# Nextomics/NextPolish2

Hardware: AMD Instinct MI355X
Metric: polished reference Mbp/s (whole node) at 30x HiFi + k21/k31; FASTA identical to oracle (higher is better)
Workload: dtype u8

## Files before the change

### nextpolish2_amd/csrc/np2_batch.cpp

```cpp
#include "../../include/np2.h"
#include "np2_ctx.hpp"

#include <atomic>
#include <climits>
#include <cstring>
#include <condition_variable>
#include <mutex>
#include <thread>
#include <pthread.h>

#include <linux/futex.h>
#include <sys/syscall.h>
#include <unistd.h>

using namespace np2;

namespace {

struct Job {
    np2_contig *contig = nullptr;
    const np2_opts_t *opts = nullptr;
    uint8_t **out_bases = nullptr;
    uint32_t **out_pos = nullptr;
    uint64_t *out_len = nullptr;
    uint32_t *out_span = nullptr;
    int *rc = nullptr;
};

}

struct np2_batch {
    np2_ctx *parent = nullptr;
    int device = 0;
    hipStream_t stream = nullptr;
    std::vector<np2_ctx *> slots;
    std::vector<Recorder> recs;
    std::vector<std::thread> workers;
    std::string err;

    std::mutex mu;
    std::condition_variable cv_start, cv_done;
    uint64_t job_gen = 0;
    std::vector<Job> jobs;
    int n_running = 0;
    bool quit = false;

    std::mutex sync_mu;
    int n_active = 0, n_waiting = 0;
    std::atomic<uint32_t> flush_gen{0};
    std::atomic<bool> failed{false};
    std::string fail_msg;

    uint32_t *done_host = nullptr, *done_dev = nullptr;
    uint32_t done_seq = 0;
    std::atomic<uint32_t> issued_seq{0};
    std::atomic<uint32_t> done_pub{0};
    std::atomic<bool> spinner{false};
    double t_issued_last = 0;
    uint32_t wait_logged_seq = 0;

    bool time_diff = false;
    std::vector<std::pair<hipEvent_t, hipEvent_t>> diff_events;
    size_t diff_used = 0;
    float last_diff_ms = 0;
    int last_diff_launches = 0;
    uint64_t stat_launches = 0, stat_cmds = 0, stat_flushes = 0;
    double t_last_end = 0, ms_host = 0, ms_issue = 0, ms_wait = 0;
    std::vector<double> flush_log;
    double call_ms = 0, tail_ms = 0;
};

namespace {

inline void wait_generation(std::atomic<uint32_t> &gen, uint32_t seen) {
    static const double spin_us = getenv("NP2_BATCH_SPIN_US") ? atof(getenv("NP2_BATCH_SPIN_US")) : (wait_naps() ? 0.0 : 5.0);
    const double t_end = now_ms() + spin_us * 1e-3;
    for (;;) {
        for (int i = 0; i < 64; ++i) {
            if (gen.load(std::memory_order_acquire) != seen) return;
            __builtin_ia32_pause();
        }
        if (now_ms() >= t_end) break;
    }
    while (gen.load(std::memory_order_acquire) == seen)
        (void)syscall(SYS_futex, reinterpret_cast<uint32_t *>(&gen), FUTEX_WAIT_PRIVATE, seen, nullptr, nullptr, 0);
}
inline void publish_generation(std::atomic<uint32_t> &gen, uint32_t next) {
    gen.store(next, std::memory_order_release);
    (void)syscall(SYS_futex, reinterpret_cast<uint32_t *>(&gen), FUTEX_WAKE_PRIVATE, INT_MAX, nullptr, nullptr, 0);
}

__device__ __forceinline__ void k_flush_done(const uint32_t np2_bid, const uint32_t np2_nb, uint32_t *__restrict__ word, uint32_t seq) {
    if (threadIdx.x == 0) {
        __threadfence_system();
        __hip_atomic_store(word, seq, __ATOMIC_RELEASE, __HIP_MEMORY_SCOPE_SYSTEM);
    }
}

void flush(np2_batch *b) {
    const int n = (int)b->recs.size();
    const double t_begin = now_ms();
    double t_issued = t_begin;
    std::vector<size_t> idx(n, 0);
    hipStream_t s = b->stream;
    Recorder *saved = tl_recorder();
    tl_recorder() = nullptr;
    try {
        for (;;) {
            bool any = false;
            for (int i = 0; i < n; ++i) {
                auto &q = b->recs[i].q;
                while (idx[i] < q.size() && !q[idx[i]].kd) {
                    q[idx[i]].fn(s);
                    ++idx[i];
                    ++b->stat_cmds;
                }
                any |= idx[i] < q.size();
            }
            if (!any) break;
            const KernelDesc *best = nullptr;
            int best_n = 0, best_defer = 0;
            static constexpr size_t LOOKAHEAD = 8;
            for (int i = 0; i < n; ++i) {
                auto &q = b->recs[i].q;
                if (idx[i] >= q.size()) continue;
                const KernelDesc *kd = q[idx[i]].kd;
                bool seen = false;
                for (int j = 0; j < i && !seen; ++j)
                    seen = idx[j] < b->recs[j].q.size() && b->recs[j].q[idx[j]].kd == kd;
                if (seen) continue;
                int c = 0, defer = 0;
                for (int j = 0; j < n; ++j) {
                    auto &qj = b->recs[j].q;
                    if (idx[j] >= qj.size()) continue;
                    if (qj[idx[j]].kd == kd) {
                        ++c;
                        continue;
                    }
                    for (size_t k = idx[j] + 1; k < qj.size() && k <= idx[j] + LOOKAHEAD; ++k)
                        if (qj[k].kd == kd) {
                            ++defer;
                            break;
                        }
                }
                if (!best || defer < best_defer || (defer == best_defer && c > best_n)) best = kd, best_n = c, best_defer = defer;
            }
            uint32_t grids[MAXB];
            const void *args[MAXB];
            int m = 0;
            const bool timed = b->time_diff && strcmp(best->name, "k_diff_reads") == 0;
            auto issue = [&]() {
                if (!m) return;
                if (timed) {
                    if (b->diff_used == b->diff_events.size()) {
                        hipEvent_t e0 = nullptr, e1 = nullptr;
                        HIPCHK(hipEventCreate(&e0));
                        HIPCHK(hipEventCreate(&e1));
                        b->diff_events.push_back({e0, e1});
                    }
                    HIPCHK(hipEventRecord(b->diff_events[b->diff_used].first, s));
                }
                best->launch(s, m, grids, args);
                if (timed) {
                    HIPCHK(hipEventRecord(b->diff_events[b->diff_used].second, s));
                    ++b->diff_used;
                }
                ++b->stat_launches;
                m = 0;
            };
            for (int i = 0; i < n; ++i) {
                auto &r = b->recs[i];
                if (idx[i] >= r.q.size() || r.q[idx[i]].kd != best) continue;
                grids[m] = r.q[idx[i]].grid;
                args[m] = r.arena.data() + r.q[idx[i]].arg_off;
                ++m;
                ++idx[i];
                ++b->stat_cmds;
                if (m == best->max_batch) issue();
            }
            issue();
        }
        HIPCHK(hipGetLastError());
        const uint32_t seq = ++b->done_seq;
        NP2_LAUNCH(k_flush_done, 1, 64, s, b->done_dev, seq);
        t_issued = now_ms();
        b->issued_seq.store(seq, std::memory_order_release);
    } catch (const std::exception &ex) {
        b->fail_msg = ex.what();
        b->failed.store(true);
        (void)hipStreamSynchronize(s);
        for (np2_ctx *cx : b->slots) cx->lb_dirty = true, cx->h2d_inflight = false;
    }
    tl_recorder() = saved;
    for (auto &r : b->recs) r.clear();
    ++b->stat_flushes;
    b->ms_host += t_begin - b->t_last_end;
    b->ms_issue += t_issued - t_begin;
    b->flush_log.push_back(t_begin - b->t_last_end);
    b->flush_log.push_back(t_issued - t_begin);
    b->flush_log.push_back(0.0);
    b->t_last_end = t_issued;
    b->t_issued_last = t_issued;
}

void wait_done(np2_batch *b, uint32_t seq) {
    for (;;) {
        const uint32_t pub = b->done_pub.load(std::memory_order_acquire);
        if ((int32_t)(pub - seq) >= 0 || b->failed.load()) break;
        bool expected = false;
        if (b->spinner.compare_exchange_strong(expected, true)) {
            uint64_t spins = 0;
            uint32_t cur;
            HostWait hw;
            while ((int32_t)((cur = __atomic_load_n(b->done_host, __ATOMIC_ACQUIRE)) - seq) < 0) {
                if (b->failed.load()) break;
                if ((++spins & (wait_naps() ? 0xFFu : 0xFFFFu)) == 0) {
                    hipError_t e = hipStreamQuery(b->stream);
                    if (e != hipSuccess && e != hipErrorNotReady) {
                        b->fail_msg = std::string("device error during a batch flush: ") + hipGetErrorString(e);
                        b->failed.store(true);
                        break;
                    }
                    if (e == hipSuccess && (int32_t)(__atomic_load_n(b->done_host, __ATOMIC_ACQUIRE) - seq) < 0) {
                        b->fail_msg = "batch flush completed without posting";
                        b->failed.store(true);
                        break;
                    }
                }
                hw.pause();
            }
            b->spinner.store(false);
            publish_generation(b->done_pub, b->failed.load() ? pub + 1 : cur);
            if (b->failed.load()) return;
            continue;
        }
        wait_generation(b->done_pub, pub);
    }
    if (b->failed.load()) return;
    std::lock_guard<std::mutex> l(b->sync_mu);
    if (b->wait_logged_seq != seq && b->issued_seq.load() == seq && !b->flush_log.empty()) {
        const double t = now_ms();
        b->wait_logged_seq = seq;
        b->ms_wait += t - b->t_issued_last;
        b->flush_log.back() = t - b->t_issued_last;
        b->t_last_end = t;
    }
}

void group_sync(Recorder *r, bool need_done) {
    np2_batch *b = (np2_batch *)r->group;
    uint32_t my_gen;
    bool flushed = false;
    {
        std::lock_guard<std::mutex> l(b->sync_mu);
        my_gen = b->flush_gen.load(std::memory_order_relaxed);
        if (++b->n_waiting == b->n_active) {
            flush(b);
            b->n_waiting = 0;
            publish_generation(b->flush_gen, my_gen + 1);
            flushed = true;
        }
    }
    if (!flushed) wait_generation(b->flush_gen, my_gen);
    if (need_done && !b->failed.load()) wait_done(b, b->issued_seq.load(std::memory_order_acquire));
    if (b->failed.load()) throw Np2Error(NP2_E_DEVICE, "batch flush failed: " + b->fail_msg);
}

void leave_wave(np2_batch *b, Recorder *r) {
    std::lock_guard<std::mutex> l(b->sync_mu);
    if (!r->q.empty()) {
        np2_ctx *cx = b->slots[r->slot];
        cx->lb_dirty = true;
        cx->h2d_inflight = false;
    }
    r->clear();
    --b->n_active;
    if (b->n_active > 0 && b->n_waiting == b->n_active) {
        const uint32_t g = b->flush_gen.load(std::memory_order_relaxed);
        flush(b);
        b->n_waiting = 0;
        publish_generation(b->flush_gen, g + 1);
    }
}

void worker_main(np2_batch *b, int slot) {
    (void)hipSetDevice(b->device);
    (void)pthread_setname_np(pthread_self(), "np2-slot");
    uint64_t seen = 0;
    for (;;) {
        Job job;
        {
            std::unique_lock<std::mutex> l(b->mu);
            b->cv_start.wait(l, [&] { return b->quit || b->job_gen != seen; });
            if (b->quit) return;
            seen = b->job_gen;
            job = b->jobs[slot];
        }
        if (!job.contig) continue;
        Recorder *r = &b->recs[slot];
        tl_recorder() = r;
        int rc = np2_polish_resident(b->slots[slot], job.contig, job.opts, job.out_bases, job.out_pos, job.out_len);
        tl_recorder() = nullptr;
        for (auto &g : r->graveyard)
            dev_release_idle(g.first, (g.second >> 63) ? 0 : g.second, (g.second >> 63) ? (g.second & ~(1ull << 63)) : 0);
        r->graveyard.clear();
        leave_wave(b, r);
        if (rc == NP2_OK && job.out_span) (void)np2_last_span(b->slots[slot], &job.out_span[0], &job.out_span[1]);
        *job.rc = rc;
        {
            std::lock_guard<std::mutex> l(b->mu);
            if (--b->n_running == 0) b->cv_done.notify_all();
        }
    }
}

auto batch_sink(np2_batch *b) {
    return [b](int, const std::string &msg) { b->err = msg; };
}

}

extern "C" {

int np2_batch_create(np2_batch_t **out, np2_ctx_t *parent, int n_slots) {
    if (!out || !parent || n_slots < 1 || n_slots > 256) return NP2_E_ARG;
    *out = nullptr;
    return abi_guard([&] {
        std::unique_ptr<np2_batch, void (*)(np2_batch_t *)> b(new np2_batch(), np2_batch_destroy);
        b->parent = parent;
        b->device = parent->device;
        HIPCHK(hipSetDevice(b->device));
        HIPCHK(hipStreamCreateWithFlags(&b->stream, hipStreamNonBlocking));
        HIPCHK(hipHostMalloc((void **)&b->done_host, 256 * (size_t)(n_slots + 1), hipHostMallocMapped | hipHostMallocCoherent));
        memset(b->done_host, 0, 256 * (size_t)(n_slots + 1));
        HIPCHK(hipHostGetDevicePointer((void **)&b->done_dev, b->done_host, 0));
        b->recs.resize(n_slots);
        b->jobs.resize(n_slots);
        for (int i = 0; i < n_slots; ++i) {
            np2_ctx *cx = ctx_create_slot(parent, b->stream, b->done_host + 64 * (size_t)(i + 1), b->done_dev + 64 * (size_t)(i + 1));
            b->slots.push_back(cx);
            b->recs[i].group = b.get();
            b->recs[i].slot = i;
            b->recs[i].sync_fn = &group_sync;
        }
        for (int i = 0; i < n_slots; ++i) b->workers.emplace_back(worker_main, b.get(), i);
        *out = b.release();
        return NP2_OK;
    }, [parent](int, const std::string &msg) { parent->err = msg; });
}

void np2_batch_destroy(np2_batch_t *b) {
    if (!b) return;
    {
        std::lock_guard<std::mutex> l(b->mu);
        b->quit = true;
    }
    b->cv_start.notify_all();
    for (auto &t : b->workers) t.join();
    (void)hipSetDevice(b->device);
    if (b->stream) (void)hipStreamSynchronize(b->stream);
    {
        DevSyncScope idle;
        for (np2_ctx *cx : b->slots) np2_ctx_destroy(cx);
    }
    for (auto &e : b->diff_events) {
        (void)hipEventDestroy(e.first);
        (void)hipEventDestroy(e.second);
    }
    if (b->done_host) (void)hipHostFree(b->done_host);
    if (b->stream) (void)hipStreamDestroy(b->stream);
    delete b;
}

int np2_batch_set_priority(np2_batch_t *b, int high) {
    if (!b) return NP2_E_ARG;
    return abi_guard([&] {
        HIPCHK(hipSetDevice(b->device));
        int least = 0, greatest = 0;
        HIPCHK(hipDeviceGetStreamPriorityRange(&least, &greatest));
        HIPCHK(hipStreamSynchronize(b->stream));
        hipStream_t s = nullptr;
        HIPCHK(hipStreamCreateWithPriority(&s, hipStreamNonBlocking, high ? greatest : least));
        (void)hipStreamDestroy(b->stream);
        b->stream = s;
        for (np2_ctx *cx : b->slots) ctx_slot_set_stream(cx, s);
        return NP2_OK;
    }, batch_sink(b));
}

int np2_batch_slots(np2_batch_t *b) { return b ? (int)b->slots.size() : 0; }
np2_ctx_t *np2_batch_slot_ctx(np2_batch_t *b, int slot) {
    return (b && slot >= 0 && slot < (int)b->slots.size()) ? b->slots[slot] : nullptr;
}
const char *np2_batch_last_error(np2_batch_t *b) { return b ? b->err.c_str() : "null batch"; }
int np2_batch_set_sink(np2_batch_t *b, int slot, void *device_ptr, uint64_t cap) {
    if (!b || slot < 0 || slot >= (int)b->slots.size()) return NP2_E_ARG;
    b->slots[slot]->sink_dst = (uint8_t *)device_ptr;
    b->slots[slot]->sink_cap = device_ptr ? cap : 0;
    return NP2_OK;
}

int np2_batch_polish(np2_batch_t *b, np2_contig_t *const *contigs, int n, const np2_opts_t *opts, uint8_t **out_bases,
                     uint32_t **out_pos, uint64_t *out_len, uint32_t *out_span, int *rcs) {
    if (!b || !contigs || n < 0 || !opts || !out_len || !rcs) return NP2_E_ARG;
    return abi_guard([&] {
        const int S = (int)b->slots.size();
        int worst = NP2_OK;
        b->diff_used = 0;
        b->flush_log.clear();
        b->t_last_end = now_ms();
        const double t_call0 = b->t_last_end;
        for (int w0 = 0; w0 < n; w0 += S) {
            const int m = std::min(S, n - w0);
            {
                std::lock_guard<std::mutex> l(b->mu);
                for (int i = 0; i < S; ++i) {
                    Job j;
                    if (i < m) {
                        j.contig = contigs[w0 + i];
                        j.opts = opts;
                        j.out_bases = out_bases ? &out_bases[w0 + i] : nullptr;
                        j.out_pos = out_pos ? &out_pos[w0 + i] : nullptr;
                        j.out_len = &out_len[w0 + i];
                        j.out_span = out_span ? &out_span[2 * (w0 + i)] : nullptr;
                        j.rc = &rcs[w0 + i];
                    }
                    b->jobs[i] = j;
                }
                b->n_running = m;
                {
                    std::lock_guard<std::mutex> l2(b->sync_mu);
                    b->n_active = m;
                    b->n_waiting = 0;
                    b->failed.store(false);
                }
                ++b->job_gen;
            }
            b->cv_start.notify_all();
            {
                std::unique_lock<std::mutex> l(b->mu);
                b->cv_done.wait(l, [&] { return b->n_running == 0; });
            }
            for (int i = 0; i < m; ++i)
                if (rcs[w0 + i] != NP2_OK) {
                    worst = rcs[w0 + i];
                    b->err = std::string("contig ") + std::to_string(w0 + i) + ": " + np2_last_error(b->slots[i]);
                }
        }
        b->call_ms = now_ms() - t_call0;
        b->tail_ms = now_ms() - b->t_last_end;
        if (b->time_diff) {
            b->last_diff_ms = 0;
// ... 41 lines not shown
```

### nextpolish2_amd/csrc/np2_cand.hip

```cpp
#include "np2_common.hpp"
#include "np2_kernels.hpp"
#include "np2_blockscan.hpp"
#include "np2_lookback.hpp"

namespace np2 {

template <int MODE>
__device__ __forceinline__ void k_scan_small(const uint32_t np2_bid, const uint32_t np2_nb, const uint32_t *__restrict__ in, uint32_t *__restrict__ out,
                                                     uint32_t n_host, const uint32_t *__restrict__ n_dev,
                                                     uint32_t *__restrict__ total_out, bool write_end) {
    __shared__ uint32_t sh[16];
    const uint32_t n = n_dev ? min(*n_dev, n_host) : n_host;
    uint32_t total;
    if (MODE == 2) {
        total = block_scan_array<OpMinI32>(
            n, sh, [&](uint32_t i) { return in[i]; },
            [&](uint32_t i, uint32_t pre, uint32_t v) { out[i] = OpMinI32::apply(pre, v); });
    } else {
        total = block_scan_array<OpAdd>(
            n, sh, [&](uint32_t i) { return in[i]; },
            [&](uint32_t i, uint32_t pre, uint32_t v) { out[i] = MODE == 0 ? pre : pre + v; });
    }
    if (threadIdx.x == 0) {
        if (MODE == 0 && write_end) out[n] = total;
        if (total_out) *total_out = total;
    }
}

static constexpr uint32_t SCAN_LB_ITEMS = 8;
static constexpr uint32_t SCAN_LB_THREADS = 1024;
static constexpr uint32_t SCAN_LB_BLOCK = SCAN_LB_ITEMS * SCAN_LB_THREADS;
template <bool POPC>
__device__ __forceinline__ void scan_lb_excl_body(const uint32_t np2_bid, const uint32_t np2_nb, Lookback lb, uint32_t n_blocks, const uint32_t *__restrict__ in,
                                                      uint32_t *__restrict__ out, uint32_t n, bool write_end,
                                                      uint32_t *__restrict__ err) {
    __shared__ uint32_t sh[16];
    const uint32_t bid = lb_block_id(lb, sh);
    const uint32_t i0 = bid * SCAN_LB_BLOCK + threadIdx.x * SCAN_LB_ITEMS;
    uint32_t v[SCAN_LB_ITEMS], sum = 0;
    const bool wide = (((uintptr_t)in | (uintptr_t)out) & 15) == 0;
    if (wide && i0 + SCAN_LB_ITEMS <= (POPC ? n - 1 : n)) {
        const uint4 a = *reinterpret_cast<const uint4 *>(in + i0), b = *reinterpret_cast<const uint4 *>(in + i0 + 4);
        v[0] = a.x, v[1] = a.y, v[2] = a.z, v[3] = a.w, v[4] = b.x, v[5] = b.y, v[6] = b.z, v[7] = b.w;
    } else {
#pragma unroll
        for (uint32_t k = 0; k < SCAN_LB_ITEMS; ++k) v[k] = i0 + k < (POPC ? n - 1 : n) ? in[i0 + k] : 0u;
    }
    if (POPC) {
#pragma unroll
        for (uint32_t k = 0; k < SCAN_LB_ITEMS; ++k) v[k] = (uint32_t)__builtin_popcount(v[k]);
    }
#pragma unroll
    for (uint32_t k = 0; k < SCAN_LB_ITEMS; ++k) sum += v[k];
    uint32_t total, pre, dummy;
    uint32_t run = block_excl_scan<OpAdd, 16>(sum, sh, total);
    lb_exclusive2(lb, bid, total, 0u, sh, err, pre, dummy);
    run += pre;
    if (wide && i0 + SCAN_LB_ITEMS <= n) {
        uint4 a, b;
        a.x = run, a.y = a.x + v[0], a.z = a.y + v[1], a.w = a.z + v[2];
        b.x = a.w + v[3], b.y = b.x + v[4], b.z = b.y + v[5], b.w = b.z + v[6];
        *reinterpret_cast<uint4 *>(out + i0) = a;
        *reinterpret_cast<uint4 *>(out + i0 + 4) = b;
        run = b.w + v[7];
    } else {
#pragma unroll
        for (uint32_t k = 0; k < SCAN_LB_ITEMS; ++k) {
            if (i0 + k < n) out[i0 + k] = run;
            run += v[k];
        }
    }
    if (write_end && n && i0 <= n - 1 && n - 1 < i0 + SCAN_LB_ITEMS) out[n] = run;
    if (write_end && n == 0 && bid == 0 && threadIdx.x == 0) out[0] = 0;
}

__device__ __forceinline__ void k_scan_lb_excl(const uint32_t np2_bid, const uint32_t np2_nb, Lookback lb, uint32_t n_blocks, const uint32_t *__restrict__ in,
                                               uint32_t *__restrict__ out, uint32_t n, bool write_end, uint32_t *__restrict__ err) {
    scan_lb_excl_body<false>(np2_bid, np2_nb, lb, n_blocks, in, out, n, write_end, err);
}
__device__ __forceinline__ void k_scan_lb_popc(const uint32_t np2_bid, const uint32_t np2_nb, Lookback lb, uint32_t n_blocks, const uint32_t *__restrict__ in,
                                               uint32_t *__restrict__ out, uint32_t n, bool write_end, uint32_t *__restrict__ err) {
    scan_lb_excl_body<true>(np2_bid, np2_nb, lb, n_blocks, in, out, n, write_end, err);
}

struct CandCtx {
    const np2_read_t *reads;
    const uint8_t *nib;
    const uint64_t *ck_off;
    const uint32_t *ckpt;
    const uint32_t *lq_start;
    const uint32_t *lq_end;
    const uint32_t *pj;
    const uint32_t *pcount;
    const uint8_t *alive;
    const ReadInfo *rinfo;
    const uint32_t *tile_rd_off;
    const uint32_t *tile_rd;
    uint32_t n_tiles;
    uint32_t ksize;
    const uint64_t *rec_key;
    const uint32_t *rec_read;
    const uint32_t *tile_n;
    const uint16_t *rec_pidx;
    uint32_t bucket_cap;
    const uint32_t *refnib;
    uint32_t L;
};

__device__ __forceinline__ void cand_anchor(const CandCtx &cx, uint32_t r, const np2_read_t &rd, uint64_t ck_off, uint32_t start,
                                            uint32_t &col, uint32_t &t) {
    col = 0;
    t = rd.aln_t_s;
    const uint32_t ck_first = (rd.aln_t_s + CKPT - 1) >> CKPT_SHIFT;
    const uint32_t cki = start >> CKPT_SHIFT;
    if (r == 0) {
        col = start;
        t = start;
    } else if (cki >= ck_first) {
        col = cx.ckpt[ck_off + (cki - ck_first)];
        t = cki << CKPT_SHIFT;
    }
}

__device__ __forceinline__ uint32_t nth_col16(uint64_t m64, uint32_t n) {
    uint32_t col = 0;
    uint32_t m = (uint32_t)m64;
    uint32_t c = (uint32_t)__builtin_popcount(m);
    if (n > c) n -= c, col = 8, m = (uint32_t)(m64 >> 32);
    c = (uint32_t)__builtin_popcount(m & 0xFFFFu);
    if (n > c) n -= c, col += 4, m >>= 16;
    c = (uint32_t)__builtin_popcount(m & 0xFFu);
    if (n > c) n -= c, col += 2, m >>= 8;
    c = (uint32_t)__builtin_popcount(m & 0xFu);
    if (n > c) col += 1;
    return col;
}

__device__ uint32_t cand_measure(const CandCtx &cx, uint32_t r, const np2_read_t &rd, uint64_t ck_off, uint32_t start,
                                 uint32_t end, uint32_t &col_start) {
    uint32_t col_ck, t_ck;
    cand_anchor(cx, r, rd, ck_off, start, col_ck, t_ck);
    col_start = col_ck;
    if (end < t_ck) return 0;
    const uint32_t want_s = (start > t_ck ? start - t_ck : 0u) + 1;
    const uint32_t want_e = end + 1 - t_ck + 1;
    const uint8_t *base = cx.nib + rd.nib_off;
    const uint32_t n_cols = rd.n_cols;
    uint32_t seen = 0, len = 0;
    bool started = false;
    uint4 win = make_uint4(0, 0, 0, 0);
    uint32_t win_blk = 0xFFFFFFFFu;
    const uint64_t N1 = 0x1111111111111111ULL;
    for (uint32_t wi = col_ck >> 4;; ++wi) {
        const uint32_t c0 = wi << 4;
        if (c0 >= n_cols) break;
        if ((wi >> 1) != win_blk) {
            win_blk = wi >> 1;
            win = *reinterpret_cast<const uint4 *>(base + ((size_t)win_blk << 4));
        }
        const uint32_t r0 = (wi & 1) ? win.z : win.x, r1 = (wi & 1) ? win.w : win.y;
        const uint64_t w = (uint64_t)(((r0 & 0x0F0F0F0Fu) << 4) | ((r0 >> 4) & 0x0F0F0F0Fu)) |
                           ((uint64_t)(((r1 & 0x0F0F0F0Fu) << 4) | ((r1 >> 4) & 0x0F0F0F0Fu)) << 32);
        uint64_t valid = N1;
        if (c0 < col_ck) valid &= ~((1ULL << (4 * (col_ck - c0))) - 1ULL);
        if (n_cols - c0 < 16) valid &= (1ULL << (4 * (n_cols - c0))) - 1ULL;
// ... 402 lines not shown
        if (lane == 0) {
            reg_ncand[g] = kept;
            reg_bytes[g] = bytes;
            reg_maxlen[g] = mx;
        }
        sum_k[h / 4] += kept, sum_b[h / 4] += bytes, sum_m[h / 4] += mx;
    }
#pragma unroll
    for (uint32_t q = 0; q < RM_RPW / 4; ++q)
        if (lane == 0 && mb0 + q < n_mb) {
            blk_sum[mb0 + q] = sum_k[q];
            blk_sum[n_mb + mb0 + q] = sum_b[q];
            blk_sum[2 * n_mb + mb0 + q] = sum_m[q];
        }
}

__device__ __forceinline__ void k_cand_offsets(const uint32_t np2_bid, const uint32_t np2_nb, const uint32_t *__restrict__ blk_sum, uint32_t n_blk,
                                                       uint32_t n_reg, uint32_t *__restrict__ blk_coff,
                                                       uint32_t *__restrict__ blk_soff, uint32_t *__restrict__ cand_off,
                                                       uint32_t *__restrict__ reg_soff, uint32_t *__restrict__ n_cand,
                                                       uint32_t *__restrict__ n_bytes, uint32_t *__restrict__ grow) {
    __shared__ uint32_t sh[16];
    const uint32_t ta = block_scan_array<OpAdd>(
        n_blk, sh, [&](uint32_t i) { return blk_sum[i]; }, [&](uint32_t i, uint32_t pre, uint32_t) { blk_coff[i] = pre; });
    const uint32_t tb = block_scan_array<OpAdd>(
        n_blk, sh, [&](uint32_t i) { return blk_sum[n_blk + i]; },
        [&](uint32_t i, uint32_t pre, uint32_t) { blk_soff[i] = pre; });
    const uint32_t tc = block_scan_array<OpAdd>(
        n_blk, sh, [&](uint32_t i) { return blk_sum[2 * n_blk + i]; }, [&](uint32_t, uint32_t, uint32_t) {});
    if (threadIdx.x == 0) {
        cand_off[n_reg] = ta;
        reg_soff[n_reg] = tb;
        *n_cand = ta;
        *n_bytes = tb;
        *grow = tc;
    }
}

__device__ __forceinline__ void k_cand_offsets_lb(const uint32_t np2_bid, const uint32_t np2_nb, Lookback lb, uint32_t n_blocks, const uint32_t *__restrict__ blk_sum,
                                                         uint32_t n_blk, uint32_t n_reg, uint32_t *__restrict__ blk_coff,
                                                         uint32_t *__restrict__ blk_soff, uint32_t *__restrict__ cand_off,
                                                         uint32_t *__restrict__ reg_soff, uint32_t *__restrict__ n_cand,
                                                         uint32_t *__restrict__ n_bytes, uint32_t *__restrict__ grow,
                                                         uint32_t *__restrict__ err) {
    __shared__ uint32_t sh[8];
    const uint32_t bid = lb_block_id(lb, sh);
    const uint32_t i0 = (bid * 256 + threadIdx.x) * 4;
    uint32_t a[4], b[4], sa = 0, sb = 0;
#pragma unroll
    for (uint32_t k = 0; k < 4; ++k) {
        a[k] = i0 + k < n_blk ? blk_sum[i0 + k] : 0u;
        b[k] = i0 + k < n_blk ? blk_sum[n_blk + i0 + k] : 0u;
        sa += a[k];
        sb += b[k];
    }
    uint32_t ta, tb, pa, pb;
    uint32_t ra = block_excl_scan<OpAdd, 4>(sa, sh, ta);
    uint32_t rb = block_excl_scan<OpAdd, 4>(sb, sh, tb);
    lb_exclusive2(lb, bid, ta, tb, sh, err, pa, pb);
    ra += pa, rb += pb;
#pragma unroll
    for (uint32_t k = 0; k < 4; ++k)
        if (i0 + k < n_blk) {
            blk_coff[i0 + k] = ra;
            blk_soff[i0 + k] = rb;
            ra += a[k];
            rb += b[k];
        }
    if (bid == n_blocks - 1 && threadIdx.x == 255) {
        cand_off[n_reg] = ra;
        reg_soff[n_reg] = rb;
        *n_cand = ra;
        *n_bytes = rb;
    }
    if (bid == 0) {
        uint32_t c = 0, tc;
        for (uint32_t i = threadIdx.x; i < n_blk; i += 256) c += blk_sum[2 * n_blk + i];
        (void)block_excl_scan<OpAdd, 4>(c, sh, tc);
        if (threadIdx.x == 0) *grow = tc;
    }
}

static constexpr uint32_t MERGE_LB_BLOCKS = 32;
__device__ __forceinline__ void k_lq_merge_scan_lb(const uint32_t np2_bid, const uint32_t np2_nb, Lookback lb, const uint32_t *__restrict__ raw_start,
                                                   const uint32_t *__restrict__ raw_end, const uint32_t *__restrict__ n_raw, uint32_t n_host,
                                                   uint32_t *__restrict__ headflag, uint32_t *__restrict__ hidx, uint32_t *__restrict__ err) {
    __shared__ uint32_t sh[16];
    const uint32_t bid = lb_block_id(lb, sh);
    const uint32_t n = min(*n_raw, n_host);
    const uint32_t seg = ((n + MERGE_LB_BLOCKS - 1) / MERGE_LB_BLOCKS + 1023u) & ~1023u;
    const uint32_t lo = min(bid * seg, n), hi = min(lo + seg, n);
    auto flag = [&](uint32_t j) { return (j >= 1 && raw_end[j] >= raw_start[j - 1]) ? 0u : 1u; };
    uint32_t cnt = 0;
    for (uint32_t j = lo + threadIdx.x; j < hi; j += 1024) cnt += flag(j);
    uint32_t total, pre, dummy;
    (void)block_excl_scan<OpAdd, 16>(cnt, sh, total);
    lb_exclusive2(lb, bid, total, 0u, sh, err, pre, dummy);
    uint32_t carry = pre;
    for (uint32_t j0 = lo; j0 < hi; j0 += 1024) {
        const uint32_t j = j0 + threadIdx.x;
        const uint32_t v = j < hi ? flag(j) : 0u;
        uint32_t tot;
        const uint32_t ex = block_excl_scan<OpAdd, 16>(v, sh, tot);
        if (j < hi) {
            hidx[j] = carry + ex;
            headflag[j] = v;
        }
        carry += tot;
    }
}

__device__ __forceinline__ void k_region_write(const uint32_t np2_bid0, const uint32_t np2_nb, CandCtx cx, uint32_t n_reg, const uint32_t *__restrict__ kept_read,
                                                      const uint32_t *__restrict__ kept_len,
                                                      const uint32_t *__restrict__ kept_col,
                                                      const uint32_t *__restrict__ reg_ncand,
                                                      const uint32_t *__restrict__ reg_bytes,
                                                      const uint32_t *__restrict__ blk_coff,
                                                      const uint32_t *__restrict__ blk_soff,
                                                      uint32_t *__restrict__ cand_off, uint32_t *__restrict__ reg_soff,
                                                      uint32_t cand_cap,
                                                      uint32_t seq_cap, uint32_t *__restrict__ cand_order,
                                                      uint64_t *__restrict__ cand_kmer, uint32_t *__restrict__ cand_seq_off,
                                                      uint8_t *__restrict__ cand_seq) {
    const uint32_t np2_bid = xcd_order(np2_bid0, np2_nb);
    __shared__ __attribute__((aligned(4))) uint8_t s_str[RM_REG][CLEAN_MAX_LEN];
    __shared__ uint64_t s_km[RM_REG];
    __shared__ uint32_t s_so[RM_REG][64];
    __shared__ uint32_t s_oc[RM_REG];
    __shared__ uint32_t s_q[4][RM_RPW * 64];
    const uint32_t lane = threadIdx.x & 63, wv = (uint32_t)__builtin_amdgcn_readfirstlane((int)(threadIdx.x >> 6));
    const uint32_t g0 = (np2_bid * 4 + wv) * RM_RPW, mb0 = g0 / 4;
    uint32_t nq = 0;
    uint32_t oc = 0, ob = 0;
    if (g0 < n_reg) oc = blk_coff[mb0], ob = blk_soff[mb0];
    uint32_t clean_h = 0;
    uint32_t my_len[RM_RPW], my_so[RM_RPW], my_ci[RM_RPW];
    bool my_clean[RM_RPW];
    uint32_t n[RM_RPW], rb[RM_RPW], st[RM_RPW], ln0[RM_RPW];
#pragma unroll
    for (uint32_t h = 0; h < RM_RPW; ++h) {
        const uint32_t g = g0 + h;
        n[h] = 0, rb[h] = 0, st[h] = 0, ln0[h] = 0;
        if (g < n_reg) n[h] = reg_ncand[g], rb[h] = reg_bytes[g], st[h] = cx.lq_start[g], ln0[h] = cx.lq_end[g] - st[h] + 1;
    }
    uint32_t len[RM_RPW], col[RM_RPW], rd_[RM_RPW], refc[RM_RPW];
#pragma unroll
    for (uint32_t h = 0; h < RM_RPW; ++h) {
        const size_t ks = (size_t)(g0 + h) * LQSEQ_MAX_CAN_COUNT + lane;
        const bool act = lane < n[h];
        len[h] = act ? kept_len[ks] : 0u;
        col[h] = act ? kept_col[ks] : 0u;
        rd_[h] = act ? kept_read[ks] : 0u;
        const uint32_t p = st[h] + lane;
        refc[h] = (n[h] && lane < ln0[h] && ln0[h] <= CLEAN_MAX_LEN) ? cx.refnib[p >> 3] >> (4 * (p & 7)) : 0u;
    }
#pragma unroll
    for (uint32_t h = 0; h < RM_RPW; ++h) {
        const uint32_t g = g0 + h, slot = wv * RM_RPW + h;
        my_len[h] = 0, my_so[h] = 0, my_ci[h] = 0, my_clean[h] = false;
        if (g >= n_reg) continue;
        if (g == n_reg - 1 && lane == 0 && cand_off[n_reg] < cand_cap) cand_seq_off[cand_off[n_reg]] = reg_soff[n_reg];
        if (lane == 0) {
            cand_off[g] = oc;
            reg_soff[g] = ob;
            s_oc[slot] = oc;
        }
        const bool act = lane < n[h];
        const uint32_t so = ob + wave_excl(len[h]);
        const uint32_t ci = oc + lane;
        const bool ok = act && ci < cand_cap && (uint64_t)so + len[h] <= seq_cap;
        if (ok) {
            cand_order[ci] = rd_[h];
            cand_seq_off[ci] = so;
        }
        const bool clean = ok && col[h] == CAND_CLEAN;
        const uint64_t cm = __ballot(clean);
        const bool queued = ok && (!clean || (lane == 0 && rd_[h] == 0));
        my_len[h] = len[h], my_so[h] = so, my_ci[h] = ci, my_clean[h] = clean && !queued;
        s_so[slot][lane] = so;
        if (cm) {
            clean_h |= 1u << h;
            if (lane < ln0[h]) s_str[slot][lane] = (uint8_t)((0x54474341u >> (8 * (refc[h] & 3))) & 0xFFu);
        }
        const uint64_t dq = __ballot(queued);
        if (queued) s_q[wv][nq + lanes_below(dq)] = (slot << 6) | lane;
        nq += (uint32_t)__builtin_popcountll(dq);
        oc += n[h];
        ob += rb[h];
    }
    wave_lds_sync();
    for (uint32_t e = lane; e < nq; e += 64) {
        const uint32_t w = s_q[wv][e], slot = w >> 6, li = w & 63;
        const uint32_t g = (np2_bid * 4 + slot / RM_RPW) * RM_RPW + slot % RM_RPW;
        const size_t ks = (size_t)g * LQSEQ_MAX_CAN_COUNT + li;
        const uint32_t r = kept_read[ks], len = kept_len[ks];
        uint32_t col = kept_col[ks];
        const ReadInfo ri = cx.rinfo[r];
        const np2_read_t rd = rinfo_read(ri);
        const uint32_t t0 = max(cx.lq_start[g], rd.aln_t_s);
        if (col == CAND_CLEAN) col = t0;
        const uint32_t ci = s_oc[slot] + li;
        uint64_t km;
        cand_write(cx, r, rd, ri.pj, g, col, t0, len, cand_seq + s_so[slot][li], &km);
        cand_kmer[ci] = km;
        if (li == 0 && r == 0) s_km[slot] = km;
    }
    wave_lds_sync();
#pragma unroll
    for (uint32_t h = 0; h < RM_RPW; ++h) {
        if (!((clean_h >> h) & 1u)) continue;
        const uint32_t slot = wv * RM_RPW + h;
        if (my_clean[h]) {
            cand_kmer[my_ci[h]] = s_km[slot];
            typedef uint32_t u32_any __attribute__((aligned(1)));
            uint8_t *dst = cand_seq + my_so[h];
            const uint32_t L4 = my_len[h] & ~3u;
            for (uint32_t j = 0; j < L4; j += 4) *reinterpret_cast<u32_any *>(dst + j) = *reinterpret_cast<const uint32_t *>(&s_str[slot][j]);
            for (uint32_t j = L4; j < my_len[h]; ++j) dst[j] = s_str[slot][j];
        }
    }
}

void launch_scan_small_excl(hipStream_t s, const uint32_t *in, uint32_t *out, uint32_t n, const uint32_t *n_dev,
                            uint32_t *total_out, bool write_end) {
    NP2_LAUNCH(k_scan_small<0>, dim3(1), 1024, s, in, out, n, n_dev, total_out, write_end);
}
void launch_scan_lb_excl(hipStream_t s, const Lookback &lb, const uint32_t *in, uint32_t *out, uint32_t n, bool write_end,
                          uint32_t *err) {
    const uint32_t nb = scan_lb_blocks(n);
    NP2_LAUNCH(k_scan_lb_excl, dim3(nb), SCAN_LB_THREADS, s, lb, nb, in, out, n, write_end, err);
}
void launch_scan_lb_popc(hipStream_t s, const Lookback &lb, const uint32_t *bits, uint32_t *out, uint32_t n_words, uint32_t *err) {
    const uint32_t nb = scan_lb_blocks((uint64_t)n_words + 1);
    NP2_LAUNCH(k_scan_lb_popc, dim3(nb), SCAN_LB_THREADS, s, lb, nb, bits, out, n_words + 1, false, err);
}
uint32_t scan_lb_blocks(uint64_t n) { return (uint32_t)std::max<uint64_t>(1, (n + SCAN_LB_BLOCK - 1) / SCAN_LB_BLOCK); }
void launch_scan_small_incl(hipStream_t s, const int32_t *in, int32_t *out, uint32_t n, const uint32_t *n_dev) {
    NP2_LAUNCH(k_scan_small<1>, dim3(1), 1024, s, (const uint32_t *)in, (uint32_t *)out, n, n_dev, (uint32_t *)nullptr, false);
}
void launch_scan_small_min(hipStream_t s, const int32_t *in, int32_t *out, uint32_t n, const uint32_t *n_dev) {
    NP2_LAUNCH(k_scan_small<2>, dim3(1), 1024, s, (const uint32_t *)in, (uint32_t *)out, n, n_dev, (uint32_t *)nullptr, false);
}
static CandCtx mk_cand(const CandPtrs &c) {
    return CandCtx{c.reads, c.nib,    c.ck_off, c.ckpt,        c.lq_start, c.lq_end, c.pj,
                   c.pcount, c.alive, c.rinfo, c.tile_rd_off, c.tile_rd, c.n_tiles,  c.ksize,
                   c.rec_key, c.rec_read, c.tile_n, c.rec_pidx, c.bucket_cap, c.refnib, c.L};
}
void launch_region_measure(hipStream_t s, const CandPtrs &c, uint32_t n_reg, uint32_t *kept_read, uint32_t *kept_len,
                           uint32_t *kept_col, uint32_t *reg_ncand, uint32_t *reg_bytes, uint32_t *reg_maxlen,
                           uint32_t *blk_sum) {
    if (n_reg)
        NP2_LAUNCH_WAVES(k_region_measure, RM_WAVES, dim3((n_reg + RM_REG - 1) / RM_REG), 256, s,
                         mk_cand(c), n_reg, kept_read, kept_len, kept_col, reg_ncand, reg_bytes, reg_maxlen, blk_sum);
}
uint32_t cand_offsets_blocks(uint32_t n_reg) { return ((n_reg + 3) / 4 + 1023) / 1024; }
void launch_cand_offsets(hipStream_t s, const uint32_t *blk_sum, uint32_t n_reg, uint32_t *blk_coff, uint32_t *blk_soff,
                         uint32_t *cand_off, uint32_t *reg_soff, uint32_t *n_cand, uint32_t *n_bytes, uint32_t *grow,
                         const Lookback *lb, uint32_t *err) {
    if (lb)
        NP2_LAUNCH(k_cand_offsets_lb, dim3(cand_offsets_blocks(n_reg)), 256, s, *lb, cand_offsets_blocks(n_reg), blk_sum, (n_reg + 3) / 4, n_reg, blk_coff, blk_soff, cand_off, reg_soff, n_cand, n_bytes, grow, err);
    else
        NP2_LAUNCH(k_cand_offsets, dim3(1), 1024, s, blk_sum, (n_reg + 3) / 4, n_reg, blk_coff, blk_soff, cand_off, reg_soff, n_cand, n_bytes, grow);
}
void launch_lq_merge_scan_lb(hipStream_t s, const Lookback &lb, const uint32_t *raw_start, const uint32_t *raw_end, const uint32_t *n_raw,
                             uint32_t n_host, uint32_t *headflag, uint32_t *hidx, uint32_t *err) {
    NP2_LAUNCH(k_lq_merge_scan_lb, dim3(MERGE_LB_BLOCKS), 1024, s, lb, raw_start, raw_end, n_raw, n_host, headflag, hidx, err);
}
uint32_t lq_merge_lb_blocks() { return MERGE_LB_BLOCKS; }
void launch_region_write(hipStream_t s, const CandPtrs &c, uint32_t n_reg, const uint32_t *kept_read,
                         const uint32_t *kept_len, const uint32_t *kept_col, const uint32_t *reg_ncand,
                         const uint32_t *reg_bytes, const uint32_t *blk_coff, const uint32_t *blk_soff, uint32_t *cand_off,
                         uint32_t *reg_soff, uint32_t cand_cap, uint32_t seq_cap, uint32_t *cand_order, uint64_t *cand_kmer,
                         uint32_t *cand_seq_off, uint8_t *cand_seq) {
    if (n_reg)
        NP2_LAUNCH(k_region_write, dim3((n_reg + RM_REG - 1) / RM_REG), 256, s, mk_cand(c), n_reg, kept_read, kept_len, kept_col, reg_ncand, reg_bytes, blk_coff, blk_soff, cand_off, reg_soff, cand_cap, seq_cap, cand_order, cand_kmer, cand_seq_off, cand_seq);
}

}
```

### nextpolish2_amd/csrc/np2_ctx.hpp

```cpp
#pragma once
#include "../../include/np2.h"
#include "np2_abi.hpp"
#include "np2_common.hpp"
#include "np2_kernels.hpp"
#include "np2_hostcpu.hpp"

#include <algorithm>
#include <chrono>
#include <cstdio>
#include <cstdlib>
#include <cstring>
#include <map>
#include <memory>
#include <exception>
#include <mutex>
#include <stdexcept>
#include <string>
#include <vector>

namespace np2h {

using namespace np2;


// ... 341 lines not shown
}

struct YakTable {
    uint32_t k = 0, cap_log2 = 0;
    std::shared_ptr<DevBuf<uint64_t>> table;
    std::shared_ptr<DevBuf<uint32_t>> ord;
    YakDev dev() const { return YakDev{table->p, cap_log2, k, ord ? ord->p : nullptr}; }
};

struct Timing {
    std::vector<std::string> names;
    std::vector<float> ms;
    std::string joined;
    std::vector<std::pair<std::string, float>> host;
};
inline double now_ms() {
    return std::chrono::duration<double, std::milli>(std::chrono::steady_clock::now().time_since_epoch()).count();
}


}

using namespace np2h;

struct np2_contig {
    np2_contig() {
        reads.cached = nib.cached = refnib.cached = ck_off.cached = ckpt.cached = descs.cached = true;
        tile_rd_off.cached = tile_rd.cached = true;
    }
    uint32_t L = 0, R = 0;
    uint64_t nib_bytes = 0, n_cols = 0, n_ckpt = 0;
    DevBuf<np2_read_t> reads;
    DevBuf<uint8_t> nib;
    DevBuf<uint8_t> refnib;
    uint32_t ref_stride = 0;
    DevBuf<uint64_t> ck_off;
    DevBuf<uint32_t> ckpt;
    uint32_t n_chunks = 0;
    DevBuf<ChunkDesc> descs;
    uint32_t n_tiles = 0;
    DevBuf<uint32_t> tile_rd_off, tile_rd;
    uint32_t tile_cap = TILE_CAP;
};

struct np2_ctx {
    int device = 0;
    hipStream_t stream = nullptr;
    hipStream_t stream_out = nullptr;
    hipEvent_t ev_out = nullptr;
    uint8_t *out_host[2] = {nullptr, nullptr};
    size_t out_host_cap[2] = {0, 0};
    int out_slot = 0;
    bool out_pending = false;
    uint64_t out_len = 0;
    std::vector<YakTable> yaks;
    std::string err;
    bool trace = false;
    std::map<std::string, std::vector<uint8_t>> trace_items;
    Timing timing;
    std::vector<std::pair<std::string, std::pair<hipEvent_t, hipEvent_t>>> pending_events;

    PinnedBuf pin_d2h, pin_h2d;
    uint32_t *mbox_host = nullptr, *mbox_dev = nullptr;
    uint32_t mbox_seq = 0;
    bool borrowed_state = false;
    uint8_t *sink_dst = nullptr;
    uint64_t sink_cap = 0;
    uint32_t last_first_pos = 0, last_last_pos = 0;
    const uint8_t *last_dbase = nullptr;
    const uint32_t *last_dpos = nullptr;
    DevBuf<uint32_t> shard_bounds;
    uint64_t last_len = 0;
    bool reuse_identical_pass = true;
    bool h2d_inflight = false;
    bool stage_timing = false;
    DevBuf<uint8_t> tmp;
    DevBuf<uint64_t> keys_raw, keys;
    DevBuf<uint32_t> vals_raw, vals;
    DevBuf<uint32_t> npos, ncount, nminr, nbesti, node_off, run_start, run_end, n0_besti, emit, eoff;
    DevBuf<uint16_t> nbases, ndelta;
    DevBuf<int64_t> nscore;
    DevBuf<int32_t> cov, mval, smin;
    DevBuf<uint8_t> alive, cns_base, cns_cls, lq_kind, lq_nothead;
    DevBuf<uint32_t> cns_pos, lq_next, rflag, rstart, rend, ridx, raw_start, raw_end, headflag, hidx, lq_start,
        lq_end;
    DevBuf<uint32_t> pj, pcount, reg_ncand, reg_bytes, reg_soff, reg_maxlen, blk_sum, blk_coff, blk_soff, kept_read, kept_len, kept_col, cand_off, cand_order, cand_seq_off, kill_ids;
    DevBuf<uint64_t> cand_kmer;
    DevBuf<uint8_t> cand_seq;
    DevBuf<uint16_t> kscore;
    DevBuf<uint32_t> scal;
    DevBuf<uint64_t> lb_status;
    DevBuf<uint32_t> lb_ticket;
    uint32_t lb_ticket_total = 0, lb_epoch = 0;
    bool lb_dirty = false;
    static constexpr size_t LB_MAX_BLOCKS = 1u << 20;
    DevBuf<uint32_t> mlen;
    DevBuf<uint8_t> reg_lable, grp, cns_base2, rech_groups, rech_groups_tmp;
    DevBuf<uint8_t> votepack;
    DevBuf<uint8_t> votepack2;
    DevBuf<uint32_t> rech_headjobs;
    DevBuf<uint32_t> ecount, eval, eval_s, eflag, eidx, seed_cand, keep_n, keep_list, cns_pos2, sp_idx_s,
        sp_idx_e, ap_g, ap_s, ap_e, rech, rech_joboff, job_len,
        job_off32;
    DevBuf<int32_t> ew, ap_delta, ap_shift;
    DevBuf<uint64_t> ekey, ekey_s;
    DevBuf<uint16_t> keep_ks;
    DevBuf<uint32_t> long_list;
    DevBuf<uint64_t> bt_path;
    DevBuf<uint64_t> chunk_st;
    uint32_t chunk_epoch = 0;
    DevBuf<uint32_t> tile_cur, tile_n, tile_scan, tile_scanb, tile_nn, tile_nr, tile_noff, tile_roff;
    uint32_t tile_cap = TILE_CAP;
    uint32_t bucket_cap = 0;
    DevBuf<uint2> nrec;
    DevBuf<uint8_t> votebuf;
    DevBuf<uint32_t> band, band_n, band_off, row_cnt;
    DevBuf<int64_t> run_gain, tile_gain;
    DevBuf<uint8_t> out_snap;
    DevBuf<uint8_t> run_flag;
    uint32_t deep_min = 65536;
    DevBuf<uint32_t> lq_list, hbits;
    DevBuf<uint16_t> tile_pidx;
    bool pidx_valid = false;
    DevBuf<ReadInfo> rinfo;
    DevBuf<uint32_t> lqc, lqoff;
    DevBuf<uint8_t> pflag;
    DevBuf<uint32_t> dp_list;
    DevBuf<uint16_t> pf_slots;
    DevBuf<uint32_t> pf_bad, pf_bad2;
    DevBuf<uint64_t> pf_prof;
    bool front_fused = false;
    struct Hooks {
        bool front_unfused = false, pf_prof = false, edge_sort = false;
        bool test_misspeculate = false, shard_spec_log = false, phase_profile = false, exact_grow = false, no_speculate = false;
        bool has_grow_guess = false;
        uint32_t grow_guess = 0;
        bool has_pf_cap = false, has_pf_cap_big = false, has_pf_halo = false, has_pf_cov_max = false;
        uint32_t pf_cap = 0, pf_cap_big = 0, pf_halo = 0, pf_cov_max = 0;
        void read() {
            auto on = [](const char *n) { return getenv(n) != nullptr; };
            auto u32 = [](const char *n, bool &has, uint32_t &v) {
                if (const char *e = getenv(n)) has = true, v = (uint32_t)atol(e);
            };
            front_unfused = on("NP2_FRONT_UNFUSED"), pf_prof = on("NP2_PF_PROF"), edge_sort = on("NP2_EDGE_SORT");
            test_misspeculate = on("NP2_TEST_MISSPECULATE");
            shard_spec_log = on("NP2_SHARD_SPEC_LOG"), phase_profile = on("NP2_PHASE_PROFILE"), exact_grow = on("NP2_EXACT_GROW");
            no_speculate = on("NP2_NO_SPECULATE");
            u32("NP2_TEST_GROW_GUESS", has_grow_guess, grow_guess);
            u32("NP2_PF_CAP", has_pf_cap, pf_cap), u32("NP2_PF_CAP_BIG", has_pf_cap_big, pf_cap_big);
            u32("NP2_PF_HALO", has_pf_halo, pf_halo), u32("NP2_PF_COV_MAX", has_pf_cov_max, pf_cov_max);
        }
    } hooks;
    bool pf_big = getenv("NP2_PF_BIG") != nullptr;
    uint32_t front_redos = 0;
    DevBuf<uint16_t> kscore_saved;
    DevBuf<uint8_t> sstr;
    DevBuf<uint64_t> soff;
    DevBuf<uint16_t> sscore;
};


namespace np2h {


enum Scal { S_ERR = 0, S_NNODES, S_NRUNS, S_BEST, S_PATHBEGIN, S_NRAW, S_NREG, S_DUP, S_LAST0, S_LAST1, S_GAIN0,
            S_GAIN1, S_DEEP, S_NDPLIST, S_NRECH, S_NGROUPS, S_NLONG, S_NLQ, S_PF, S_M0, S_M1, S_M2, S_M3, S_NC, S_SB, S_GROW,
            S_NBAD, S_PFOUT, S_PFGAIN0, S_PFGAIN1, S_PFEND0, S_PFEND1, S_NBAD2, S_NOKEY, S_COUNT = 34 };
static_assert(S_M1 % 2 == 0 && S_LAST0 % 2 == 0 && S_GAIN0 % 2 == 0 && S_PFGAIN0 % 2 == 0 && S_PFEND0 % 2 == 0,
              "64-bit device counters live in these slot pairs");

static constexpr int NP2_MAX_YAK = 15;
static constexpr uint32_t SCAL_TOTAL = 96;
static_assert(S_COUNT + 2 * (NP2_MAX_YAK + 2) <= SCAL_TOTAL && S_COUNT < 64, "round counters behind the posted block; the mailbox holds 64 words");

inline double thread_cpu_ms() {
    timespec ts;
    clock_gettime(CLOCK_THREAD_CPUTIME_ID, &ts);
    return ts.tv_sec * 1e3 + ts.tv_nsec * 1e-6;
}
struct WallTimer {
    np2_ctx *cx;
    const char *name;
    double t0, c0 = 0;
    WallTimer(np2_ctx *c, const char *n);
    ~WallTimer();
};
// ... 247 lines not shown
```

### nextpolish2_amd/csrc/np2_host.cpp

```cpp
#include "../../include/np2.h"
#include "np2_common.hpp"
#include "np2_kernels.hpp"
#include "np2_ctx.hpp"
#include "np2_phase_host.hpp"

#include <algorithm>
#include <atomic>
#include <thread>
#include <chrono>
#include <cstdio>
#include <cstdlib>
#include <cstring>
#include <map>
#include <mutex>
#include <stdexcept>
#include <string>
#include <unordered_map>
#include <unordered_set>
#include <future>
#include <functional>
#include <vector>

using namespace np2;

// ... 130 lines not shown
            off_own.assign(off, off + R + 1);
            edges_own.assign(edges, edges + off[R]);
            off = off_own.data(), edges = edges_own.data();
        }
        if (!view_key) return;
        pair_key.assign(view_key, view_key + view_n);
        pair_cnt.assign(view_cnt, view_cnt + view_n);
        view_key = nullptr, view_cnt = nullptr, view_n = 0;
    }
    std::vector<uint32_t> first_key;
    std::vector<int32_t> ref_w;
    std::vector<uint8_t> ref_seen, bad;
    const uint8_t *d_bad = nullptr;
    bool key_added = false;
};

bool vote_rows_from_pairs(VoteData &vd, bool use_all) {
    const uint32_t R = vd.R;
    const uint64_t *k = vd.keys();
    const uint32_t *cn = vd.cnts();
    const uint64_t np = vd.n_pairs();
    std::vector<uint32_t> n_lo(R, 0), n_up(R, 0);
    uint32_t nokey = 0;
    auto listed = [&](uint64_t i, uint32_t &a, uint32_t &b) {
        a = (uint32_t)(k[i] >> 32), b = (uint32_t)k[i];
        if (a >= R || b >= R || vd.first_key[a] == 0xFFFFFFFFu || vd.first_key[b] == 0xFFFFFFFFu) return false;
        return use_all || !(vd.bad[a] | vd.bad[b]);
    };
    for (uint64_t i = 0; i < np; ++i) {
        uint32_t a = (uint32_t)(k[i] >> 32), b = (uint32_t)k[i];
        if (b <= a || b - a - 1 >= EDGE_BAND || (i && k[i - 1] >= k[i])) return false;
        if (a >= R || b >= R || vd.first_key[a] == 0xFFFFFFFFu || vd.first_key[b] == 0xFFFFFFFFu) ++nokey;
        if (listed(i, a, b)) ++n_lo[b], ++n_up[a];
    }
    vd.off_own.assign((size_t)R + 1, 0);
    std::vector<uint32_t> cur_lo(R), cur_up(R);
    for (uint32_t v = 0; v < R; ++v) {
        cur_lo[v] = vd.off_own[v], cur_up[v] = vd.off_own[v] + n_lo[v];
        vd.off_own[v + 1] = cur_up[v] + n_up[v];
    }
    vd.edges_own.resize(vd.off_own[R]);
    for (uint64_t i = 0; i < np; ++i) {
        uint32_t a, b;
        if (!listed(i, a, b)) continue;
        const int32_t same = (int32_t)(cn[i] & 0xFFFFu), neg = (int32_t)(cn[i] >> 16);
        const float w = (float)(neg >= 3 ? -neg : same - neg);
        vd.edges_own[cur_lo[b]++] = phase::Graph::Edge(a, w);
        vd.edges_own[cur_up[a]++] = phase::Graph::Edge(b, w);
    }
    vd.off = vd.off_own.data(), vd.edges = vd.edges_own.data(), vd.n_nokey = nokey;
    return true;
}

void vote_collect(np2_ctx *cx, np2_contig *c, PassCounts &pc, bool asref, bool use_all, int pass, uint32_t own_lo,
                  uint32_t own_hi, VoteData &vd, bool wide = false, uint64_t key_add = 0) {
    hipStream_t s = cx->stream;
    const uint32_t R = c->R, n_reg = pc.n_reg;
    RegionTables rt = region_tables(cx, n_reg);
    uint32_t NE = 0, NU = 0;
    vd = VoteData();
    vd.R = R;
    {
        EventTimer t(cx, "vote_phase");
        cx->reg_lable.ensure(n_reg + 2);
        cx->grp.ensure((size_t)pc.NC_cap + 2);
        cx->ecount.ensure(n_reg + 2);
        cx->eoff.ensure(std::max<size_t>(n_reg + 2, (size_t)c->L + 2));
        const size_t RP = ((size_t)R + 63) & ~(size_t)63;
        const size_t band_words = (size_t)R * EDGE_BAND;
        const size_t b_v = RP * 10, b_off = (((size_t)R + 2) * 4 + 15) & ~(size_t)15;
        uint8_t *vbuf;
        uint32_t *row_off;
        if (wide) {
            cx->votebuf.ensure(b_v);
            cx->band_off.ensure((size_t)R + 2);
            vbuf = cx->votebuf.p, row_off = cx->band_off.p;
        } else {
            cx->votepack.ensure(b_v + b_off + band_words * 2 * sizeof(phase::Graph::Edge) + 64);
            vbuf = cx->votepack.p, row_off = (uint32_t *)(cx->votepack.p + b_v);
        }
        uint32_t *v_first = (uint32_t *)vbuf;
        int32_t *v_refw = (int32_t *)(vbuf + RP * 4);
        uint8_t *v_seen = vbuf + RP * 8, *v_bad = vbuf + RP * 9;
        op_fill(cx, v_first, 0xFF, RP * 4);
        op_fill(cx, v_refw, 0, RP * 6);
        launch_vote_phase(s, rt, asref, use_all, cx->lq_start.p, own_lo, own_hi, cx->reg_lable.p, cx->grp.p, cx->ecount.p,
                          v_refw, v_seen, v_bad, v_first, cx->scal.p + S_ERR);
        exclusive_total_n(cx, cx->ecount.p, cx->eoff.p, n_reg);
        launch_vote_counts(s, v_first, v_bad, R, cx->scal.p + S_M1);
        cx->band.ensure(band_words + 4);
        cx->band_n.ensure((size_t)R + 2);
        op_fill(cx, cx->scal.p + S_M3, 0, 4);
        launch_edges_row(s, rt, cx->grp.p, cx->ecount.p, cx->pj.p, cx->pcount.p, cx->alive.p, R, cx->band.p, cx->band_n.p,
                         cx->scal.p + S_M3);
        if (wide) {
            exclusive_total_n(cx, cx->band_n.p, row_off, R);
            cx->ekey.ensure(band_words + 2);
            cx->eval.ensure(band_words + 2);
            launch_band_emit(s, cx->band.p, R, row_off, cx->ekey.p, cx->eval.p, cx->scal.p + S_NRAW, key_add);
        } else {
            cx->row_cnt.ensure((size_t)R + 2);
            launch_vote_rows_count(s, cx->band.p, cx->band_n.p, v_bad, use_all, R, cx->row_cnt.p, cx->scal.p + S_NOKEY);
            exclusive_total_n(cx, cx->row_cnt.p, row_off, R);
            launch_vote_rows_emit(s, cx->band.p, cx->band_n.p, v_bad, use_all, v_first, R, row_off, cx->votepack.p + b_v + b_off,
                                  cx->scal.p + S_NRAW, cx->scal.p + S_NOKEY);
        }
    }
    const size_t RP = ((size_t)R + 63) & ~(size_t)63;
    const size_t b_v = RP * 10, b_off = (((size_t)R + 2) * 4 + 15) & ~(size_t)15;
    auto per_read = [&](const uint8_t *vb) {
        vd.first_key.assign((const uint32_t *)vb, (const uint32_t *)vb + R);
        vd.ref_w.assign((const int32_t *)(vb + RP * 4), (const int32_t *)(vb + RP * 4) + R);
        vd.ref_seen.assign(vb + RP * 8, vb + RP * 8 + R);
        vd.bad.assign(vb + RP * 9, vb + RP * 9 + R);
    };
    bool far = false, have_per_read = false;
    {
        std::vector<uint32_t> sc;
        uint8_t *pin = nullptr;
        const size_t EB = sizeof(phase::Graph::Edge);
        static_assert(sizeof(phase::Graph::Edge) == 8 && alignof(phase::Graph::Edge) <= 8, "an edge is {u32 neighbour, f32 weight}");
        const uint32_t likely = (uint32_t)std::min<size_t>((size_t)R * EDGE_BAND * 2, std::max<size_t>((size_t)R * 128, 1u << 15));
        if (wide) {
            sc = fetch_scal(cx, cx->scal.p + S_M0, cx->eoff.p + n_reg);
        } else {
            pin = (uint8_t *)cx->pin_d2h.ensure(b_v + b_off + (size_t)likely * EB + 64);
            const uint32_t seq = ++cx->mbox_seq;
            launch_post(cx->stream, cx->scal.p, S_COUNT, cx->mbox_dev, seq, cx->scal.p + S_M0, cx->eoff.p + n_reg, nullptr, nullptr,
                        nullptr, nullptr, nullptr, nullptr, nullptr, nullptr);
            op_d2h(cx, pin, cx->votepack.p, b_v + b_off);
            launch_copy_counted(cx->stream, (uint32_t *)(pin + b_v + b_off), (const uint32_t *)(cx->votepack.p + b_v + b_off),
                                (const uint32_t *)(cx->votepack.p + b_v) + R, likely * (uint32_t)(EB / 4), (uint32_t)(EB / 4));
            op_sync(cx);
            if (__atomic_load_n(&cx->mbox_host[0], __ATOMIC_ACQUIRE) != seq)
                throw Np2Error(NP2_E_DEVICE, "mailbox not posted after a synchronisation");
            sc.assign(cx->mbox_host + 1, cx->mbox_host + 1 + S_COUNT);
        }
        check_region_err(cx, sc[S_ERR]);
        pc.resolve(sc);
        NE = sc[S_M0];
        if (!cx->trace && sc[S_M1] == 0 && sc[S_M2] == 0) {
            if (NE) throw Np2Error(NP2_E_DEVICE, "internal: pair edges without voting reads");
            return;
        }
        NU = sc[S_NRAW];
        far = sc[S_M3] != 0 || cx->hooks.edge_sort;
        if (!wide) cx->timing.host.push_back({far ? "vote_sort" : "vote_rows", 1.0f});
        if (!wide) {
            per_read(pin);
            have_per_read = true;
            vd.d_bad = cx->votepack.p + RP * 9;
            if (!far) {
                if (NU > likely) {
                    pin = (uint8_t *)cx->pin_d2h.ensure(b_v + b_off + (size_t)NU * EB + 64);
                    op_d2h(cx, pin, cx->votepack.p, b_v + b_off + (size_t)NU * EB);
                    op_sync(cx);
                }
                vd.off = (const uint32_t *)(pin + b_v), vd.edges = (const phase::Graph::Edge *)(pin + b_v + b_off);
                vd.n_nokey = sc[S_NOKEY];
                if (vd.off[R] != NU) throw Np2Error(NP2_E_DEVICE, "internal: vote rows and edge count disagree");
            }
        }
    }
    vd.any = true;
    if (NE && far) {
        {
            EventTimer t(cx, "vote_phase");
            cx->ekey.ensure(NE + 2);
            cx->ekey_s.ensure(NE + 2);
            cx->eval.ensure(NE + 2);
            cx->eval_s.ensure(NE + 2);
            cx->eflag.ensure(NE + 2);
            cx->eidx.ensure(NE + 2);
            cx->ew.ensure(NE + 2);
            cx->tmp.ensure(prim_temp_bytes((size_t)NE + 2));
// ... 139 lines not shown
        else throw Np2Error(NP2_E_DEVICE, "internal: loser outside the contig's reads");
    losers.clear();
    for (uint32_t r = 0; r < R; ++r)
        if (lost[r]) losers.push_back(r);
    return losers;
}

struct CnsDev {
    uint32_t *pos;
    uint8_t *base;
    const uint32_t *M_p;
    uint32_t M_cap;
};

CnsDev splice_gpu(np2_ctx *cx, const CnsDev &in, uint32_t n_reg, uint8_t lable, uint32_t grow_bound, bool to_b,
                  uint32_t version) {
    hipStream_t s = cx->stream;
    EventTimer t(cx, "splice");
    cx->sp_idx_s.ensure(n_reg + 2);
    cx->sp_idx_e.ensure(n_reg + 2);
    cx->ap_g.ensure(n_reg + 2);
    cx->ap_s.ensure(n_reg + 2);
    cx->ap_e.ensure(n_reg + 2);
    cx->ap_delta.ensure(n_reg + 2);
    cx->ap_shift.ensure(n_reg + 2);
    cx->mlen.ensure(16);
    const uint32_t out_cap = in.M_cap + grow_bound;
    const size_t cap = (size_t)out_cap + 64;
    uint32_t *opos = to_b ? cx->cns_pos2.ensure(cap) : cx->cns_pos.ensure(cap);
    uint8_t *obase = to_b ? cx->cns_base2.ensure(cap) : cx->cns_base.ensure(cap);
    uint32_t *const stuck_p = cx->scal.p + S_COUNT + 2 * version, *const nap_p = stuck_p + 1;
    launch_splice_find(s, in.pos, in.M_p, cx->lq_start.p, cx->lq_end.p, cx->reg_lable.p, lable, n_reg, cx->sp_idx_s.p,
                       cx->sp_idx_e.p, stuck_p);
    launch_splice_plan(s, next_lookback(cx, region_lb_blocks(n_reg)), cx->reg_lable.p, lable, n_reg, stuck_p,
                       cx->sp_idx_s.p, cx->sp_idx_e.p, cx->seed_cand.p, cx->cand_seq_off.p, cx->ap_g.p, cx->ap_s.p,
                       cx->ap_e.p, cx->ap_delta.p, cx->ap_shift.p, nap_p, in.M_p, cx->mlen.p + version, out_cap,
                       cx->scal.p + S_ERR);
    launch_splice_write(s, in.pos, in.base, in.M_p, in.M_cap, cx->ap_g.p, cx->ap_s.p, cx->ap_e.p, cx->ap_delta.p,
                        cx->ap_shift.p, nap_p, n_reg, cx->lq_start.p, cx->seed_cand.p, cx->cand_seq_off.p,
                        cx->cand_seq.p, opos, obase);
    return CnsDev{opos, obase, cx->mlen.p + version, out_cap};
}

Cns fetch_cns_dev(np2_ctx *cx, const CnsDev &c) {
    Cns r;
    const uint32_t M = d2h(cx, c.M_p, 1)[0];
    r.pos = d2h(cx, c.pos, M);
    r.base = d2h(cx, c.base, M);
    return r;
}

CnsDev recheck_gpu(np2_ctx *cx, const CnsDev &in, const PassCounts &pc, int yak_idx, uint16_t min_kmer_count,
                   bool first_yak, bool to_b, uint32_t version) {
    hipStream_t s = cx->stream;
    const uint32_t n_reg = pc.n_reg, ksize = cx->yaks[yak_idx].k;
    uint32_t n_rech = 0, n_groups = 0, n_jobs = 0;
    uint64_t blob_bound = 0;
    {
        EventTimer t(cx, "recheck");
        cx->rech.ensure(n_reg + 2);
        cx->rech_groups.ensure((size_t)(n_reg + 2) * rech_group_bytes());
        cx->rech_joboff.ensure(n_reg + 2);
        cx->rech_groups_tmp.ensure((size_t)(n_reg + 2) * rech_group_bytes());
        cx->rech_headjobs.ensure(n_reg + 2);
        launch_rech_list(s, next_lookback(cx, region_lb_blocks(n_reg)), cx->reg_lable.p, n_reg, cx->rech.p, cx->scal.p + S_NRECH,
                         (unsigned long long *)(cx->scal.p + S_M1), cx->scal.p + S_ERR);
        launch_rech_groups(s, next_lookback(cx, region_lb_blocks(n_reg)), cx->rech.p, cx->scal.p + S_NRECH, n_reg, in.pos, in.M_p,
                           cx->lq_start.p, cx->lq_end.p, cx->keep_n.p, ksize, cx->reg_maxlen.p, cx->rech_groups_tmp.p,
                           cx->rech_headjobs.p, cx->rech_groups.p,
                           cx->rech_joboff.p, cx->scal.p + S_NGROUPS,
                           cx->scal.p + S_M0, (unsigned long long *)(cx->scal.p + S_M1), cx->scal.p + S_ERR);
        std::vector<uint32_t> sc = fetch_scal(cx);
        blob_bound = (uint64_t)sc[S_M1] | ((uint64_t)sc[S_M2] << 32);
        check_region_err(cx, sc[S_ERR]);
        n_rech = sc[S_NRECH];
        n_groups = sc[S_NGROUPS];
        n_jobs = sc[S_M0];
    }
    if (n_rech) {
        RechPtrs rp{cx->rech_groups.p, cx->rech_joboff.p, cx->rech.p, cx->cand_off.p, cx->keep_list.p,
                    cx->cand_seq_off.p, cx->cand_seq.p, in.base, n_groups};
        if (n_jobs) {
            EventTimer t(cx, "recheck");
            cx->job_len.ensure(n_jobs + 2);
            cx->job_off32.ensure(n_jobs + 2);
            cx->soff.ensure(n_jobs + 2);
            cx->sscore.ensure(n_jobs + 2);
            cx->tmp.ensure(prim_temp_bytes((size_t)n_jobs + 2));
            launch_rech_job_len(s, rp, n_jobs, cx->job_len.p);
            exclusive_total_n(cx, cx->job_len.p, cx->job_off32.p, n_jobs);
            if (blob_bound >= 0xFFFFFFF0ull)
                blob_bound = fetch_scal(cx, cx->scal.p + S_M0, cx->job_off32.p + n_jobs)[S_M0];
            cx->sstr.ensure((size_t)blob_bound + 64);
            launch_rech_job_build(s, rp, n_jobs, cx->job_off32.p, cx->soff.p, cx->sstr.p);
            launch_score_strings(s, cx->yaks[yak_idx].dev(), cx->sstr.p, cx->soff.p, n_jobs, min_kmer_count,
                                 cx->sscore.p, true);
            launch_rech_apply(s, rp, cx->sscore.p, cx->keep_ks.p);
        }
        EventTimer t(cx, "recheck");
        launch_rech_select(s, cx->rech.p, cx->scal.p + S_NRECH, n_rech, cx->cand_off.p, cx->keep_n.p, cx->keep_list.p,
                           cx->keep_ks.p, cx->cand_order.p, first_yak, cx->reg_lable.p, cx->seed_cand.p);
    }
    CnsDev out = splice_gpu(cx, in, n_reg, LB_RECH, pc.grow, to_b, version);
    launch_rech_relabel(s, cx->reg_lable.p, n_reg);
    return out;
}

void gpu_score_strings(np2_ctx *cx, int yak_idx, const std::vector<uint8_t> &blob, const std::vector<uint64_t> &off,
                       uint16_t min_kmer_count, std::vector<uint16_t> &scores) {
    const size_t n = off.size() - 1;
    scores.assign(n, 0);
    if (!n) return;
    cx->sstr.ensure(blob.size() + 16);
    cx->soff.ensure(off.size());
    cx->sscore.ensure(n);
    {
        op_sync(cx);
        uint8_t *pin = (uint8_t *)cx->pin_h2d.ensure(blob.size() + off.size() * 8 + 16);
        const size_t o2 = (blob.size() + 7) & ~(size_t)7;
        memcpy(pin, blob.data(), blob.size());
        memcpy(pin + o2, off.data(), off.size() * 8);
        op_h2d(cx, cx->sstr.p, pin, blob.size());
        op_h2d(cx, cx->soff.p, pin + o2, off.size() * 8);
        cx->h2d_inflight = true;
    }
    {
        EventTimer t(cx, "score_strings");
        launch_score_strings(cx->stream, cx->yaks[yak_idx].dev(), cx->sstr.p, cx->soff.p, n, min_kmer_count,
                             cx->sscore.p, false);
    }
    scores = d2h(cx, cx->sscore.p, n);
}

struct PassOut {
    bool has_regions = false;
    Cns cns;
};

void run_diff(np2_ctx *cx, np2_contig *c, uint32_t &T) {
    hipStream_t s = cx->stream;
    const uint32_t L = c->L, R = c->R, NCH = c->n_chunks;
    const uint32_t n_tiles = (L + TILE - 1) >> TILE_SHIFT;
    const uint32_t bcap = std::min(cx->tile_cap, c->tile_cap);
    const uint64_t buckets = (uint64_t)n_tiles * bcap;
    uint64_t ovf_cap = std::max<uint64_t>(c->n_cols / 256 + 65536, 1u << 18);
    cx->tmp.ensure(prim_temp_bytes(std::max<size_t>((size_t)NCH + 2, (size_t)L + 2)));
    cx->tile_n.ensure(n_tiles + 2);
    cx->tile_scan.ensure(n_tiles + 2);
    cx->tile_scanb.ensure(n_tiles + 2);
    cx->tile_nn.ensure(n_tiles + 2);
    cx->tile_nr.ensure(n_tiles + 2);
    cx->tile_noff.ensure(n_tiles + 2);
    cx->tile_roff.ensure(n_tiles + 2);
    cx->tile_gain.ensure(n_tiles + 2);
    if (cx->tile_cur.cap < (size_t)n_tiles + 2) {
        cx->tile_cur.ensure(n_tiles + 2);
        zero32(cx, cx->tile_cur.p, cx->tile_cur.cap);
    }
    if (cx->chunk_st.cap < (size_t)NCH + 2) {
        cx->chunk_st.ensure(NCH + 2);
        zero32(cx, cx->chunk_st.p, cx->chunk_st.cap, 8);
    }
    static const bool precount_env = getenv("NP2_DENSE_PRECOUNT") != nullptr;
    bool precount = precount_env;
    for (int attempt = 0; attempt < 4; ++attempt) {
        if (ovf_cap >= 0xFFFFFFF0ull) throw Np2Error(NP2_E_NOMEM, "too many exception nodes");
        cx->keys_raw.ensure(buckets + ovf_cap + 1);
        cx->vals_raw.ensure(buckets + ovf_cap + 1);
        zero32(cx, cx->scal.p, SCAL_TOTAL);
        if (++cx->chunk_epoch == 0) ++cx->chunk_epoch;
        if (precount) launch_chunk_counts(s, c->descs.p, NCH, c->nib.p, cx->chunk_st.p, cx->chunk_epoch);
        {
            EventTimer t(cx, "diff_reads", true);
            launch_diff_reads(s, c->descs.p, NCH, c->nib.p, (const uint64_t *)c->refnib.p, c->refnib.p, c->refnib.p + c->ref_stride, c->ref_stride, L,
                              cx->keys_raw.p, cx->vals_raw.p, cx->tile_cur.p, n_tiles, bcap, buckets, (uint32_t)ovf_cap,
                              cx->scal.p + S_M3, c->ckpt.p, cx->chunk_st.p, cx->chunk_epoch, cx->scal.p + S_ERR);
        }
        {
            EventTimer t(cx, "sort_exceptions");
            const bool wide = n_tiles >= 2048;
            Lookback lb{};
            if (wide) lb = next_lookback(cx, tile_scan_blocks(n_tiles));
            launch_tile_layout(s, cx->tile_cur.p, n_tiles, bcap, cx->tile_n.p, cx->tile_scan.p, cx->tile_scanb.p,
                               cx->scal.p + S_M3, cx->scal.p + S_M0, wide ? &lb : nullptr, cx->scal.p + S_ERR);
// ... 66 lines not shown
    cx->emit.ensure(L + 2);
    NodeArrays nd{cx->npos.p, cx->nbases.p, cx->ndelta.p, cx->ncount.p, cx->nminr.p};
    launch_tile_count(s, cx->keys_raw.p, cx->vals_raw.p, cx->tile_n.p, cx->tile_scan.p, cx->bucket_cap, n_tiles,
                      cx->alive.p, cx->tile_nn.p, cx->tile_nr.p);
    {
        const bool wide = n_tiles >= 2048;
        Lookback lb{};
        if (wide) lb = next_lookback(cx, tile_scan_blocks(n_tiles));
        launch_tile_offsets(s, cx->tile_nn.p, cx->tile_nr.p, n_tiles, cx->tile_noff.p, cx->tile_roff.p,
                            cx->scal.p + S_NNODES, cx->scal.p + S_NRUNS, cx->scal.p + S_BEST, S_NLQ + 1 - S_BEST,
                            wide ? &lb : nullptr, cx->scal.p + S_ERR);
    }
    launch_tile_write(s, cx->keys_raw.p, cx->vals_raw.p, cx->tile_n.p, cx->tile_scan.p, cx->bucket_cap, cx->tile_noff.p,
                      cx->tile_roff.p, n_tiles, cx->alive.p, L, nd, cx->nrec.p, cx->node_off.p, cx->run_start.p,
                      c->reads.p, c->tile_rd_off.p, c->tile_rd.p, cx->cov.p, c->refnib.p, cx->emit.p,
                      (long long *)cx->tile_gain.p, cx->scal.p + S_DEEP , cx->deep_min,
                      cx->pflag.p);
    n_runs = std::min<uint32_t>(T, L);
    n_nodes = T;
    if (cx->trace) n_nodes = d2h(cx, cx->scal.p + S_NNODES, 1)[0];
}

GraphPtrs graph_ptrs(np2_ctx *cx, np2_contig *c) {
    NodeArrays nd{cx->npos.p, cx->nbases.p, cx->ndelta.p, cx->ncount.p, cx->nminr.p};
    return GraphPtrs{c->refnib.p, cx->node_off.p, nd, cx->cov.p, c->L, cx->nrec.p, cx->scal.p + S_DEEP, cx->pflag.p};
}

void trace_graph(np2_ctx *cx, np2_contig *c, int pass, uint32_t n_nodes) {
    if (!cx->trace) return;
    const uint32_t L = c->L;
    auto off = d2h(cx, cx->node_off.p, (size_t)L + 1);
    auto nb = d2h(cx, cx->nbases.p, n_nodes);
    auto ndl = d2h(cx, cx->ndelta.p, n_nodes);
    auto nc = d2h(cx, cx->ncount.p, n_nodes);
    auto cov = d2h(cx, cx->cov.p, (size_t)L);
    auto rn = d2h(cx, c->refnib.p, (size_t)(L + 1) / 2);
    auto code = [&](uint32_t p) -> unsigned { return (rn[p >> 1] >> (4 * (p & 1))) & 7; };
    std::vector<uint32_t> goff(L + 1, 0), gcount;
    std::vector<uint16_t> gbases, gdelta;
    for (uint32_t p = 0; p < L; ++p) {
        uint16_t b, d;
        if (p >= 2)
            b = (uint16_t)((code(p - 2) << 8) | (code(p - 1) << 4) | code(p)), d = 0;
        else if (p == 1)
            b = (uint16_t)(0x0F00 | (code(0) << 4) | code(1)), d = 1;
        else
            b = (uint16_t)(0x4FF0 | code(0)), d = 0;
        uint32_t e0 = 0;
        for (uint32_t i = off[p]; i < off[p + 1]; ++i)
            if (node_delta3(nb[i], ndl[i]) == 0) e0 += nc[i];
        gbases.push_back(b);
        gdelta.push_back(d);
        gcount.push_back((uint32_t)cov[p] - e0);
        for (uint32_t i = off[p]; i < off[p + 1]; ++i) {
            gbases.push_back(nb[i]);
            gdelta.push_back(ndl[i]);
            gcount.push_back(nc[i]);
        }
        goff[p + 1] = (uint32_t)gcount.size();
    }
    trace_put(cx, pass, "graph.off", goff);
    trace_put(cx, pass, "graph.bases", gbases);
    trace_put(cx, pass, "graph.delta", gdelta);
    trace_put(cx, pass, "graph.count", gcount);
}

struct CnsBounds {
    uint32_t M_cap, lq_cap, n_words;
};
CnsBounds cns_buffers(np2_ctx *cx, np2_contig *c, uint32_t n_nodes, uint32_t n_runs, uint32_t T) {
    const uint32_t L = c->L;
    if ((uint64_t)L + T + 2 >= 0xFFFFFFF0ull) throw Np2Error(NP2_E_NOMEM, "consensus bound exceeds 32 bits");
    const uint32_t M_cap = L + T + 2;
    cx->eoff.ensure(L + 2);
    cx->cns_pos.ensure(M_cap + 2);
    cx->cns_base.ensure(M_cap + 2);
    cx->cns_cls.ensure(M_cap + 2);
    cx->lq_kind.ensure(M_cap + 2);
    cx->lq_next.ensure(M_cap + 2);
    cx->lq_nothead.ensure(M_cap + 2);
    cx->rflag.ensure(M_cap + 2);
    cx->rstart.ensure(M_cap + 2);
    cx->rend.ensure(M_cap + 2);
    cx->ridx.ensure(M_cap + 2);
    cx->raw_start.ensure(M_cap + 2);
    cx->raw_end.ensure(M_cap + 2);
    cx->headflag.ensure(M_cap + 2);
    cx->hidx.ensure(M_cap + 2);
    cx->lq_start.ensure(M_cap + 2);
    cx->lq_end.ensure(M_cap + 2);
    cx->tmp.ensure(prim_temp_bytes((size_t)M_cap + 2));
    const uint32_t lq_cap = (uint32_t)std::min<uint64_t>(2ull * n_nodes + n_runs + 2, M_cap);
    const uint32_t n_words = (M_cap + 31) / 32;
    cx->lq_list.ensure((size_t)lq_cap + 2);
    cx->hbits.ensure((size_t)n_words + 2);
    return CnsBounds{M_cap, lq_cap, n_words};
}
void lq_regions_issue(np2_ctx *cx, const CnsBounds &b, const uint32_t *M_p, const uint32_t *n_lq) {
    hipStream_t s = cx->stream;
    EventTimer t(cx, "lq_regions");
    launch_lq_scan(s, cx->cns_pos.p, cx->cns_base.p, cx->cns_cls.p, M_p, cx->lq_list.p, n_lq, b.lq_cap, cx->lq_kind.p,
                   cx->lq_next.p, cx->lq_nothead.p, cx->hbits.p, b.n_words + 1, cx->rstart.p, cx->rend.p);
    launch_scan_lb_popc(s, next_lookback(cx, scan_lb_blocks((size_t)b.n_words + 1)), cx->hbits.p, cx->ridx.p, b.n_words,
                        cx->scal.p + S_ERR);
    launch_scatter_regions(s, cx->hbits.p, b.n_words, cx->ridx.p, cx->rstart.p, cx->rend.p, cx->raw_start.p,
                           cx->raw_end.p, cx->scal.p + S_NRAW);
    launch_lq_merge_scan_lb(s, next_lookback(cx, lq_merge_lb_blocks()), cx->raw_start.p, cx->raw_end.p, cx->scal.p + S_NRAW, b.M_cap,
                            cx->headflag.p, cx->hidx.p, cx->scal.p + S_ERR);
    launch_lq_merge_write(s, cx->raw_start.p, cx->raw_end.p, cx->scal.p + S_NRAW, cx->headflag.p, cx->hidx.p,
                          cx->lq_start.p, cx->lq_end.p, cx->scal.p + S_NREG);
}

void consensus_and_regions_issue(np2_ctx *cx, np2_contig *c, uint32_t n_nodes, uint32_t n_runs, uint32_t T) {
    hipStream_t s = cx->stream;
    const uint32_t L = c->L;
    const CnsBounds cb = cns_buffers(cx, c, n_nodes, n_runs, T);
    const uint32_t M_cap = cb.M_cap, lq_cap = cb.lq_cap;
    GraphPtrs gp = graph_ptrs(cx, c);
    cx->n0_besti.ensure(L + 2);
    cx->run_gain.ensure((size_t)n_runs + 2);
    cx->run_flag.ensure((size_t)n_runs + 2);
    cx->emit.ensure(L + 2);
    cx->bt_path.ensure((size_t)M_cap + 2);
    cx->lqc.ensure((size_t)n_runs + 4);
    cx->lqoff.ensure((size_t)n_runs + 4);
    const uint32_t *const n_lq = cx->lqoff.p + n_runs;
    const uint32_t *M_p = cx->eoff.p + L;
    {
        EventTimer t(cx, "dp_backtrack");
        cx->dp_list.ensure((size_t)n_runs + 2);
        uint32_t *const dp_list = cx->dp_list.p, *const n_dp_list = cx->scal.p + S_NDPLIST;
        launch_dp_short(s, gp, c->refnib.p, cx->run_start.p, cx->scal.p + S_NRUNS, n_runs, cx->run_end.p, cx->run_gain.p,
                        cx->emit.p, cx->scal.p + S_PATHBEGIN, cx->bt_path.p, dp_list, n_dp_list);
        launch_dp_long(s, gp, cx->run_start.p, n_runs, cx->nrec.p, cx->nscore.p, cx->nbesti.p, cx->n0_besti.p,
                       cx->run_end.p, (int64_t *)(cx->scal.p + S_LAST0), cx->run_gain.p, cx->emit.p,
                       cx->scal.p + S_PATHBEGIN, cx->bt_path.p, cx->run_flag.p, dp_list, n_dp_list);
        launch_dp_finish(s, gp, cx->run_start.p, cx->scal.p + S_NRUNS, cx->nscore.p, cx->nbesti.p, cx->n0_besti.p,
                         (const int64_t *)(cx->scal.p + S_LAST0), (unsigned long long *)(cx->scal.p + S_GAIN0),
                         cx->scal.p + S_DUP , cx->scal.p + S_BEST,
                         cx->run_gain.p, (const long long *)cx->tile_gain.p,
                         (c->L + TILE - 1) >> TILE_SHIFT, cx->emit.p, cx->scal.p + S_PATHBEGIN, cx->bt_path.p);
        exclusive_total(cx, cx->emit.p, cx->eoff.p, (size_t)L + 1);
        launch_bt_write(s, gp, cx->run_start.p, cx->scal.p + S_NRUNS, n_runs, cx->emit.p, cx->eoff.p, cx->bt_path.p,
                        cx->cns_pos.p, cx->cns_base.p, cx->cns_cls.p, cx->lq_nothead.p, cx->lqc.p);
        exclusive_total(cx, cx->lqc.p, cx->lqoff.p, (size_t)n_runs + 1);
        launch_lq_list(s, gp, cx->run_start.p, cx->scal.p + S_NRUNS, n_runs, cx->emit.p, cx->eoff.p, cx->bt_path.p,
                       cx->lqoff.p, lq_cap, cx->lq_list.p, cx->scal.p + S_ERR);
        launch_default_tail(s, gp, cx->scal.p + S_BEST, M_p, cx->cns_base.p, cx->cns_cls.p, cx->lq_list.p,
                            cx->lqoff.p + n_runs, lq_cap, cx->scal.p + S_ERR);
    }
    lq_regions_issue(cx, cb, M_p, n_lq);
}

bool front_can_fuse(np2_ctx *cx) {
    return !cx->hooks.front_unfused && cx->bucket_cap != 0 && cx->pidx_valid;
}
void pass_front_fused_issue(np2_ctx *cx, np2_contig *c, uint32_t T) {
    hipStream_t s = cx->stream;
    const uint32_t L = c->L;
    const uint32_t n_tiles = (L + TILE - 1) >> TILE_SHIFT;
    const CnsBounds cb = cns_buffers(cx, c, T, std::min<uint32_t>(T, L), T);
    cx->pf_slots.ensure(pf_slot_entries(n_tiles, T));
    cx->pf_bad.ensure((size_t)n_tiles + 2);
    cx->pf_bad2.ensure((size_t)n_tiles + 2);
    const np2_ctx::Hooks &hk = cx->hooks;
    const uint32_t cap_lim = hk.has_pf_cap ? hk.pf_cap : PF_CAP, cap_big = hk.has_pf_cap_big ? hk.pf_cap_big : PF_CAP_BIG,
                   halo_lim = (hk.has_pf_halo ? hk.pf_halo : PF_HALO) & ~15u, cov_max = hk.has_pf_cov_max ? hk.pf_cov_max : PF_COV_MAX;
    PfTile a{cx->keys_raw.p, cx->vals_raw.p, cx->tile_n.p, cx->tile_scan.p, cx->tile_pidx.p, cx->alive.p, c->reads.p,
             c->tile_rd_off.p, c->tile_rd.p, c->refnib.p, cx->pf_slots.p, cx->tile_nn.p, cx->tile_nr.p,
             (long long *)cx->tile_gain.p, cx->scal.p + S_PF, cx->scal.p + S_NBAD, cx->pf_bad.p, cx->scal.p + S_NBAD2, cx->pf_bad2.p,
             (long long *)(cx->scal.p + S_PFEND0), (unsigned long long *)(cx->scal.p + S_PFGAIN0), nullptr, L, n_tiles, cx->bucket_cap,
             cap_lim, cap_big, halo_lim, std::min(cov_max, cx->deep_min), cx->pf_big ? 1u : 0u};
    uint32_t *const M_p = cx->eoff.p + L;
    uint32_t *const n_lq = cx->scal.p + S_NRUNS;
    const bool prof = cx->hooks.pf_prof && tl_recorder() == nullptr;
    if (prof) {
        cx->pf_prof.ensure((size_t)n_tiles * 8 + 8);
        zero32(cx, cx->pf_prof.p, (size_t)n_tiles * 8, 8);
        a.prof = (unsigned long long *)cx->pf_prof.p;
    }
    {
        EventTimer t(cx, "pass_front");
        launch_pf_tile(s, a);
        if (prof) {
            auto st = d2h(cx, cx->pf_prof.p, (size_t)n_tiles * 8);
            double sum[8] = {0}, mx[8] = {0};
            size_t cnt = 0;
            for (uint32_t t = 0; t < n_tiles; ++t) {
                const uint64_t *q = st.data() + (size_t)t * 8;
                if (!q[7] || !q[0]) continue;
                ++cnt;
                for (int i = 1; i < 8; ++i) {
                    const double d = (double)(q[i] - q[i - 1]);
// ... 1456 lines not shown
```

### nextpolish2_amd/csrc/np2_kernels.hip

```cpp
#include "np2_common.hpp"
#include "np2_kernels.hpp"
#include "np2_blockscan.hpp"
#include "np2_nib128.hpp"
#include "../../include/np2.h"

namespace np2 {

__device__ __forceinline__ uint8_t ref_code(const uint8_t *__restrict__ refnib, uint32_t p) {
    return (refnib[p >> 1] >> (4 * (p & 1))) & 7;
}

__device__ __forceinline__ void k_encode_ref(const uint32_t np2_bid, const uint32_t np2_nb, const uint8_t *__restrict__ read0, uint32_t L, uint8_t *__restrict__ refnib,
                             uint32_t nbytes_total, uint32_t stride, uint32_t *__restrict__ err) {
    uint32_t i = np2_bid * blockDim.x + threadIdx.x;
    if (i >= nbytes_total) return;
    uint32_t c0 = 2 * i, c1 = 2 * i + 1;
    uint8_t b = c0 < L ? read0[i] : 0;
    uint8_t hi = c0 < L ? (b >> 4) : 0, lo = c1 < L ? (b & 15) : 0;
    if ((c0 < L && c0 != 0 && (hi & 8)) || (c1 < L && (lo & 8))) atomicOr(err, 1u);
    if (c0 < L && (hi & 7) == 7) atomicOr(err, 1u);
    if (c1 < L && (lo & 7) == 7) atomicOr(err, 1u);
    refnib[i] = (uint8_t)((hi & 7) | ((lo & 7) << 4));
    const uint8_t nx = c1 + 1 < L ? (uint8_t)((read0[i + 1] >> 4) & 7) : (uint8_t)0;
    refnib[stride + i] = (uint8_t)(((hi & 7) << 4) | (lo & 7));
    refnib[2 * (size_t)stride + i] = (uint8_t)(((lo & 7) << 4) | nx);
}

__device__ __forceinline__ void k_post(const uint32_t np2_bid, const uint32_t np2_nb, uint32_t *__restrict__ scal, uint32_t n_scal, uint32_t *__restrict__ mbox, uint32_t seq,
                       uint32_t *__restrict__ dst0, const uint32_t *__restrict__ src0, uint32_t *__restrict__ dst1,
                       const uint32_t *__restrict__ src1, uint32_t *__restrict__ dst2, const uint32_t *__restrict__ src2,
                       uint32_t *__restrict__ dst3, const uint32_t *__restrict__ src3,
                       const uint32_t *__restrict__ ends_of, uint32_t *__restrict__ ends_dst) {
    if (threadIdx.x == 0) {
        if (dst0) *dst0 = *src0;
        if (dst1) *dst1 = *src1;
        if (dst2) *dst2 = *src2;
        if (dst3) *dst3 = *src3;
        if (ends_of) {
            const uint32_t n = *dst0;
            ends_dst[0] = n ? ends_of[0] : 0u;
            ends_dst[1] = n ? ends_of[n - 1] : 0u;
        }
    }
    __threadfence();
    if (threadIdx.x < n_scal)
        mbox[1 + threadIdx.x] = __hip_atomic_load(&scal[threadIdx.x], __ATOMIC_RELAXED, __HIP_MEMORY_SCOPE_AGENT);
    __threadfence_system();
    if (threadIdx.x == 0) __hip_atomic_store(&mbox[0], seq, __ATOMIC_RELEASE, __HIP_MEMORY_SCOPE_SYSTEM);
}
__device__ __forceinline__ void k_fill(const uint32_t np2_bid, const uint32_t np2_nb, uint8_t *__restrict__ p, uint64_t n, uint32_t v4) {
    const uint64_t o = ((uint64_t)np2_bid * 256 + threadIdx.x) * 16;
    if (o >= n) return;
    if ((((uintptr_t)p) & 15) == 0 && o + 16 <= n) {
        *reinterpret_cast<uint4 *>(p + o) = make_uint4(v4, v4, v4, v4);
    } else {
        for (uint64_t i = o; i < min(o + 16, n); ++i) p[i] = (uint8_t)v4;
    }
}
__device__ __forceinline__ void k_copy(const uint32_t np2_bid, const uint32_t np2_nb, uint8_t *__restrict__ dst, const uint8_t *__restrict__ src, uint64_t n) {
    const uint64_t o = ((uint64_t)np2_bid * 256 + threadIdx.x) * 16;
    if (o >= n) return;
    const uintptr_t al = ((uintptr_t)dst) | ((uintptr_t)src);
    if ((al & 15) == 0 && o + 16 <= n) {
        *reinterpret_cast<uint4 *>(dst + o) = *reinterpret_cast<const uint4 *>(src + o);
    } else if ((al & 3) == 0 && o + 16 <= n) {
#pragma unroll
        for (uint32_t q = 0; q < 4; ++q)
            *reinterpret_cast<uint32_t *>(dst + o + 4 * q) = *reinterpret_cast<const uint32_t *>(src + o + 4 * q);
    } else {
        for (uint64_t i = o; i < min(o + 16, n); ++i) dst[i] = src[i];
    }
}
__device__ __forceinline__ void k_copy_len(const uint32_t np2_bid, const uint32_t np2_nb, uint8_t *__restrict__ dst, const uint8_t *__restrict__ src,
                                           const uint32_t *__restrict__ n_dev, uint32_t elem, uint64_t cap) {
    k_copy(np2_bid, np2_nb, dst, src, min((uint64_t)*n_dev * elem, cap));
}
__device__ __forceinline__ void k_copy_counted(const uint32_t np2_bid, const uint32_t np2_nb, uint32_t *__restrict__ dst, const uint32_t *__restrict__ src,
                                               const uint32_t *__restrict__ n_dev, uint32_t cap, uint32_t words_per) {
    const uint32_t n = (uint32_t)min((uint64_t)*n_dev * words_per, (uint64_t)cap);
    const bool wide = ((((uintptr_t)dst) | ((uintptr_t)src)) & 15) == 0;
    for (uint64_t o = ((uint64_t)np2_bid * 256 + threadIdx.x) * 4; o < n; o += (uint64_t)np2_nb * 256 * 4) {
        if (wide && o + 4 <= n) {
            *reinterpret_cast<uint4 *>(dst + o) = *reinterpret_cast<const uint4 *>(src + o);
        } else {
            for (uint64_t i = o; i < min(o + 4, (uint64_t)n); ++i) dst[i] = src[i];
        }
    }
}
__device__ __forceinline__ void k_init_alive(const uint32_t np2_bid, const uint32_t np2_nb, const np2_read_t *__restrict__ reads, uint32_t R, uint8_t *__restrict__ alive) {
    uint32_t r = np2_bid * blockDim.x + threadIdx.x;
    if (r < R) alive[r] = (reads[r].flags & NP2_READ_DROPPED) ? 0 : 1;
}
__device__ __forceinline__ void k_kill_flagged(const uint32_t np2_bid, const uint32_t np2_nb, const uint8_t *__restrict__ flag, uint32_t n, uint8_t *__restrict__ alive) {
    uint32_t i = np2_bid * blockDim.x + threadIdx.x;
    if (i < n && flag[i]) alive[i] = 0;
}
__device__ __forceinline__ void k_kill_reads(const uint32_t np2_bid, const uint32_t np2_nb, const uint32_t *__restrict__ ids, uint32_t n, uint8_t *__restrict__ alive) {
    uint32_t i = np2_bid * blockDim.x + threadIdx.x;
    if (i < n) alive[ids[i]] = 0;
}
__device__ __forceinline__ void k_revive_reads(const uint32_t np2_bid, const uint32_t np2_nb, const uint32_t *__restrict__ ids, uint32_t n, uint8_t *__restrict__ alive) {
    uint32_t i = np2_bid * blockDim.x + threadIdx.x;
    if (i < n) alive[ids[i]] = 1;
}

struct Graph {
    const uint8_t *refnib;
    const uint32_t *node_off;
    NodeArrays nd;
    const int32_t *cov;
    uint32_t L;
    const uint2 *nrec;
    const uint32_t *deep;
};
__device__ __forceinline__ void n0_key(const Graph &g, uint32_t p, uint16_t &bases, uint16_t &delta) {
    const uint8_t c = ref_code(g.refnib, p);
    if (p >= 2) {
        bases = (uint16_t)((ref_code(g.refnib, p - 2) << 8) | (ref_code(g.refnib, p - 1) << 4) | c);
        delta = 0;
    } else if (p == 1) {
        bases = (uint16_t)(0x0F00 | (ref_code(g.refnib, 0) << 4) | c);
        delta = 1;
    } else {
        bases = (uint16_t)(0x4FF0 | c);
        delta = 0;
    }
}
__device__ __forceinline__ uint32_t n0_count(const Graph &g, uint32_t p) {
    uint32_t e0 = 0;
    for (uint32_t i = g.node_off[p]; i < g.node_off[p + 1]; ++i)
    {
        const uint2 rc = g.nrec[i];
        if (node_delta3((uint16_t)rc.x, (uint16_t)(rc.x >> 16)) == 0) e0 += rc.y;
    }
// ... 841 lines not shown
#pragma unroll
            for (uint32_t st = 1; st <= 8; ++st) {
                if (resolved) continue;
                const uint32_t w = 8 - st;
                const uint8_t cl = (uint8_t)(c8 >> (8 * w));
                if (cl == CLS_RESET) {
                    kind = LQK_RESET, pp = p + st, resolved = true;
                } else if (cl == CLS_LQ) {
                    kind = LQK_LINK, pp = p + st, resolved = true;
                } else if (st > 4) {
                    const uint32_t w1 = w + 1 <= 7 ? w + 1 : 7, w2 = w + 2 <= 7 ? w + 2 : 7;
                    if (ps[w1] != ps[w2] && (uint8_t)(b8 >> (8 * w1)) != (uint8_t)(b8 >> (8 * w2)))
                        kind = LQK_CLOSE, pp = p + st, resolved = true;
                }
            }
            if (!resolved) pp = p + 9;
        }
        for (; !resolved && pp < M; ++pp) {
            const uint32_t ii = M - 1 - pp;
            const uint8_t cl = cns_cls[ii];
            if (cl == CLS_RESET) {
                kind = LQK_RESET;
                break;
            }
            if (cl == CLS_LQ) {
                kind = LQK_LINK;
                break;
            }
            if (pp - p > 4) {
                const uint32_t i1 = ii + 1, i2 = ii + 2;
                if (cns_pos[i1] != cns_pos[i2] && cns_base[i1] != cns_base[i2]) {
                    kind = LQK_CLOSE;
                    break;
                }
            }
        }
        lq_kind[p] = kind;
        lq_next[p] = pp;
        if (kind == LQK_LINK) lq_nothead[pp] = 1;
    }
}

__device__ __forceinline__ void k_lq_region(const uint32_t np2_bid, const uint32_t np2_nb, const uint32_t *__restrict__ cns_pos, const uint8_t *__restrict__ cns_base,
                            const uint32_t *__restrict__ M_p, const uint32_t *__restrict__ lq_list,
                            const uint32_t *__restrict__ n_lq_p, uint32_t lq_cap,
                            const uint8_t *__restrict__ lq_kind, const uint32_t *__restrict__ lq_next,
                            const uint8_t *__restrict__ lq_nothead, uint32_t *__restrict__ hbits,
                            uint32_t *__restrict__ rstart, uint32_t *__restrict__ rend) {
    const uint32_t M = *M_p, n_lq = min(*n_lq_p, lq_cap);
    for (uint32_t j = np2_bid * blockDim.x + threadIdx.x; j < n_lq; j += np2_nb * blockDim.x) {
        const uint32_t p = M - 1 - lq_list[j];
        if (lq_nothead[p]) continue;
        uint32_t q = p;
        while (lq_kind[q] == LQK_LINK) q = lq_next[q];
        if (lq_kind[q] != LQK_CLOSE) continue;
        const uint32_t pe = lq_next[q];
        const uint32_t lq_e = pe - 2;
        uint32_t lq_s = p > 2 ? p - 2 : 1;
#define CP(x) cns_pos[M - 1 - (x)]
#define CB(x) cns_base[M - 1 - (x)]
        for (;;) {
            const uint32_t i = M - 1 - lq_s;
            if (lq_s <= 1) break;
            if (lq_s >= 9 && i + 8 < M) {
                uint32_t ps[9];
                uint8_t bs[9];
                __builtin_memcpy(ps, cns_pos + i, 36);
                __builtin_memcpy(bs, cns_base + i, 9);
                uint32_t k = 0;
                while (k < 8 && (ps[k + 1] == ps[k] || bs[k + 1] == bs[k])) ++k;
                lq_s -= k;
                if (k < 8) break;
            } else {
                if (CP(lq_s - 1) == CP(lq_s) || CB(lq_s - 1) == CB(lq_s)) --lq_s; else break;
            }
        }
        rend[p] = CP(lq_s);
        rstart[p] = CP(lq_e);
#undef CP
#undef CB
        atomicOr(&hbits[p >> 5], 1u << (p & 31));
    }
}
__device__ __forceinline__ void k_lq_bits_count(const uint32_t np2_bid, const uint32_t np2_nb, const uint32_t *__restrict__ hbits, uint32_t n_words,
                                uint32_t *__restrict__ wcnt) {
    const uint32_t w = np2_bid * blockDim.x + threadIdx.x;
    if (w <= n_words) wcnt[w] = w < n_words ? (uint32_t)__builtin_popcount(hbits[w]) : 0u;
}
__device__ __forceinline__ void k_scatter_regions(const uint32_t np2_bid, const uint32_t np2_nb, const uint32_t *__restrict__ hbits, uint32_t n_words,
                                  const uint32_t *__restrict__ woff, const uint32_t *__restrict__ rstart,
                                  const uint32_t *__restrict__ rend, uint32_t *__restrict__ raw_start,
                                  uint32_t *__restrict__ raw_end, uint32_t *__restrict__ n_raw) {
    const uint32_t w = np2_bid * blockDim.x + threadIdx.x;
    if (w == 0) *n_raw = woff[n_words];
    if (w >= n_words) return;
    uint32_t bits = hbits[w], k = woff[w];
    for (; bits; bits &= bits - 1, ++k) {
        const uint32_t p = (w << 5) + (uint32_t)__builtin_ctz(bits);
        raw_start[k] = rstart[p];
        raw_end[k] = rend[p];
    }
}

__device__ __forceinline__ void k_lq_merge_flag(const uint32_t np2_bid, const uint32_t np2_nb, const uint32_t *__restrict__ raw_start, const uint32_t *__restrict__ raw_end,
                                const uint32_t *__restrict__ n_raw, uint32_t *__restrict__ headflag) {
    const uint32_t n = *n_raw;
    for (uint32_t j = np2_bid * blockDim.x + threadIdx.x; j < n; j += np2_nb * blockDim.x)
        headflag[j] = !(j >= 1 && raw_end[j] >= raw_start[j - 1]);
}
__device__ __forceinline__ void k_lq_merge_scan(const uint32_t np2_bid, const uint32_t np2_nb, const uint32_t *__restrict__ raw_start, const uint32_t *__restrict__ raw_end,
                                                const uint32_t *__restrict__ n_raw, uint32_t n_host, uint32_t *__restrict__ headflag,
                                                uint32_t *__restrict__ hidx) {
    __shared__ uint32_t sh[16];
    const uint32_t n = min(*n_raw, n_host);
    block_scan_array<OpAdd>(
        n, sh, [&](uint32_t j) { return (j >= 1 && raw_end[j] >= raw_start[j - 1]) ? 0u : 1u; },
        [&](uint32_t j, uint32_t pre, uint32_t v) {
            hidx[j] = pre;
            headflag[j] = v;
        });
}
__device__ __forceinline__ void k_lq_merge_write(const uint32_t np2_bid, const uint32_t np2_nb, const uint32_t *__restrict__ raw_start, const uint32_t *__restrict__ raw_end,
                                 const uint32_t *__restrict__ n_raw, const uint32_t *__restrict__ headflag,
                                 const uint32_t *__restrict__ hidx, uint32_t *__restrict__ lq_start,
                                 uint32_t *__restrict__ lq_end, uint32_t *__restrict__ n_reg) {
    const uint32_t n = *n_raw;
    for (uint32_t j = np2_bid * blockDim.x + threadIdx.x; j < n; j += np2_nb * blockDim.x) {
        if (headflag[j]) {
            uint32_t l = j;
            while (l + 1 < n && !headflag[l + 1]) ++l;
            lq_end[hidx[j]] = raw_end[j];
            lq_start[hidx[j]] = raw_start[l];
        }
        if (j == n - 1) *n_reg = hidx[j] + headflag[j];
    }
}

__device__ __forceinline__ uint32_t count_ge_desc(const uint32_t *a, uint32_t n, uint32_t v) {
    uint32_t lo = 0, hi = n;
    while (lo < hi) {
        uint32_t mid = (lo + hi) >> 1;
        if (a[mid] >= v) lo = mid + 1; else hi = mid;
    }
    return lo;
}
__device__ __forceinline__ uint32_t count_gt_desc(const uint32_t *a, uint32_t n, uint32_t v) {
    uint32_t lo = 0, hi = n;
    while (lo < hi) {
        uint32_t mid = (lo + hi) >> 1;
        if (a[mid] > v) lo = mid + 1; else hi = mid;
    }
    return lo;
}

__device__ __forceinline__ void k_read_m(const uint32_t np2_bid, const uint32_t np2_nb, const np2_read_t *__restrict__ reads, uint32_t R, const uint8_t *__restrict__ alive,
                         const uint32_t *__restrict__ lq_start, uint32_t n_reg, int32_t *__restrict__ mval) {
    uint32_t r = np2_bid * blockDim.x + threadIdx.x;
    if (r >= R) return;
    if (!alive[r]) {
        mval[r] = 0x7FFFFFFF;
        return;
    }
    const uint32_t c = count_ge_desc(lq_start, n_reg, reads[r].aln_t_s);
    mval[r] = c ? (int32_t)(c - 1) : 0;
}

__device__ __forceinline__ void k_pair_count(const uint32_t np2_bid, const uint32_t np2_nb, const np2_read_t *__restrict__ reads, uint32_t R, const uint8_t *__restrict__ alive,
                             const uint32_t *__restrict__ lq_start, const uint32_t *__restrict__ lq_end,
                             uint32_t n_reg, const int32_t *__restrict__ smin, uint32_t *__restrict__ pj,
                             uint32_t *__restrict__ pcount, const uint64_t *__restrict__ ck_off,
                             ReadInfo *__restrict__ rinfo) {
    uint32_t r = np2_bid * blockDim.x + threadIdx.x;
    if (r >= R) return;
    uint32_t cnt = 0, j = 0;
    const np2_read_t rd = reads[r];
    if (alive[r]) {
        const uint32_t s = min((uint32_t)smin[r], n_reg - 1);
        const uint32_t ts = rd.aln_t_s, te = rd.aln_t_e;
        if (!(lq_start[s] < ts || lq_end[s] > te)) {
            j = count_gt_desc(lq_end, n_reg, te);
            cnt = s - j + 1;
        }
    }
    pj[r] = j;
    pcount[r] = cnt;
    rinfo[r] = ReadInfo{rd.aln_t_s, rd.n_cols, (uint32_t)(rd.nib_off >> 4), (uint32_t)ck_off[r], rd.aln_t_e, j, cnt, 0u};
}


__global__ void k_yak_insert(const uint64_t *__restrict__ words, const uint64_t *__restrict__ bucket_off,
                             uint32_t n_buckets, uint64_t *__restrict__ table, uint32_t cap_log2,
                             uint32_t *__restrict__ dup_flag, uint32_t gap) {
    const uint32_t b = blockIdx.y;
    if (b >= n_buckets) return;
    const uint64_t n = bucket_off[b + 1] - bucket_off[b] - gap;
    const uint64_t capm = (1ULL << cap_log2) - 1;
    uint64_t *tb = table + ((uint64_t)b << cap_log2);
    for (uint64_t i = (uint64_t)blockIdx.x * blockDim.x + threadIdx.x; i < n; i += (uint64_t)gridDim.x * blockDim.x) {
        const uint64_t w = words[bucket_off[b] + i];
        const uint64_t key = w >> 10;
        uint64_t s = key & capm;
        for (;;) {
            const unsigned long long old = atomicCAS((unsigned long long *)&tb[s], (unsigned long long)YAK_EMPTY,
                                                     (unsigned long long)w);
            if (old == YAK_EMPTY) break;
            if ((old >> 10) == key) {
                atomicOr(dup_flag, 1u);
                break;
            }
            s = (s + 1) & capm;
        }
    }
}

__global__ void k_yak_insert_dup(const uint64_t *__restrict__ words, const uint64_t *__restrict__ bucket_off,
                                 uint32_t n_buckets, uint64_t *__restrict__ table, uint32_t cap_log2,
                                 uint32_t *__restrict__ ord, uint32_t gap) {
    const uint32_t b = blockIdx.y;
    if (b >= n_buckets) return;
// ... 56 lines not shown
                __builtin_memcpy(&x, s + st + 8 * wd, 8);
                uint64_t c = ((x >> 1) ^ (x >> 2)) & 0x0303030303030303ULL;
                c = (c | (c >> 6)) & 0x000F000F000F000FULL;
                c = (c | (c >> 12)) & 0x000000FF000000FFULL;
                c = (c | (c >> 24)) & 0xFFFFULL;
                codes |= c << (16 * wd);
                uint64_t b = (x >> 3) & 0x0101010101010101ULL;
                b = (b | (b >> 7)) & 0x0003000300030003ULL;
                b = (b | (b >> 14)) & 0x0000000F0000000FULL;
                b = (b | (b >> 28)) & 0xFFULL;
                bad |= b << (8 * wd);
            }
            if ((bad & ((1ULL << k) - 1ULL)) == 0) {
                codes &= mask;
                uint64_t rb = __builtin_bitreverse64(codes);
                rb = ((rb >> 1) & 0x5555555555555555ULL) | ((rb & 0x5555555555555555ULL) << 1);
                const uint64_t fw = rb >> (64 - 2 * k), rv = ~codes & mask;
                mn = min(mn, (uint32_t)yak_get(y, yak_hash64(fw < rv ? fw : rv, mask), min_count));
            }
        }
    }
    for (int o = 32; o > 0; o >>= 1) mn = min(mn, (uint32_t)__shfl_xor(mn, o));
    return mn == 0xFFFFFFFFu ? (uint16_t)0 : (uint16_t)mn;
}

__device__ __forceinline__ void k_score_strings(const uint32_t np2_bid, const uint32_t np2_nb, YakDev y, const uint8_t *__restrict__ strs, const uint64_t *__restrict__ off,
                                uint64_t n, uint16_t min_count, uint16_t *__restrict__ out, uint32_t own_strings) {
    const uint64_t w = ((uint64_t)np2_bid * (blockDim.x >> 6)) + (uint32_t)__builtin_amdgcn_readfirstlane((int)(threadIdx.x >> 6));
    if (w >= n) return;
    const uint16_t sc = own_strings ? wave_score_string(y, strs + off[w], (uint32_t)(off[w + 1] - off[w]), min_count)
                                    : wave_score_string_any(y, strs + off[w], (uint32_t)(off[w + 1] - off[w]), min_count);
    if ((threadIdx.x & 63) == 0) out[w] = sc;
}

__device__ __forceinline__ void k_cand_score(const uint32_t np2_bid, const uint32_t np2_nb, YakDev y, const uint32_t *__restrict__ cand_seq_off, const uint64_t *__restrict__ cand_kmer,
                             const uint32_t *__restrict__ n_cand_p, uint16_t min_count,
                             uint16_t *__restrict__ kscore, uint32_t *__restrict__ long_list,
                             uint32_t *__restrict__ n_long) {
    const uint32_t c = np2_bid * blockDim.x + threadIdx.x;
    const bool live = c < *n_cand_p;
    const uint32_t len = live ? cand_seq_off[c + 1] - cand_seq_off[c] : 0u;
    const bool is_long = live && len > y.k;
    const uint64_t m = __ballot(is_long);
    if (m) {
        const uint32_t lane = threadIdx.x & 63, lead = (uint32_t)__builtin_ctzll(m);
        uint32_t base = 0;
        if (lane == lead) base = atomicAdd(n_long, (uint32_t)__builtin_popcountll(m));
        base = __shfl(base, lead);
        if (is_long) long_list[base + (uint32_t)__builtin_popcountll(m & ((1ULL << lane) - 1ULL))] = c;
    }
    if (!live) return;
    uint16_t sc = 0;
    if (!is_long) {
        const uint64_t km = cand_kmer[c];
        if (km != INVALID_KMER) sc = yak_get(y, km, min_count);
    }
    kscore[c] = sc;
}
__device__ __forceinline__ void k_cand_score_long(const uint32_t np2_bid, const uint32_t np2_nb, YakDev y, const uint32_t *__restrict__ cand_seq_off,
                                  const uint8_t *__restrict__ cand_seq, const uint32_t *__restrict__ long_list,
                                  const uint32_t *__restrict__ n_long, uint16_t min_count,
                                  uint16_t *__restrict__ kscore) {
    const uint32_t nl = *n_long;
    for (uint32_t w = (uint32_t)__builtin_amdgcn_readfirstlane((int)((np2_bid * blockDim.x + threadIdx.x) >> 6)); w < nl; w += (np2_nb * blockDim.x) >> 6) {
        const uint32_t c = long_list[w];
        const uint16_t sc = wave_score_string(y, cand_seq + cand_seq_off[c], cand_seq_off[c + 1] - cand_seq_off[c],
                                              min_count);
        if ((threadIdx.x & 63) == 0) kscore[c] = sc;
    }
}

}

namespace np2 {
static inline dim3 grid1(uint64_t n, uint32_t bs = 256) { return dim3((unsigned)((n + bs - 1) / bs)); }

void launch_encode_ref(hipStream_t s, const uint8_t *read0, uint32_t L, uint8_t *refnib, uint32_t nbytes,
                       uint32_t stride, uint32_t *err) {
    NP2_LAUNCH(k_encode_ref, grid1(nbytes), 256, s, read0, L, refnib, nbytes, stride, err);
}
void launch_post(hipStream_t s, uint32_t *scal, uint32_t n_scal, uint32_t *mbox, uint32_t seq, uint32_t *d0,
                 const uint32_t *s0, uint32_t *d1, const uint32_t *s1, uint32_t *d2, const uint32_t *s2, uint32_t *d3,
                 const uint32_t *s3, const uint32_t *ends_of, uint32_t *ends_dst) {
    NP2_LAUNCH(k_post, dim3(1), 64, s, scal, n_scal, mbox, seq, d0, s0, d1, s1, d2, s2, d3, s3, ends_of, ends_dst);
}
void launch_fill(hipStream_t s, uint8_t *p, uint64_t bytes, uint8_t byte) {
    if (bytes) NP2_LAUNCH(k_fill, grid1((bytes + 15) / 16), 256, s, p, bytes, 0x01010101u * byte);
}
void launch_copy(hipStream_t s, uint8_t *dst, const uint8_t *src, uint64_t bytes) {
    if (bytes) NP2_LAUNCH(k_copy, grid1((bytes + 15) / 16), 256, s, dst, src, bytes);
}
void launch_copy_len(hipStream_t s, uint8_t *dst, const uint8_t *src, const uint32_t *n_dev, uint32_t elem, uint64_t cap_bytes) {
    if (cap_bytes) NP2_LAUNCH(k_copy_len, grid1((cap_bytes + 15) / 16), 256, s, dst, src, n_dev, elem, cap_bytes);
}
void launch_copy_counted(hipStream_t s, uint32_t *dst, const uint32_t *src, const uint32_t *n_dev, uint32_t cap, uint32_t words_per) {
    if (cap) NP2_LAUNCH(k_copy_counted, dim3(std::max<uint32_t>(1, std::min<uint32_t>((cap + 1023) / 1024, 2048))), 256, s, dst, src, n_dev, cap, words_per);
}
void launch_init_alive(hipStream_t s, const np2_read_t *reads, uint32_t R, uint8_t *alive) {
    NP2_LAUNCH(k_init_alive, grid1(R), 256, s, reads, R, alive);
}
void launch_kill_flagged(hipStream_t s, const uint8_t *flag, uint32_t n, uint8_t *alive) {
    if (n) NP2_LAUNCH(k_kill_flagged, grid1(n), 256, s, flag, n, alive);
}
void launch_kill_reads(hipStream_t s, const uint32_t *ids, uint32_t n, uint8_t *alive) {
    if (n) NP2_LAUNCH(k_kill_reads, grid1(n), 256, s, ids, n, alive);
}
void launch_revive_reads(hipStream_t s, const uint32_t *ids, uint32_t n, uint8_t *alive) {
    if (n) NP2_LAUNCH(k_revive_reads, grid1(n), 256, s, ids, n, alive);
}
static Graph mk_graph(const GraphPtrs &gp) { return Graph{gp.refnib, gp.node_off, gp.nd, gp.cov, gp.L, gp.nrec, gp.deep}; }

void launch_dp_short(hipStream_t s, const GraphPtrs &gp, const void *refw, const uint32_t *run_start,
                     const uint32_t *n_runs, uint32_t max_runs, uint32_t *run_end, int64_t *run_gain, uint32_t *emit,
                     uint32_t *path_begin, uint64_t *path, uint32_t *dp_list, uint32_t *n_dp_list) {
    if (max_runs)
        NP2_LAUNCH(k_dp_bt_short, dim3(std::min<uint32_t>((max_runs + 63) / 64, DP_GRID_CAP)), 64, s, run_start, n_runs, mk_graph(gp), (const uint32_t *)refw, run_end, run_gain, emit, path_begin, path, dp_list, n_dp_list);
}
void launch_dp_long(hipStream_t s, const GraphPtrs &gp, const uint32_t *run_start, uint32_t max_runs, const uint2 *nrec,
                    int64_t *nscore, uint32_t *nbesti, uint32_t *n0_besti, uint32_t *run_end, int64_t *last_n0_score,
                    int64_t *run_gain, uint32_t *emit, uint32_t *path_begin, uint64_t *path, uint8_t *run_flag,
                    const uint32_t *dp_list, const uint32_t *n_dp_list) {
    if (!max_runs) return;
    NP2_LAUNCH(k_dp_bt_oct, dim3(std::min<uint32_t>((max_runs + 7) / 8, 2048u)), 64, s, run_start, mk_graph(gp), nrec, nscore, nbesti, n0_besti, run_end, last_n0_score, run_gain, emit, path_begin, path, run_flag, dp_list, n_dp_list);
    NP2_LAUNCH(k_dp_bt_long, dim3(std::min<uint32_t>((max_runs + DP_BLOCK - 1) / DP_BLOCK, 512u)), DP_BLOCK, s, run_start, mk_graph(gp), nrec, nscore, nbesti, n0_besti, run_end, last_n0_score, run_gain, emit, path_begin, path, run_flag, dp_list, n_dp_list);
}
void launch_dp_finish(hipStream_t s, const GraphPtrs &gp, const uint32_t *run_start, const uint32_t *n_runs,
                      const int64_t *nscore, const uint32_t *nbesti, const uint32_t *n0_besti, const int64_t *last_n0_score,
                      unsigned long long *total_gain, uint32_t *blocks_done, uint32_t *best_idx, const int64_t *run_gain,
                      const long long *tile_gain, uint32_t n_tiles, uint32_t *emit, uint32_t *path_begin, uint64_t *path) {
    NP2_LAUNCH(k_dp_finish, dim3(64), 256, s, run_gain, n_runs, tile_gain, n_tiles, total_gain, blocks_done, mk_graph(gp), nscore, last_n0_score, run_start, nbesti, n0_besti, best_idx, emit, path_begin, path);
}
static inline dim3 run_grid(uint32_t bound) { return dim3(std::max<uint32_t>(1, std::min<uint32_t>((bound + 256) / 256, 4096))); }
void launch_bt_write(hipStream_t s, const GraphPtrs &gp, const uint32_t *run_start, const uint32_t *n_runs,
                     uint32_t run_bound, const uint32_t *emit, const uint32_t *eoff, const uint64_t *path,
                     uint32_t *cns_pos, uint8_t *cns_base, uint8_t *cns_cls, uint8_t *lq_nothead, uint32_t *lqc) {
    NP2_LAUNCH(k_cns_write, grid1(gp.L), 256, s, gp.refnib, gp.pflag, emit, eoff, gp.L, cns_pos, cns_base, cns_cls, lq_nothead);
    NP2_LAUNCH(k_cns_runs, run_grid(4 * (uint64_t)run_bound > 0xFFFFFFF0ull ? 0xFFFFFFF0u : 4 * run_bound), 256, s, run_start, n_runs, run_bound, gp.node_off, emit, eoff, path, cns_pos, cns_base, cns_cls, lq_nothead, lqc);
}
void launch_lq_list(hipStream_t s, const GraphPtrs &gp, const uint32_t *run_start, const uint32_t *n_runs,
                    uint32_t run_bound, const uint32_t *emit, const uint32_t *eoff, const uint64_t *path,
                    const uint32_t *lqoff, uint32_t cap, uint32_t *lq_list, uint32_t *err) {
    NP2_LAUNCH(k_lq_list, run_grid(run_bound), 256, s, run_start, n_runs, run_bound, gp.node_off, emit, eoff, path, lqoff, cap, lq_list, err);
}
void launch_default_tail(hipStream_t s, const GraphPtrs &gp, const uint32_t *best_idx, const uint32_t *M_p, uint8_t *cns_base,
                         uint8_t *cns_cls, uint32_t *lq_list, uint32_t *n_lq, uint32_t cap, uint32_t *err) {
    NP2_LAUNCH(k_default_tail, 1, 64, s, best_idx, gp.node_off, gp.pflag, gp.L, M_p, cns_base, cns_cls, lq_list, n_lq, cap, err);
}
static inline dim3 lq_grid(uint32_t cap) { return dim3(std::max<uint32_t>(1, std::min<uint32_t>((cap + 2047) / 2048, 2048))); }
void launch_lq_scan(hipStream_t s, const uint32_t *cns_pos, const uint8_t *cns_base, const uint8_t *cns_cls,
                    const uint32_t *M_p, const uint32_t *lq_list, const uint32_t *n_lq, uint32_t lq_cap, uint8_t *lq_kind,
                    uint32_t *lq_next, uint8_t *lq_nothead, uint32_t *hbits, uint32_t n_hwords, uint32_t *rstart, uint32_t *rend) {
    NP2_LAUNCH(k_lq_scan, lq_grid(std::max(lq_cap, n_hwords / 4)), 256, s, cns_pos, cns_base, cns_cls, M_p, lq_list, n_lq, lq_cap, lq_kind, lq_next, lq_nothead, hbits, n_hwords);
    NP2_LAUNCH(k_lq_region, lq_grid(lq_cap), 256, s, cns_pos, cns_base, M_p, lq_list, n_lq, lq_cap, lq_kind, lq_next, lq_nothead, hbits, rstart, rend);
}
void launch_lq_bits_count(hipStream_t s, const uint32_t *hbits, uint32_t n_words, uint32_t *wcnt) {
    NP2_LAUNCH(k_lq_bits_count, grid1((uint64_t)n_words + 1), 256, s, hbits, n_words, wcnt);
}
void launch_scatter_regions(hipStream_t s, const uint32_t *hbits, uint32_t n_words, const uint32_t *woff,
                            const uint32_t *rstart, const uint32_t *rend, uint32_t *raw_start, uint32_t *raw_end,
                            uint32_t *n_raw) {
    NP2_LAUNCH(k_scatter_regions, grid1(std::max<uint32_t>(n_words, 1)), 256, s, hbits, n_words, woff, rstart, rend, raw_start, raw_end, n_raw);
}
void launch_lq_merge_flag(hipStream_t s, const uint32_t *raw_start, const uint32_t *raw_end, const uint32_t *n_raw,
                          uint32_t *headflag) {
    NP2_LAUNCH(k_lq_merge_flag, dim3(256), 256, s, raw_start, raw_end, n_raw, headflag);
}
void launch_lq_merge_scan(hipStream_t s, const uint32_t *raw_start, const uint32_t *raw_end, const uint32_t *n_raw, uint32_t n_host,
                          uint32_t *headflag, uint32_t *hidx) {
    NP2_LAUNCH(k_lq_merge_scan, dim3(1), 1024, s, raw_start, raw_end, n_raw, n_host, headflag, hidx);
}
void launch_lq_merge_write(hipStream_t s, const uint32_t *raw_start, const uint32_t *raw_end, const uint32_t *n_raw,
                           const uint32_t *headflag, const uint32_t *hidx, uint32_t *lq_start, uint32_t *lq_end,
                           uint32_t *n_reg) {
    NP2_LAUNCH(k_lq_merge_write, dim3(256), 256, s, raw_start, raw_end, n_raw, headflag, hidx, lq_start, lq_end, n_reg);
}
void launch_read_m(hipStream_t s, const np2_read_t *reads, uint32_t R, const uint8_t *alive, const uint32_t *lq_start,
                   uint32_t n_reg, int32_t *mval) {
    NP2_LAUNCH(k_read_m, grid1(R), 256, s, reads, R, alive, lq_start, n_reg, mval);
}
void launch_pair_count(hipStream_t s, const np2_read_t *reads, uint32_t R, const uint8_t *alive,
                       const uint32_t *lq_start, const uint32_t *lq_end, uint32_t n_reg, const int32_t *smin,
                       uint32_t *pj, uint32_t *pcount, const uint64_t *ck_off, ReadInfo *rinfo) {
    NP2_LAUNCH(k_pair_count, grid1(R), 256, s, reads, R, alive, lq_start, lq_end, n_reg, smin, pj, pcount, ck_off, rinfo);
}
void launch_yak_insert(hipStream_t s, const uint64_t *words, const uint64_t *bucket_off, uint32_t n_buckets,
                       uint64_t max_bucket, uint64_t *table, uint32_t cap_log2, uint32_t *dup_flag, uint32_t gap) {
    uint32_t gx = (uint32_t)((max_bucket + 255) / 256);
    if (gx == 0) gx = 1;
    if (gx > 64) gx = 64;
    hipLaunchKernelGGL(k_yak_insert, dim3(gx, n_buckets), dim3(256), 0, s, words, bucket_off, n_buckets, table,
                       cap_log2, dup_flag, gap);
}
void launch_yak_insert_dup(hipStream_t s, const uint64_t *words, const uint64_t *bucket_off, uint32_t n_buckets,
                           uint64_t max_bucket, uint64_t *table, uint32_t cap_log2, uint32_t *ord, uint32_t gap) {
    uint32_t gx = (uint32_t)((max_bucket + 255) / 256);
    gx = std::min<uint32_t>(64, std::max<uint32_t>(1, gx));
    hipLaunchKernelGGL(k_yak_insert_dup, dim3(gx, n_buckets), dim3(256), 0, s, words, bucket_off, n_buckets, table,
                       cap_log2, ord, gap);
}
void launch_lookup(hipStream_t s, const YakDev &y, const uint64_t *hashes, uint64_t n, uint16_t min_count,
                   uint16_t *out) {
    if (n) NP2_LAUNCH(k_lookup, grid1(n), 256, s, y, hashes, n, min_count, out);
}
void launch_score_strings(hipStream_t s, const YakDev &y, const uint8_t *strs, const uint64_t *off, uint64_t n,
                          uint16_t min_count, uint16_t *out, bool own_strings) {
    if (n) NP2_LAUNCH(k_score_strings, grid1(n * 64), 256, s, y, strs, off, n, min_count, out, own_strings ? 1u : 0u);
}
void launch_cand_score(hipStream_t s, const YakDev &y, const uint32_t *cand_seq_off, const uint8_t *cand_seq,
                       const uint64_t *cand_kmer, const uint32_t *n_cand_p, uint32_t cand_cap, uint16_t min_count,
                       uint16_t *kscore, uint32_t *long_list, uint32_t *n_long) {
    if (!cand_cap) return;
    NP2_LAUNCH(k_cand_score, grid1(cand_cap), 256, s, y, cand_seq_off, cand_kmer, n_cand_p, min_count, kscore, long_list, n_long);
    NP2_LAUNCH(k_cand_score_long, dim3(std::max<uint32_t>(16, std::min<uint32_t>(1024, cand_cap / 4096))), 256, s, y, cand_seq_off, cand_seq, long_list, n_long, min_count, kscore);
}
}
```

### nextpolish2_amd/csrc/np2_kernels.hpp

```cpp
#pragma once
#include <cstddef>
#include <cstdint>
#include <hip/hip_runtime.h>
#include "../../include/np2.h"
#include "np2_lookback.hpp"
#include "np2_launch.hpp"

namespace np2 {

static constexpr uint32_t TILE_SHIFT = 10;
static constexpr uint32_t TILE = 1u << TILE_SHIFT;
static constexpr uint32_t TILE_CAP = 4096;

static constexpr uint32_t DENSE_COLS = 4096;
struct ChunkDesc {
    uint64_t nib_off;
    uint64_t ckbase;
    uint32_t read, ts;
    uint32_t c0, ncols;
    uint32_t first_chunk;
    uint32_t aln_t_e, nck;
    uint32_t pad0;
    uint32_t pad[4];
};
// ... 13 lines not shown
    uint32_t L;
    const uint2 *nrec;
    const uint32_t *deep;
    const uint8_t *pflag;
};
struct __attribute__((aligned(16))) ReadInfo {
    uint32_t aln_t_s, n_cols;
    uint32_t nib16;
    uint32_t ck_off;
    uint32_t aln_t_e;
    uint32_t pj, pcount;
    uint32_t pad;
};
struct CandPtrs {
    const np2_read_t *reads;
    const uint8_t *nib;
    const uint64_t *ck_off;
    const uint32_t *ckpt;
    const uint32_t *lq_start;
    const uint32_t *lq_end;
    const uint32_t *pj;
    const uint32_t *pcount;
    const uint8_t *alive;
    const ReadInfo *rinfo;
    const uint32_t *tile_rd_off;
    const uint32_t *tile_rd;
    uint32_t n_tiles;
    uint32_t ksize;
    const uint64_t *rec_key;
    const uint32_t *rec_read;
    const uint32_t *tile_n;
    const uint16_t *rec_pidx;
    uint32_t bucket_cap;
    const uint32_t *refnib;
    uint32_t L;
};
struct YakDev {
    const uint64_t *table;
    uint32_t cap_log2;
    uint32_t k;
    const uint32_t *ord;
};
static constexpr uint64_t YAK_EMPTY = ~0ULL;
#if defined(__HIPCC__)
__device__ __forceinline__ uint16_t yak_get(const YakDev &y, uint64_t x, uint16_t min_count) {
    const uint64_t capm = (1ULL << y.cap_log2) - 1;
    const uint64_t *tb = y.table + ((x & 1023) << y.cap_log2);
    const uint64_t key = x >> 10;
    uint64_t s = key & capm;
    if (y.ord) {
        const uint32_t *ob = y.ord + ((x & 1023) << y.cap_log2);
        uint16_t c = 0;
        int64_t at = -1;
        for (;;) {
            const uint64_t w = tb[s];
            if (w == YAK_EMPTY) return c;
            if ((w >> 10) == key && (uint16_t)(w & 1023) >= min_count && (int64_t)ob[s] > at) at = ob[s], c = (uint16_t)(w & 1023);
            s = (s + 1) & capm;
        }
    }
    for (;;) {
        const uint64_t w = tb[s];
        if (w == YAK_EMPTY) return 0;
        if ((w >> 10) == key) {
            const uint16_t c = (uint16_t)(w & 1023);
            return c >= min_count ? c : 0;
        }
        s = (s + 1) & capm;
    }
}
#endif

void launch_encode_ref(hipStream_t s, const uint8_t *read0, uint32_t L, uint8_t *refnib, uint32_t nbytes, uint32_t stride, uint32_t *err);
void launch_chunk_counts(hipStream_t s, const ChunkDesc *descs, uint32_t n_chunks, const uint8_t *nib, uint64_t *chunk_st, uint32_t epoch);
void launch_diff_reads(hipStream_t s, const ChunkDesc *descs, uint32_t n_chunks, const uint8_t *nib, const uint64_t *refw,
                       const uint8_t *refnib, const uint8_t *refeo, uint32_t eo_stride, uint32_t L, uint64_t *keys, uint32_t *vals, uint32_t *tile_cur,
                       uint32_t n_tiles, uint32_t bucket_cap, uint64_t ovf_base, uint32_t ovf_cap, uint32_t *ovf_cnt,
                       uint32_t *ckpt, uint64_t *chunk_st, uint32_t epoch, uint32_t *err);
void launch_post(hipStream_t s, uint32_t *scal, uint32_t n_scal, uint32_t *mbox, uint32_t seq, uint32_t *d0 = nullptr,
                 const uint32_t *s0 = nullptr, uint32_t *d1 = nullptr, const uint32_t *s1 = nullptr, uint32_t *d2 = nullptr,
                 const uint32_t *s2 = nullptr, uint32_t *d3 = nullptr, const uint32_t *s3 = nullptr,
                 const uint32_t *ends_of = nullptr, uint32_t *ends_dst = nullptr);
void launch_fill(hipStream_t s, uint8_t *p, uint64_t bytes, uint8_t byte);
void launch_copy(hipStream_t s, uint8_t *dst, const uint8_t *src, uint64_t bytes);
void launch_copy_len(hipStream_t s, uint8_t *dst, const uint8_t *src, const uint32_t *n_dev, uint32_t elem, uint64_t cap_bytes);
void launch_copy_counted(hipStream_t s, uint32_t *dst, const uint32_t *src, const uint32_t *n_dev, uint32_t cap, uint32_t words_per = 1);
void launch_init_alive(hipStream_t s, const np2_read_t *reads, uint32_t R, uint8_t *alive);
void launch_kill_reads(hipStream_t s, const uint32_t *ids, uint32_t n, uint8_t *alive);
void launch_revive_reads(hipStream_t s, const uint32_t *ids, uint32_t n, uint8_t *alive);
void launch_kill_flagged(hipStream_t s, const uint8_t *flag, uint32_t n, uint8_t *alive);
void launch_dp_short(hipStream_t s, const GraphPtrs &gp, const void *refw, const uint32_t *run_start,
                     const uint32_t *n_runs, uint32_t max_runs, uint32_t *run_end, int64_t *run_gain, uint32_t *emit,
                     uint32_t *path_begin, uint64_t *path, uint32_t *dp_list, uint32_t *n_dp_list);
void launch_dp_long(hipStream_t s, const GraphPtrs &gp, const uint32_t *run_start, uint32_t max_runs, const uint2 *nrec,
                    int64_t *nscore, uint32_t *nbesti, uint32_t *n0_besti, uint32_t *run_end, int64_t *last_n0_score,
                    int64_t *run_gain, uint32_t *emit, uint32_t *path_begin, uint64_t *path, uint8_t *run_flag,
                    const uint32_t *dp_list, const uint32_t *n_dp_list);
void launch_dp_finish(hipStream_t s, const GraphPtrs &gp, const uint32_t *run_start, const uint32_t *n_runs,
                      const int64_t *nscore, const uint32_t *nbesti, const uint32_t *n0_besti, const int64_t *last_n0_score,
                      unsigned long long *total_gain, uint32_t *blocks_done, uint32_t *best_idx, const int64_t *run_gain,
                      const long long *tile_gain, uint32_t n_tiles, uint32_t *emit, uint32_t *path_begin, uint64_t *path);
void launch_bt_write(hipStream_t s, const GraphPtrs &gp, const uint32_t *run_start, const uint32_t *n_runs,
                     uint32_t run_bound, const uint32_t *emit, const uint32_t *eoff, const uint64_t *path,
                     uint32_t *cns_pos, uint8_t *cns_base, uint8_t *cns_cls, uint8_t *lq_nothead, uint32_t *lqc);
void launch_lq_list(hipStream_t s, const GraphPtrs &gp, const uint32_t *run_start, const uint32_t *n_runs,
                    uint32_t run_bound, const uint32_t *emit, const uint32_t *eoff, const uint64_t *path,
                    const uint32_t *lqoff, uint32_t cap, uint32_t *lq_list, uint32_t *err);
void launch_default_tail(hipStream_t s, const GraphPtrs &gp, const uint32_t *best_idx, const uint32_t *M_p, uint8_t *cns_base,
                         uint8_t *cns_cls, uint32_t *lq_list, uint32_t *n_lq, uint32_t cap, uint32_t *err);
void launch_lq_scan(hipStream_t s, const uint32_t *cns_pos, const uint8_t *cns_base, const uint8_t *cns_cls,
                    const uint32_t *M_p, const uint32_t *lq_list, const uint32_t *n_lq, uint32_t lq_cap, uint8_t *lq_kind,
                    uint32_t *lq_next, uint8_t *lq_nothead, uint32_t *hbits, uint32_t n_hwords, uint32_t *rstart, uint32_t *rend);
void launch_lq_merge_scan_lb(hipStream_t s, const Lookback &lb, const uint32_t *raw_start, const uint32_t *raw_end, const uint32_t *n_raw,
                             uint32_t n_host, uint32_t *headflag, uint32_t *hidx, uint32_t *err);
uint32_t lq_merge_lb_blocks();
void launch_lq_merge_scan(hipStream_t s, const uint32_t *raw_start, const uint32_t *raw_end, const uint32_t *n_raw, uint32_t n_host,
                          uint32_t *headflag, uint32_t *hidx);
void launch_scan_lb_popc(hipStream_t s, const Lookback &lb, const uint32_t *bits, uint32_t *out, uint32_t n_words, uint32_t *err);
void launch_lq_bits_count(hipStream_t s, const uint32_t *hbits, uint32_t n_words, uint32_t *wcnt);
void launch_scatter_regions(hipStream_t s, const uint32_t *hbits, uint32_t n_words, const uint32_t *woff,
                            const uint32_t *rstart, const uint32_t *rend, uint32_t *raw_start, uint32_t *raw_end,
                            uint32_t *n_raw);
void launch_lq_merge_flag(hipStream_t s, const uint32_t *raw_start, const uint32_t *raw_end, const uint32_t *n_raw,
                          uint32_t *headflag);
void launch_lq_merge_write(hipStream_t s, const uint32_t *raw_start, const uint32_t *raw_end, const uint32_t *n_raw,
                           const uint32_t *headflag, const uint32_t *hidx, uint32_t *lq_start, uint32_t *lq_end,
                           uint32_t *n_reg);
void launch_read_m(hipStream_t s, const np2_read_t *reads, uint32_t R, const uint8_t *alive, const uint32_t *lq_start,
                   uint32_t n_reg, int32_t *mval);
void launch_yak_insert(hipStream_t s, const uint64_t *words, const uint64_t *bucket_off, uint32_t n_buckets,
                       uint64_t max_bucket, uint64_t *table, uint32_t cap_log2, uint32_t *dup_flag, uint32_t gap = 0);
void launch_yak_insert_dup(hipStream_t s, const uint64_t *words, const uint64_t *bucket_off, uint32_t n_buckets,
                           uint64_t max_bucket, uint64_t *table, uint32_t cap_log2, uint32_t *ord, uint32_t gap = 0);
void launch_lookup(hipStream_t s, const YakDev &y, const uint64_t *hashes, uint64_t n, uint16_t min_count, uint16_t *out);
void launch_score_strings(hipStream_t s, const YakDev &y, const uint8_t *strs, const uint64_t *off, uint64_t n,
                          uint16_t min_count, uint16_t *out, bool own_strings);
void launch_cand_score(hipStream_t s, const YakDev &y, const uint32_t *cand_seq_off, const uint8_t *cand_seq,
                       const uint64_t *cand_kmer, const uint32_t *n_cand_p, uint32_t cand_cap, uint16_t min_count,
                       uint16_t *kscore, uint32_t *long_list, uint32_t *n_long);


void launch_pair_count(hipStream_t s, const np2_read_t *reads, uint32_t R, const uint8_t *alive,
                       const uint32_t *lq_start, const uint32_t *lq_end, uint32_t n_reg, const int32_t *smin,
                       uint32_t *pj, uint32_t *pcount, const uint64_t *ck_off, ReadInfo *rinfo);
void launch_scan_lb_excl(hipStream_t s, const Lookback &lb, const uint32_t *in, uint32_t *out, uint32_t n, bool write_end,
                          uint32_t *err);
uint32_t scan_lb_blocks(uint64_t n);
void launch_scan_small_excl(hipStream_t s, const uint32_t *in, uint32_t *out, uint32_t n, const uint32_t *n_dev,
                            uint32_t *total_out, bool write_end);
void launch_scan_small_incl(hipStream_t s, const int32_t *in, int32_t *out, uint32_t n, const uint32_t *n_dev);
void launch_scan_small_min(hipStream_t s, const int32_t *in, int32_t *out, uint32_t n, const uint32_t *n_dev);
void launch_region_measure(hipStream_t s, const CandPtrs &c, uint32_t n_reg, uint32_t *kept_read, uint32_t *kept_len,
                           uint32_t *kept_col, uint32_t *reg_ncand, uint32_t *reg_bytes, uint32_t *reg_maxlen,
                           uint32_t *blk_sum);
uint32_t cand_offsets_blocks(uint32_t n_reg);
void launch_cand_offsets(hipStream_t s, const uint32_t *blk_sum, uint32_t n_reg, uint32_t *blk_coff, uint32_t *blk_soff,
                         uint32_t *cand_off, uint32_t *reg_soff, uint32_t *n_cand, uint32_t *n_bytes, uint32_t *grow,
                         const Lookback *lb = nullptr, uint32_t *err = nullptr);
void launch_region_write(hipStream_t s, const CandPtrs &c, uint32_t n_reg, const uint32_t *kept_read,
                         const uint32_t *kept_len, const uint32_t *kept_col, const uint32_t *reg_ncand,
                         const uint32_t *reg_bytes, const uint32_t *blk_coff, const uint32_t *blk_soff, uint32_t *cand_off,
                         uint32_t *reg_soff, uint32_t cand_cap, uint32_t seq_cap, uint32_t *cand_order, uint64_t *cand_kmer,
                         uint32_t *cand_seq_off, uint8_t *cand_seq);

uint32_t tile_scan_blocks(uint32_t n_tiles);
void launch_tile_layout(hipStream_t s, uint32_t *tile_cur, uint32_t n_tiles, uint32_t bucket_cap, uint32_t *tile_n,
                        uint32_t *tile_scan, uint32_t *tile_scanb, const uint32_t *ovf_cnt, uint32_t *out,
                        const Lookback *lb = nullptr, uint32_t *err = nullptr);
void launch_tile_sort(hipStream_t s, uint16_t *pidx, const np2_read_t *reads, const uint8_t *nib, const uint32_t *tile_n,
                      uint32_t n_tiles, uint32_t bucket_cap, uint32_t max_tile, uint64_t *keys, uint32_t *vals,
                      uint32_t *err);
void launch_gather_buckets(hipStream_t s, const np2_read_t *reads, const uint8_t *nib, const uint32_t *tile_n,
                           const uint32_t *tile_scanb, uint32_t n_tiles, uint32_t bucket_cap, const uint64_t *bkeys,
                           const uint32_t *bvals, uint64_t *keys, uint32_t *vals);
void launch_gather_spill(hipStream_t s, const np2_read_t *reads, const uint8_t *nib, const uint64_t *okeys,
                         const uint32_t *ovals, uint32_t n, uint64_t *keys, uint32_t *vals);
void launch_tile_count(hipStream_t s, const uint64_t *keys, const uint32_t *vals, const uint32_t *tile_n,
                       const uint32_t *tile_scan, uint32_t bucket_cap, uint32_t n_tiles, const uint8_t *alive,
                       uint32_t *tile_nn, uint32_t *tile_nr);
void launch_tile_offsets(hipStream_t s, const uint32_t *tile_nn, const uint32_t *tile_nr, uint32_t n_tiles,
                         uint32_t *tile_noff, uint32_t *tile_roff, uint32_t *n_nodes, uint32_t *n_runs, uint32_t *reset,
                         uint32_t n_reset, const Lookback *lb = nullptr, uint32_t *err = nullptr,
                         const long long *tile_gain = nullptr, unsigned long long *gain_total = nullptr);
void launch_tile_write(hipStream_t s, const uint64_t *keys, const uint32_t *vals, const uint32_t *tile_n,
                       const uint32_t *tile_scan, uint32_t bucket_cap, const uint32_t *tile_noff, const uint32_t *tile_roff,
                       uint32_t n_tiles, const uint8_t *alive, uint32_t L, NodeArrays nd, uint2 *nrec, uint32_t *node_off,
                       uint32_t *run_start, const np2_read_t *reads, const uint32_t *tile_rd_off, const uint32_t *tile_rd,
                       int32_t *cov, const uint8_t *refnib, uint32_t *emit, long long *tile_gain, uint32_t *deep_flag, uint32_t deep_min,
                       uint8_t *pflag);

static constexpr uint32_t PF_CAP = 960;
static constexpr uint32_t PF_HALO = 64;
static constexpr uint32_t PF_CAP_MID = 2048;
static constexpr uint32_t PF_CAP_BIG = 3584;
static constexpr uint32_t PF_COV_MAX = 8192;
static constexpr uint32_t PF_REDO = 1u;
static constexpr uint32_t PF_NEED_BIG = 2u;
struct PfTile {
    const uint64_t *keys;
    const uint32_t *vals;
    const uint32_t *tile_n, *tile_scan;
    const uint16_t *pidx;
    const uint8_t *alive;
    const np2_read_t *reads;
    const uint32_t *tile_rd_off, *tile_rd;
    const uint8_t *refnib;
    uint16_t *slots;
    uint32_t *tile_cnt, *tile_lq;
    long long *tile_gain;
    uint32_t *flags, *n_bad, *bad_list, *n_bad2, *bad_list2;
    long long *end_rel;
    unsigned long long *gain_total;
    unsigned long long *prof;
    uint32_t L, n_tiles, bucket_cap;
    uint32_t cap_lim, cap_lim_big, halo_lim, cov_max;
    uint32_t big_enabled;
};
uint64_t pf_slot_entries(uint32_t n_tiles, uint64_t T);
void launch_pf_tile(hipStream_t s, const PfTile &a);
void launch_pf_compact(hipStream_t s, uint32_t n_tiles, const uint16_t *slots, const uint32_t *tile_scan, const uint32_t *tile_cnt,
                       const uint32_t *tile_coff, const uint32_t *tile_lqoff, uint32_t *cns_pos, uint8_t *cns_base,
                       uint8_t *cns_cls, uint8_t *lq_nothead, uint32_t *lq_list, uint32_t lq_cap, uint32_t *err, uint32_t *flags,
                       uint32_t *flags_out, uint32_t *n_bad, uint32_t *n_bad2);

struct RegionTables {
    const uint32_t *cand_off;
    const uint32_t *order;
    uint16_t *kscore;
    const uint32_t *seq_off;
    const uint8_t *seq;
    uint32_t n_reg;
};
struct RechPtrs {
    const void *groups;
    const uint32_t *job_off;
    const uint32_t *rech;
    const uint32_t *cand_off;
    const uint32_t *keep_list;
    const uint32_t *seq_off;
    const uint8_t *seq;
    const uint8_t *cns_base;
    uint32_t n_groups;
};
void launch_vote_phase(hipStream_t s, const RegionTables &rt, bool asref, bool use_all, const uint32_t *lq_start,
                       uint32_t own_lo, uint32_t own_hi, uint8_t *reg_lable, uint8_t *grp, uint32_t *ecount, int32_t *ref_w,
                       uint8_t *ref_seen, uint8_t *bad, uint32_t *first_reg, uint32_t *err);
void launch_vote_counts(hipStream_t s, const uint32_t *first_reg, const uint8_t *bad, uint32_t R, uint32_t *out);
void launch_edges_write(hipStream_t s, const RegionTables &rt, const uint8_t *reg_lable, const uint8_t *grp,
                        const uint32_t *ecount, const uint32_t *eoff, uint64_t *ekey, uint32_t *eval);
static constexpr uint32_t EDGE_BAND = 256;
void launch_edges_row(hipStream_t s, const RegionTables &rt, const uint8_t *grp, const uint32_t *ecount, const uint32_t *pj,
                      const uint32_t *pcount, const uint8_t *alive, uint32_t R, uint32_t *band, uint32_t *row_n, uint32_t *ovf);
void launch_band_emit(hipStream_t s, const uint32_t *band, uint32_t R, const uint32_t *row_off, uint64_t *ukey, uint32_t *uw,
                      uint32_t *n_out, uint64_t key_add = 0);
void launch_vote_rows_count(hipStream_t s, const uint32_t *band, const uint32_t *row_n, const uint8_t *bad, bool use_all, uint32_t R,
                            uint32_t *cnt, uint32_t *nokey);
void launch_vote_rows_emit(hipStream_t s, const uint32_t *band, const uint32_t *row_n, const uint8_t *bad, bool use_all,
                           const uint32_t *first_reg, uint32_t R, const uint32_t *off, void *edges, uint32_t *n_out, uint32_t *nokey);
void launch_edge_reduce(hipStream_t s, const uint64_t *ekey, const uint32_t *eval, uint32_t n, uint32_t *flag, uint32_t *wout);
void launch_edge_compact(hipStream_t s, const uint64_t *ekey, const uint32_t *flag, const uint32_t *idx, const uint32_t *wout,
                         uint32_t n, uint64_t *ukey, uint32_t *uw, uint32_t *n_out);
void launch_seed(hipStream_t s, const RegionTables &rt, int32_t max_indel_len, uint8_t *reg_lable, uint32_t *seed_cand,
                 uint32_t *keep_n, uint32_t *keep_list, uint16_t *keep_ks, uint32_t *err);
uint32_t region_lb_blocks(uint32_t n_reg);
void launch_splice_find(hipStream_t s, const uint32_t *cns_pos, const uint32_t *M_p, const uint32_t *lq_start,
                        const uint32_t *lq_end, const uint8_t *reg_lable, uint8_t lable, uint32_t n_reg, uint32_t *idx_s,
                        uint32_t *idx_e, uint32_t *stuck);
void launch_splice_plan(hipStream_t s, const Lookback &lb, const uint8_t *reg_lable, uint8_t lable, uint32_t n_reg,
                        const uint32_t *stuck, const uint32_t *idx_s, const uint32_t *idx_e, const uint32_t *seed_cand,
                        const uint32_t *seq_off, uint32_t *ap_g, uint32_t *ap_s, uint32_t *ap_e, int32_t *ap_delta,
                        int32_t *ap_shift_incl, uint32_t *n_ap, const uint32_t *M_in, uint32_t *M_out, uint32_t out_cap , uint32_t *err);
void launch_splice_write(hipStream_t s, const uint32_t *in_pos, const uint8_t *in_base, const uint32_t *M_p, uint32_t M_cap,
                         const uint32_t *ap_g, const uint32_t *ap_s, const uint32_t *ap_e, const int32_t *ap_delta,
                         const int32_t *ap_shift_incl, const uint32_t *n_ap, uint32_t max_ap, const uint32_t *lq_start,
                         const uint32_t *seed_cand, const uint32_t *seq_off, const uint8_t *seq, uint32_t *out_pos,
                         uint8_t *out_base);
void launch_shard_bounds(hipStream_t s, const uint32_t *cns_pos, const uint32_t *M_p, const uint32_t *t, uint32_t *out);
void launch_rech_list(hipStream_t s, const Lookback &lb, const uint8_t *reg_lable, uint32_t n_reg, uint32_t *rech,
                      uint32_t *n_rech, unsigned long long *blob_bound, uint32_t *err);
void launch_rech_groups(hipStream_t s, const Lookback &lb, const uint32_t *rech, const uint32_t *n_rech_p, uint32_t max_rech,
                        const uint32_t *cns_pos, const uint32_t *M_p, const uint32_t *lq_start, const uint32_t *lq_end,
                        const uint32_t *keep_n, uint32_t ksize, const uint32_t *reg_maxlen, void *tmp_groups,
                        uint32_t *head_jobs, void *groups, uint32_t *job_off, uint32_t *n_groups, uint32_t *n_jobs,
                        unsigned long long *blob_bound, uint32_t *err);
size_t rech_group_bytes();
void launch_rech_job_len(hipStream_t s, const RechPtrs &p, uint32_t n_jobs, uint32_t *len);
void launch_rech_job_build(hipStream_t s, const RechPtrs &p, uint32_t n_jobs, const uint32_t *soff32, uint64_t *soff64,
                           uint8_t *blob);
void launch_rech_apply(hipStream_t s, const RechPtrs &p, const uint16_t *score, uint16_t *keep_ks);
void launch_rech_select(hipStream_t s, const uint32_t *rech, const uint32_t *n_rech_p, uint32_t max_rech,
                        const uint32_t *cand_off, const uint32_t *keep_n, const uint32_t *keep_list, const uint16_t *keep_ks,
                        const uint32_t *order, bool first_yak, uint8_t *reg_lable, uint32_t *seed_cand);
void launch_rech_relabel(hipStream_t s, uint8_t *reg_lable, uint32_t n_reg);

struct FrontOp {
    uint32_t col0, q0, t0;
    uint32_t len_type;
};
struct FrontRec {
    uint32_t pos, n_ops;
    uint64_t op_off;
    uint64_t seq_off;
    uint64_t out_off;
    uint32_t n_cols;
    uint32_t pad;
};
struct FrontOut {
    uint32_t aln_t_s, aln_t_e, n_cols, pad;
};
void launch_columnarise(hipStream_t s, const FrontRec *recs, uint32_t n_recs, const FrontOp *ops, const uint8_t *ref,
                        const uint8_t *seq4, uint8_t *nib, FrontOut *out);
void launch_pack_ref(hipStream_t s, const uint8_t *ref, uint32_t L, uint8_t *dst);

size_t prim_temp_bytes(size_t n);
int prim_sort_pairs_u64_u32(hipStream_t s, void *tmp, size_t tmp_bytes, const uint64_t *kin, uint64_t *kout,
                            const uint32_t *vin, uint32_t *vout, size_t n, unsigned end_bit);
int prim_exclusive_sum_u32(hipStream_t s, void *tmp, size_t tmp_bytes, const uint32_t *in, uint32_t *out, size_t n);
int prim_inclusive_sum_i32(hipStream_t s, void *tmp, size_t tmp_bytes, const int32_t *in, int32_t *out, size_t n);
int prim_inclusive_min_i32(hipStream_t s, void *tmp, size_t tmp_bytes, const int32_t *in, int32_t *out, size_t n);

}
```

### nextpolish2_amd/csrc/np2_regions.hip

```cpp
#include "np2_common.hpp"
#include "np2_kernels.hpp"
#include "np2_blockscan.hpp"
#include "np2_lookback.hpp"

namespace np2 {

static constexpr uint8_t LB_TEMP = 0x01, LB_SUCC = 0x80, LB_HETE = 0x40, LB_RECH = 0x20;

__device__ __forceinline__ uint32_t min_support(uint32_t n) { return n >= 9 ? 3u : (n >= 6 ? 2u : 1u); }

struct SubWave {
    uint32_t base;
    bool half;
    __device__ __forceinline__ uint64_t ballot(bool p) const {
        const uint64_t b = __ballot(p);
        return half ? (b >> base) & 0xFFFFFFFFull : b;
    }
    template <class T> __device__ __forceinline__ T shfl(T v, uint32_t j) const { return __shfl(v, (int)(base + j)); }
};

struct WaveStats {
    uint64_t eqmask;
    uint32_t stat;
    uint32_t c;
// ... 869 lines not shown
                                                      const uint32_t *__restrict__ n_rech_p,
                                                      const uint32_t *__restrict__ head_jobs,
                                                      const RechGroup *__restrict__ tmp_groups,
                                                      RechGroup *__restrict__ groups, uint32_t *__restrict__ job_off,
                                                      uint32_t *__restrict__ n_groups, uint32_t *__restrict__ n_jobs,
                                                      uint32_t *__restrict__ err) {
    __shared__ uint32_t sh[8];
    const uint32_t bid = lb_block_id(lb, sh);
    const uint32_t n_rech = *n_rech_p;
    uint32_t hj[LB_REG_ITEMS], hs = 0, js = 0;
#pragma unroll
    for (uint32_t k = 0; k < LB_REG_ITEMS; ++k) {
        const uint32_t e = (bid * 256 + threadIdx.x) * LB_REG_ITEMS + k;
        hj[k] = e < n_rech ? head_jobs[e] : 0u;
        hs += hj[k] ? 1u : 0u;
        js += hj[k] ? hj[k] - 1u : 0u;
    }
    uint32_t nh, nj, pre_h, pre_j;
    uint32_t lh = block_excl_scan<OpAdd, 4>(hs, sh, nh);
    uint32_t lj = block_excl_scan<OpAdd, 4>(js, sh, nj);
    lb_exclusive2(lb, bid, nh, nj, sh, err, pre_h, pre_j);
    if (pre_j + nj < pre_j) atomicOr(err, 128u);
#pragma unroll
    for (uint32_t k = 0; k < LB_REG_ITEMS; ++k) {
        if (!hj[k]) continue;
        const uint32_t e = (bid * 256 + threadIdx.x) * LB_REG_ITEMS + k;
        groups[pre_h + lh] = tmp_groups[e];
        job_off[pre_h + lh] = pre_j + lj;
        ++lh;
        lj += hj[k] - 1u;
    }
    if (bid == n_blocks - 1 && threadIdx.x == 0) {
        *n_groups = pre_h + nh;
        *n_jobs = pre_j + nj;
        job_off[pre_h + nh] = pre_j + nj;
    }
}

struct RechCtx {
    const RechGroup *groups;
    const uint32_t *job_off;
    const uint32_t *rech;
    const uint32_t *cand_off;
    const uint32_t *keep_list;
    const uint32_t *seq_off;
    const uint8_t *seq;
    const uint8_t *cns_base;
    uint32_t n_groups;
};
__device__ __forceinline__ uint32_t job_group(const RechCtx &cx, uint32_t job) {
    uint32_t lo = 0, hi = cx.n_groups;
    while (lo < hi) {
        const uint32_t mid = (lo + hi) >> 1;
        if (cx.job_off[mid] <= job) lo = mid + 1; else hi = mid;
    }
    return lo - 1;
}
template <bool WRITE> __device__ uint32_t rech_string(const RechCtx &cx, uint32_t job, uint8_t *__restrict__ out) {
    const uint32_t gi = job_group(cx, job);
    const RechGroup &G = cx.groups[gi];
    uint32_t rem = job - cx.job_off[gi];
    uint32_t pick[6];
    for (uint32_t x = G.n; x-- > 0;) {
        pick[x] = rem % G.lens[x];
        rem /= G.lens[x];
    }
    uint32_t o = 0;
    for (uint32_t i = G.sl; i < G.el; ++i, ++o)
        if (WRITE) out[o] = cx.cns_base[i];
    for (uint32_t x = 0; x < G.n; ++x) {
        const uint32_t g = cx.rech[G.first + x];
        const uint32_t c = cx.keep_list[cx.cand_off[g] + pick[x]];
        const uint32_t so = cx.seq_off[c], len = cx.seq_off[c + 1] - so;
        for (uint32_t t = 0; t < len; ++t, ++o)
            if (WRITE) out[o] = cx.seq[so + t];
        if (x + 1 < G.n)
            for (uint32_t i = G.bs[x]; i < G.be[x]; ++i, ++o)
                if (WRITE) out[o] = cx.cns_base[i];
    }
    for (uint32_t i = G.sr; i < G.er; ++i, ++o)
        if (WRITE) out[o] = cx.cns_base[i];
    return o;
}
__device__ __forceinline__ void k_rech_job_len(const uint32_t np2_bid, const uint32_t np2_nb, RechCtx cx, uint32_t n_jobs, uint32_t *__restrict__ len) {
    uint32_t j = np2_bid * blockDim.x + threadIdx.x;
    if (j < n_jobs) len[j] = rech_string<false>(cx, j, nullptr);
}
__device__ __forceinline__ void k_rech_job_build(const uint32_t np2_bid, const uint32_t np2_nb, RechCtx cx, uint32_t n_jobs, const uint64_t *__restrict__ soff,
                                 uint8_t *__restrict__ blob) {
    uint32_t j = np2_bid * blockDim.x + threadIdx.x;
    if (j < n_jobs) rech_string<true>(cx, j, blob + soff[j]);
}
__device__ __forceinline__ void k_u32_to_u64_off(const uint32_t np2_bid, const uint32_t np2_nb, const uint32_t *__restrict__ in, uint32_t n, uint64_t *__restrict__ out) {
    uint32_t i = np2_bid * blockDim.x + threadIdx.x;
    if (i < n) out[i] = in[i];
}

__device__ __forceinline__ void k_rech_apply(const uint32_t np2_bid, const uint32_t np2_nb, RechCtx cx, const uint16_t *__restrict__ score, uint16_t *__restrict__ keep_ks) {
    uint32_t gi = np2_bid * blockDim.x + threadIdx.x;
    if (gi >= cx.n_groups) return;
    const RechGroup &G = cx.groups[gi];
    const uint32_t j0 = cx.job_off[gi];
    if (G.n == 1) {
        const uint32_t g = cx.rech[G.first];
        for (uint32_t t = 0; t < G.lens[0]; ++t) keep_ks[cx.cand_off[g] + t] = score[j0 + t];
        return;
    }
    for (uint32_t x = 0; x < G.n; ++x) {
        const uint32_t g = cx.rech[G.first + x];
        for (uint32_t t = 0; t < G.lens[x]; ++t) keep_ks[cx.cand_off[g] + t] = 0;
    }
    for (uint32_t j = 0; j < G.njobs; ++j) {
        const uint16_t ks = score[j0 + j];
        if (!ks) continue;
        uint32_t rem = j;
        for (uint32_t x = G.n; x-- > 0;) {
            const uint32_t p = rem % G.lens[x];
            rem /= G.lens[x];
            keep_ks[cx.cand_off[cx.rech[G.first + x]] + p] = ks;
        }
    }
}

__device__ __forceinline__ void k_rech_select(const uint32_t np2_bid, const uint32_t np2_nb, const uint32_t *__restrict__ rech, const uint32_t *__restrict__ n_rech_p,
                              const uint32_t *__restrict__ cand_off, const uint32_t *__restrict__ keep_n,
                              const uint32_t *__restrict__ keep_list, const uint16_t *__restrict__ keep_ks,
                              const uint32_t *__restrict__ order, uint32_t first_yak, uint8_t *__restrict__ reg_lable,
                              uint32_t *__restrict__ seed_cand) {
    uint32_t e = np2_bid * blockDim.x + threadIdx.x;
    if (e >= *n_rech_p) return;
    const uint32_t g = rech[e], c0 = cand_off[g], n = keep_n[g];
    uint32_t c = 0, valid = 0;
    for (uint32_t p = 0; p < n; ++p)
        if (keep_ks[c0 + p] != 0) {
            if (c == 0 || order[keep_list[c0 + p]] == 0) c = p + 1;
            ++valid;
        }
    if (valid > 1) reg_lable[g] |= LB_TEMP;
    if (c != 0) {
        seed_cand[g] = keep_list[c0 + c - 1];
    } else if (first_yak) {
        uint32_t i = 0;
        for (uint32_t p = 0; p < n; ++p)
            if (order[keep_list[c0 + p]] == 0) {
                i = p;
                break;
            }
        seed_cand[g] = keep_list[c0 + i];
    }
}
__device__ __forceinline__ void k_rech_relabel(const uint32_t np2_bid, const uint32_t np2_nb, uint8_t *__restrict__ reg_lable, uint32_t n_reg) {
    uint32_t g = np2_bid * blockDim.x + threadIdx.x;
    if (g >= n_reg) return;
    const uint8_t l = reg_lable[g];
    if (!(l & LB_RECH)) return;
    reg_lable[g] = (l & LB_TEMP) ? (uint8_t)(l ^ LB_TEMP) : (uint8_t)(l ^ LB_RECH);
}

__device__ __forceinline__ void k_vote_counts(const uint32_t np2_bid, const uint32_t np2_nb, const uint32_t *__restrict__ first_reg, const uint8_t *__restrict__ bad,
                                                      uint32_t R, uint32_t *__restrict__ out) {
    __shared__ uint32_t sk[16], sb[16];
    uint32_t nk = 0, nb = 0;
    for (uint32_t r = threadIdx.x; r < R; r += 1024) {
        nk += first_reg[r] != 0xFFFFFFFFu ? 1u : 0u;
        nb += bad[r] ? 1u : 0u;
    }
    for (int o = 32; o > 0; o >>= 1) {
        nk += __shfl_xor(nk, o);
        nb += __shfl_xor(nb, o);
    }
    if ((threadIdx.x & 63) == 0) {
        sk[threadIdx.x >> 6] = nk;
        sb[threadIdx.x >> 6] = nb;
    }
    __syncthreads();
    if (threadIdx.x == 0) {
        uint32_t a = 0, b = 0;
        for (int i = 0; i < 16; ++i) {
            a += sk[i];
            b += sb[i];
        }
        out[0] = a;
        out[1] = b;
    }
}

static inline dim3 g1(uint64_t n, uint32_t bs = 256) { return dim3((unsigned)((n + bs - 1) / bs)); }

void launch_vote_phase(hipStream_t s, const RegionTables &rt, bool asref, bool use_all, const uint32_t *lq_start,
                       uint32_t own_lo, uint32_t own_hi, uint8_t *reg_lable, uint8_t *grp, uint32_t *ecount, int32_t *ref_w,
                       uint8_t *ref_seen, uint8_t *bad, uint32_t *first_reg, uint32_t *err) {
    if (rt.n_reg)
        NP2_LAUNCH(k_vote_phase, g1((uint64_t)((rt.n_reg + 1) / 2) * 64), 256, s, rt, asref ? 1u : 0u, use_all ? 1u : 0u, lq_start, own_lo, own_hi, reg_lable, grp, ecount, ref_w, ref_seen, bad, first_reg, err);
}
void launch_vote_counts(hipStream_t s, const uint32_t *first_reg, const uint8_t *bad, uint32_t R, uint32_t *out) {
    NP2_LAUNCH(k_vote_counts, dim3(1), 1024, s, first_reg, bad, R, out);
}
void launch_edges_write(hipStream_t s, const RegionTables &rt, const uint8_t *reg_lable, const uint8_t *grp,
                        const uint32_t *ecount, const uint32_t *eoff, uint64_t *ekey, uint32_t *eval) {
    if (rt.n_reg)
        NP2_LAUNCH(k_edges_write, g1((uint64_t)rt.n_reg * 64), 256, s, rt, reg_lable, grp, ecount, eoff, ekey, eval);
}
void launch_edges_row(hipStream_t s, const RegionTables &rt, const uint8_t *grp, const uint32_t *ecount, const uint32_t *pj,
                      const uint32_t *pcount, const uint8_t *alive, uint32_t R, uint32_t *band, uint32_t *row_n, uint32_t *ovf) {
    if (R) NP2_LAUNCH(k_edges_row, g1((uint64_t)R * 64), 256, s, rt, grp, ecount, pj, pcount, alive, R, band, row_n, ovf);
}
void launch_vote_rows_count(hipStream_t s, const uint32_t *band, const uint32_t *row_n, const uint8_t *bad, bool use_all, uint32_t R,
                            uint32_t *cnt, uint32_t *nokey) {
    if (R) NP2_LAUNCH(k_vote_rows_count, g1((uint64_t)R * 64), 256, s, band, row_n, bad, use_all ? 1u : 0u, R, cnt, nokey);
}
void launch_vote_rows_emit(hipStream_t s, const uint32_t *band, const uint32_t *row_n, const uint8_t *bad, bool use_all,
                           const uint32_t *first_reg, uint32_t R, const uint32_t *off, void *edges, uint32_t *n_out, uint32_t *nokey) {
    if (R) NP2_LAUNCH(k_vote_rows_emit, g1((uint64_t)R * 64), 256, s, band, row_n, bad, use_all ? 1u : 0u, first_reg, R, off, (uint2 *)edges, n_out, nokey);
}
void launch_band_emit(hipStream_t s, const uint32_t *band, uint32_t R, const uint32_t *row_off, uint64_t *ukey, uint32_t *uw,
                      uint32_t *n_out, uint64_t key_add) {
    if (R) NP2_LAUNCH(k_band_emit, g1((uint64_t)R * 64), 256, s, band, R, row_off, ukey, uw, n_out, key_add);
}
void launch_edge_reduce(hipStream_t s, const uint64_t *ekey, const uint32_t *eval, uint32_t n, uint32_t *flag,
                        uint32_t *wout) {
    if (n) NP2_LAUNCH(k_edge_reduce, g1(n), 256, s, ekey, eval, n, flag, wout);
}
void launch_edge_compact(hipStream_t s, const uint64_t *ekey, const uint32_t *flag, const uint32_t *idx,
                         const uint32_t *wout, uint32_t n, uint64_t *ukey, uint32_t *uw, uint32_t *n_out) {
    if (n) NP2_LAUNCH(k_edge_compact, g1(n), 256, s, ekey, flag, idx, wout, n, ukey, uw, n_out);
}
void launch_seed(hipStream_t s, const RegionTables &rt, int32_t max_indel_len, uint8_t *reg_lable, uint32_t *seed_cand,
                 uint32_t *keep_n, uint32_t *keep_list, uint16_t *keep_ks, uint32_t *err) {
    if (rt.n_reg)
        NP2_LAUNCH(k_seed, g1((uint64_t)((rt.n_reg + 1) / 2) * 64), 256, s, rt, max_indel_len, reg_lable, seed_cand, keep_n, keep_list, keep_ks, err);
}
uint32_t region_lb_blocks(uint32_t n_reg) { return (n_reg + 256 * LB_REG_ITEMS - 1) / (256 * LB_REG_ITEMS); }
void launch_splice_find(hipStream_t s, const uint32_t *cns_pos, const uint32_t *M_p, const uint32_t *lq_start,
                        const uint32_t *lq_end, const uint8_t *reg_lable, uint8_t lable, uint32_t n_reg,
                        uint32_t *idx_s, uint32_t *idx_e, uint32_t *stuck) {
    NP2_LAUNCH(k_splice_find, g1(n_reg), 256, s, cns_pos, M_p, lq_start, lq_end, reg_lable, lable, n_reg, idx_s, idx_e, stuck);
}
void launch_splice_plan(hipStream_t s, const Lookback &lb, const uint8_t *reg_lable, uint8_t lable, uint32_t n_reg,
                        const uint32_t *stuck, const uint32_t *idx_s, const uint32_t *idx_e, const uint32_t *seed_cand,
                        const uint32_t *seq_off, uint32_t *ap_g, uint32_t *ap_s, uint32_t *ap_e, int32_t *ap_delta,
                        int32_t *ap_shift_incl, uint32_t *n_ap, const uint32_t *M_in, uint32_t *M_out, uint32_t out_cap, uint32_t *err) {
    const uint32_t nb = region_lb_blocks(n_reg);
    NP2_LAUNCH(k_splice_plan, dim3(nb), 256, s, lb, nb, reg_lable, lable, n_reg, stuck, idx_s, idx_e, seed_cand, seq_off, ap_g, ap_s, ap_e, ap_delta, ap_shift_incl, n_ap, M_in, M_out, out_cap, err);
}
void launch_splice_write(hipStream_t s, const uint32_t *in_pos, const uint8_t *in_base, const uint32_t *M_p, uint32_t M_cap,
                         const uint32_t *ap_g, const uint32_t *ap_s, const uint32_t *ap_e, const int32_t *ap_delta,
                         const int32_t *ap_shift_incl, const uint32_t *n_ap, uint32_t max_ap, const uint32_t *lq_start,
                         const uint32_t *seed_cand, const uint32_t *seq_off, const uint8_t *seq, uint32_t *out_pos,
                         uint8_t *out_base) {
    NP2_LAUNCH(k_splice_bases, dim3((M_cap + SPLICE_SPAN - 1) / SPLICE_SPAN), 256, s, in_pos, in_base, M_p, ap_s, ap_e, ap_shift_incl, n_ap, out_pos, out_base);
    if (max_ap)
        NP2_LAUNCH(k_splice_seeds, g1((uint64_t)max_ap * 8, 256), 256, s, ap_g, ap_s, ap_delta, ap_shift_incl, n_ap, lq_start, seed_cand, seq_off, seq, out_pos, out_base);
}
void launch_shard_bounds(hipStream_t s, const uint32_t *cns_pos, const uint32_t *M_p, const uint32_t *t, uint32_t *out) {
    NP2_LAUNCH(k_shard_bounds, dim3(1), 64, s, cns_pos, M_p, t[0], t[1], t[2], t[3], t[4], t[5], out);
}
void launch_rech_list(hipStream_t s, const Lookback &lb, const uint8_t *reg_lable, uint32_t n_reg, uint32_t *rech,
                      uint32_t *n_rech, unsigned long long *blob_bound, uint32_t *err) {
    const uint32_t nb = region_lb_blocks(n_reg);
    NP2_LAUNCH(k_rech_list, dim3(nb), 256, s, lb, nb, reg_lable, n_reg, rech, n_rech, blob_bound, err);
}
void launch_rech_groups(hipStream_t s, const Lookback &lb, const uint32_t *rech, const uint32_t *n_rech_p, uint32_t max_rech,
                        const uint32_t *cns_pos, const uint32_t *M_p, const uint32_t *lq_start, const uint32_t *lq_end,
                        const uint32_t *keep_n, uint32_t ksize, const uint32_t *reg_maxlen, void *tmp_groups,
                        uint32_t *head_jobs, void *groups, uint32_t *job_off, uint32_t *n_groups, uint32_t *n_jobs,
                        unsigned long long *blob_bound, uint32_t *err) {
    NP2_LAUNCH(k_rech_groups, dim3((max_rech + 255) / 256), 256, s, rech, n_rech_p, cns_pos, M_p, lq_start, lq_end, keep_n, ksize, reg_maxlen, (RechGroup *)tmp_groups, head_jobs, blob_bound, err);
    const uint32_t nb = region_lb_blocks(max_rech);
    NP2_LAUNCH(k_rech_compact, dim3(nb), 256, s, lb, nb, n_rech_p, head_jobs, (const RechGroup *)tmp_groups, (RechGroup *)groups, job_off, n_groups, n_jobs, err);
}
size_t rech_group_bytes() { return sizeof(RechGroup); }
static RechCtx mk_rech(const RechPtrs &p) {
    return RechCtx{(const RechGroup *)p.groups, p.job_off, p.rech, p.cand_off, p.keep_list, p.seq_off, p.seq,
                   p.cns_base, p.n_groups};
}
void launch_rech_job_len(hipStream_t s, const RechPtrs &p, uint32_t n_jobs, uint32_t *len) {
    if (n_jobs) NP2_LAUNCH(k_rech_job_len, g1(n_jobs, 64), 64, s, mk_rech(p), n_jobs, len);
}
void launch_rech_job_build(hipStream_t s, const RechPtrs &p, uint32_t n_jobs, const uint32_t *soff32, uint64_t *soff64,
                           uint8_t *blob) {
    if (!n_jobs) return;
    NP2_LAUNCH(k_u32_to_u64_off, g1(n_jobs + 1), 256, s, soff32, n_jobs + 1, soff64);
    NP2_LAUNCH(k_rech_job_build, g1(n_jobs, 64), 64, s, mk_rech(p), n_jobs, soff64, blob);
}
void launch_rech_apply(hipStream_t s, const RechPtrs &p, const uint16_t *score, uint16_t *keep_ks) {
    if (p.n_groups) NP2_LAUNCH(k_rech_apply, g1(p.n_groups, 64), 64, s, mk_rech(p), score, keep_ks);
}
void launch_rech_select(hipStream_t s, const uint32_t *rech, const uint32_t *n_rech_p, uint32_t max_rech,
                        const uint32_t *cand_off, const uint32_t *keep_n, const uint32_t *keep_list,
                        const uint16_t *keep_ks, const uint32_t *order, bool first_yak, uint8_t *reg_lable,
                        uint32_t *seed_cand) {
    if (max_rech)
        NP2_LAUNCH(k_rech_select, g1(max_rech, 64), 64, s, rech, n_rech_p, cand_off, keep_n, keep_list, keep_ks, order, first_yak ? 1u : 0u, reg_lable, seed_cand);
}
void launch_rech_relabel(hipStream_t s, uint8_t *reg_lable, uint32_t n_reg) {
    NP2_LAUNCH(k_rech_relabel, g1(n_reg), 256, s, reg_lable, n_reg);
}

}
```

Measured before the change: 4288.

## Fuse small pipeline kernels and fold flush completion into final post kernel

Several chains of small kernels are merged: the popcount scan and region scatter become one decoupled-lookback kernel, the merge scan and merge write are combined, and recheck length, offset scan, u64 conversion and build collapse into one lookback-scan kernel. Apply and select are also fused, and two fills are merged into one launch. The batch flush can attach its completion signal to the final k_post launches through a device counter instead of issuing a separate done kernel. Together these cut launch count and per-launch latency in a launch-bound pipeline, at the cost of more complex kernels and a counter-based completion protocol.

```diff
diff --git a/nextpolish2_amd/csrc/np2_batch.cpp b/nextpolish2_amd/csrc/np2_batch.cpp
--- a/nextpolish2_amd/csrc/np2_batch.cpp
+++ b/nextpolish2_amd/csrc/np2_batch.cpp
@@ -53,6 +53,7 @@
 
     uint32_t *done_host = nullptr, *done_dev = nullptr;
     uint32_t done_seq = 0;
+    uint32_t *done_cnt = nullptr;
     std::atomic<uint32_t> issued_seq{0};
     std::atomic<uint32_t> done_pub{0};
     std::atomic<bool> spinner{false};
@@ -103,6 +104,8 @@
     double t_issued = t_begin;
     std::vector<size_t> idx(n, 0);
     hipStream_t s = b->stream;
+    bool carried = false;
+    uint32_t carried_seq = 0;
     Recorder *saved = tl_recorder();
     tl_recorder() = nullptr;
     try {
@@ -145,6 +148,25 @@
                 }
                 if (!best || defer < best_defer || (defer == best_defer && c > best_n)) best = kd, best_n = c, best_defer = defer;
             }
+            if (strcmp(best->name, "k_post") == 0) {
+                int heads = 0;
+                bool last = true;
+                for (int i = 0; i < n && last; ++i) {
+                    auto &q = b->recs[i].q;
+                    if (idx[i] >= q.size()) continue;
+                    last = q[idx[i]].kd == best && idx[i] + 1 == q.size();
+                    ++heads;
+                }
+                if (last && heads <= best->max_batch) {
+                    carried_seq = ++b->done_seq;
+                    for (int i = 0; i < n; ++i) {
+                        auto &r = b->recs[i];
+                        if (idx[i] < r.q.size())
+                            (void)post_carry_done(best->name, r.arena.data() + r.q[idx[i]].arg_off, b->done_dev, carried_seq, b->done_cnt, (uint32_t)heads);
+                    }
+                    carried = true;
+                }
+            }
             uint32_t grids[MAXB];
             const void *args[MAXB];
             int m = 0;
@@ -181,8 +203,8 @@
             issue();
         }
         HIPCHK(hipGetLastError());
-        const uint32_t seq = ++b->done_seq;
-        NP2_LAUNCH(k_flush_done, 1, 64, s, b->done_dev, seq);
+        const uint32_t seq = carried ? carried_seq : ++b->done_seq;
+        if (!carried) NP2_LAUNCH(k_flush_done, 1, 64, s, b->done_dev, seq);
         t_issued = now_ms();
         b->issued_seq.store(seq, std::memory_order_release);
     } catch (const std::exception &ex) {
@@ -334,6 +356,9 @@
         HIPCHK(hipHostMalloc((void **)&b->done_host, 256 * (size_t)(n_slots + 1), hipHostMallocMapped | hipHostMallocCoherent));
         memset(b->done_host, 0, 256 * (size_t)(n_slots + 1));
         HIPCHK(hipHostGetDevicePointer((void **)&b->done_dev, b->done_host, 0));
+        HIPCHK(hipMalloc((void **)&b->done_cnt, 64));
+        HIPCHK(hipMemset(b->done_cnt, 0, 64));
+        HIPCHK(hipStreamSynchronize(nullptr));
         b->recs.resize(n_slots);
         b->jobs.resize(n_slots);
         for (int i = 0; i < n_slots; ++i) {
@@ -368,6 +393,7 @@
         (void)hipEventDestroy(e.second);
     }
     if (b->done_host) (void)hipHostFree(b->done_host);
+    if (b->done_cnt) (void)hipFree(b->done_cnt);
     if (b->stream) (void)hipStreamDestroy(b->stream);
     delete b;
 }
diff --git a/nextpolish2_amd/csrc/np2_cand.hip b/nextpolish2_amd/csrc/np2_cand.hip
--- a/nextpolish2_amd/csrc/np2_cand.hip
+++ b/nextpolish2_amd/csrc/np2_cand.hip
@@ -81,6 +81,37 @@
 __device__ __forceinline__ void k_scan_lb_popc(const uint32_t np2_bid, const uint32_t np2_nb, Lookback lb, uint32_t n_blocks, const uint32_t *__restrict__ in,
                                                uint32_t *__restrict__ out, uint32_t n, bool write_end, uint32_t *__restrict__ err) {
     scan_lb_excl_body<true>(np2_bid, np2_nb, lb, n_blocks, in, out, n, write_end, err);
+}
+
+__device__ __forceinline__ void k_lq_scatter_lb(const uint32_t np2_bid, const uint32_t np2_nb, Lookback lb, uint32_t n_blocks, const uint32_t *__restrict__ hbits,
+                                                uint32_t n_words, const uint32_t *__restrict__ rstart, const uint32_t *__restrict__ rend,
+                                                uint32_t *__restrict__ raw_start, uint32_t *__restrict__ raw_end, uint32_t *__restrict__ n_raw,
+                                                uint32_t *__restrict__ err) {
+    __shared__ uint32_t sh[16];
+    const uint32_t bid = lb_block_id(lb, sh);
+    const uint32_t i0 = bid * SCAN_LB_BLOCK + threadIdx.x * SCAN_LB_ITEMS;
+    uint32_t w[SCAN_LB_ITEMS], sum = 0;
+    if ((((uintptr_t)hbits) & 15) == 0 && i0 + SCAN_LB_ITEMS <= n_words) {
+        const uint4 a = *reinterpret_cast<const uint4 *>(hbits + i0), b = *reinterpret_cast<const uint4 *>(hbits + i0 + 4);
+        w[0] = a.x, w[1] = a.y, w[2] = a.z, w[3] = a.w, w[4] = b.x, w[5] = b.y, w[6] = b.z, w[7] = b.w;
+    } else {
+#pragma unroll
+        for (uint32_t k = 0; k < SCAN_LB_ITEMS; ++k) w[k] = i0 + k < n_words ? hbits[i0 + k] : 0u;
+    }
+#pragma unroll
+    for (uint32_t k = 0; k < SCAN_LB_ITEMS; ++k) sum += (uint32_t)__builtin_popcount(w[k]);
+    uint32_t total, pre, dummy;
+    uint32_t run = block_excl_scan<OpAdd, 16>(sum, sh, total);
+    lb_exclusive2(lb, bid, total, 0u, sh, err, pre, dummy);
+    run += pre;
+#pragma unroll
+    for (uint32_t k = 0; k < SCAN_LB_ITEMS; ++k)
+        for (uint32_t bits = w[k]; bits; bits &= bits - 1, ++run) {
+            const uint32_t p = ((i0 + k) << 5) + (uint32_t)__builtin_ctz(bits);
+            raw_start[run] = rstart[p];
+            raw_end[run] = rend[p];
+        }
+    if (i0 <= n_words && n_words < i0 + SCAN_LB_ITEMS) *n_raw = run;
 }
 
 struct CandCtx {
@@ -649,9 +680,10 @@
 }
 
 static constexpr uint32_t MERGE_LB_BLOCKS = 32;
-__device__ __forceinline__ void k_lq_merge_scan_lb(const uint32_t np2_bid, const uint32_t np2_nb, Lookback lb, const uint32_t *__restrict__ raw_start,
-                                                   const uint32_t *__restrict__ raw_end, const uint32_t *__restrict__ n_raw, uint32_t n_host,
-                                                   uint32_t *__restrict__ headflag, uint32_t *__restrict__ hidx, uint32_t *__restrict__ err) {
+__device__ __forceinline__ void k_lq_merge_lb(const uint32_t np2_bid, const uint32_t np2_nb, Lookback lb, const uint32_t *__restrict__ raw_start,
+                                              const uint32_t *__restrict__ raw_end, const uint32_t *__restrict__ n_raw, uint32_t n_host,
+                                              uint32_t *__restrict__ lq_start, uint32_t *__restrict__ lq_end, uint32_t *__restrict__ n_reg,
+                                              uint32_t *__restrict__ err) {
     __shared__ uint32_t sh[16];
     const uint32_t bid = lb_block_id(lb, sh);
     const uint32_t n = min(*n_raw, n_host);
@@ -669,12 +701,15 @@
         const uint32_t v = j < hi ? flag(j) : 0u;
         uint32_t tot;
         const uint32_t ex = block_excl_scan<OpAdd, 16>(v, sh, tot);
-        if (j < hi) {
-            hidx[j] = carry + ex;
-            headflag[j] = v;
+        if (v) {
+            uint32_t l = j;
+            while (l + 1 < n && !flag(l + 1)) ++l;
+            lq_end[carry + ex] = raw_end[j];
+            lq_start[carry + ex] = raw_start[l];
         }
         carry += tot;
     }
+    if (threadIdx.x == 0 && (n ? (lo < n && hi == n) : bid == 0)) *n_reg = carry;
 }
 
 __device__ __forceinline__ void k_region_write(const uint32_t np2_bid0, const uint32_t np2_nb, CandCtx cx, uint32_t n_reg, const uint32_t *__restrict__ kept_read,
@@ -829,9 +864,14 @@
     else
         NP2_LAUNCH(k_cand_offsets, dim3(1), 1024, s, blk_sum, (n_reg + 3) / 4, n_reg, blk_coff, blk_soff, cand_off, reg_soff, n_cand, n_bytes, grow);
 }
-void launch_lq_merge_scan_lb(hipStream_t s, const Lookback &lb, const uint32_t *raw_start, const uint32_t *raw_end, const uint32_t *n_raw,
-                             uint32_t n_host, uint32_t *headflag, uint32_t *hidx, uint32_t *err) {
-    NP2_LAUNCH(k_lq_merge_scan_lb, dim3(MERGE_LB_BLOCKS), 1024, s, lb, raw_start, raw_end, n_raw, n_host, headflag, hidx, err);
+void launch_lq_scatter_lb(hipStream_t s, const Lookback &lb, const uint32_t *hbits, uint32_t n_words, const uint32_t *rstart,
+                          const uint32_t *rend, uint32_t *raw_start, uint32_t *raw_end, uint32_t *n_raw, uint32_t *err) {
+    const uint32_t nb = scan_lb_blocks((uint64_t)n_words + 1);
+    NP2_LAUNCH(k_lq_scatter_lb, dim3(nb), SCAN_LB_THREADS, s, lb, nb, hbits, n_words, rstart, rend, raw_start, raw_end, n_raw, err);
+}
+void launch_lq_merge_lb(hipStream_t s, const Lookback &lb, const uint32_t *raw_start, const uint32_t *raw_end, const uint32_t *n_raw,
+                        uint32_t n_host, uint32_t *lq_start, uint32_t *lq_end, uint32_t *n_reg, uint32_t *err) {
+    NP2_LAUNCH(k_lq_merge_lb, dim3(MERGE_LB_BLOCKS), 1024, s, lb, raw_start, raw_end, n_raw, n_host, lq_start, lq_end, n_reg, err);
 }
 uint32_t lq_merge_lb_blocks() { return MERGE_LB_BLOCKS; }
 void launch_region_write(hipStream_t s, const CandPtrs &c, uint32_t n_reg, const uint32_t *kept_read,
diff --git a/nextpolish2_amd/csrc/np2_ctx.hpp b/nextpolish2_amd/csrc/np2_ctx.hpp
--- a/nextpolish2_amd/csrc/np2_ctx.hpp
+++ b/nextpolish2_amd/csrc/np2_ctx.hpp
@@ -447,8 +447,7 @@
     DevBuf<int64_t> nscore;
     DevBuf<int32_t> cov, mval, smin;
     DevBuf<uint8_t> alive, cns_base, cns_cls, lq_kind, lq_nothead;
-    DevBuf<uint32_t> cns_pos, lq_next, rflag, rstart, rend, ridx, raw_start, raw_end, headflag, hidx, lq_start,
-        lq_end;
+    DevBuf<uint32_t> cns_pos, lq_next, rflag, rstart, rend, raw_start, raw_end, lq_start, lq_end;
     DevBuf<uint32_t> pj, pcount, reg_ncand, reg_bytes, reg_soff, reg_maxlen, blk_sum, blk_coff, blk_soff, kept_read, kept_len, kept_col, cand_off, cand_order, cand_seq_off, kill_ids;
     DevBuf<uint64_t> cand_kmer;
     DevBuf<uint8_t> cand_seq;
@@ -465,8 +464,7 @@
     DevBuf<uint8_t> votepack2;
     DevBuf<uint32_t> rech_headjobs;
     DevBuf<uint32_t> ecount, eval, eval_s, eflag, eidx, seed_cand, keep_n, keep_list, cns_pos2, sp_idx_s,
-        sp_idx_e, ap_g, ap_s, ap_e, rech, rech_joboff, job_len,
-        job_off32;
+        sp_idx_e, ap_g, ap_s, ap_e, rech, rech_joboff;
     DevBuf<int32_t> ew, ap_delta, ap_shift;
     DevBuf<uint64_t> ekey, ekey_s;
     DevBuf<uint16_t> keep_ks;
diff --git a/nextpolish2_amd/csrc/np2_host.cpp b/nextpolish2_amd/csrc/np2_host.cpp
--- a/nextpolish2_amd/csrc/np2_host.cpp
+++ b/nextpolish2_amd/csrc/np2_host.cpp
@@ -236,15 +236,13 @@
         uint32_t *v_first = (uint32_t *)vbuf;
         int32_t *v_refw = (int32_t *)(vbuf + RP * 4);
         uint8_t *v_seen = vbuf + RP * 8, *v_bad = vbuf + RP * 9;
-        op_fill(cx, v_first, 0xFF, RP * 4);
-        op_fill(cx, v_refw, 0, RP * 6);
+        launch_fill3(s, (uint8_t *)v_first, RP * 4, 0xFF, (uint8_t *)v_refw, RP * 6, 0, (uint8_t *)(cx->scal.p + S_M3), 4, 0);
         launch_vote_phase(s, rt, asref, use_all, cx->lq_start.p, own_lo, own_hi, cx->reg_lable.p, cx->grp.p, cx->ecount.p,
                           v_refw, v_seen, v_bad, v_first, cx->scal.p + S_ERR);
         exclusive_total_n(cx, cx->ecount.p, cx->eoff.p, n_reg);
         launch_vote_counts(s, v_first, v_bad, R, cx->scal.p + S_M1);
         cx->band.ensure(band_words + 4);
         cx->band_n.ensure((size_t)R + 2);
-        op_fill(cx, cx->scal.p + S_M3, 0, 4);
         launch_edges_row(s, rt, cx->grp.p, cx->ecount.p, cx->pj.p, cx->pcount.p, cx->alive.p, R, cx->band.p, cx->band_n.p,
                          cx->scal.p + S_M3);
         if (wide) {
@@ -550,24 +548,22 @@
                     cx->cand_seq_off.p, cx->cand_seq.p, in.base, n_groups};
         if (n_jobs) {
             EventTimer t(cx, "recheck");
-            cx->job_len.ensure(n_jobs + 2);
-            cx->job_off32.ensure(n_jobs + 2);
             cx->soff.ensure(n_jobs + 2);
             cx->sscore.ensure(n_jobs + 2);
-            cx->tmp.ensure(prim_temp_bytes((size_t)n_jobs + 2));
-            launch_rech_job_len(s, rp, n_jobs, cx->job_len.p);
-            exclusive_total_n(cx, cx->job_len.p, cx->job_off32.p, n_jobs);
-            if (blob_bound >= 0xFFFFFFF0ull)
-                blob_bound = fetch_scal(cx, cx->scal.p + S_M0, cx->job_off32.p + n_jobs)[S_M0];
+            if (blob_bound >= 0xFFFFFFF0ull) {
+                launch_rech_strings(s, next_lookback(cx, rech_string_blocks(n_jobs)), rp, n_jobs, cx->soff.p, nullptr, false,
+                                    cx->scal.p + S_ERR);
+                blob_bound = fetch_scal(cx, cx->scal.p + S_M0, (const uint32_t *)(cx->soff.p + n_jobs))[S_M0];
+            }
             cx->sstr.ensure((size_t)blob_bound + 64);
-            launch_rech_job_build(s, rp, n_jobs, cx->job_off32.p, cx->soff.p, cx->sstr.p);
+            launch_rech_strings(s, next_lookback(cx, rech_string_blocks(n_jobs)), rp, n_jobs, cx->soff.p, cx->sstr.p, true,
+                                cx->scal.p + S_ERR);
             launch_score_strings(s, cx->yaks[yak_idx].dev(), cx->sstr.p, cx->soff.p, n_jobs, min_kmer_count,
                                  cx->sscore.p, true);
-            launch_rech_apply(s, rp, cx->sscore.p, cx->keep_ks.p);
         }
         EventTimer t(cx, "recheck");
-        launch_rech_select(s, cx->rech.p, cx->scal.p + S_NRECH, n_rech, cx->cand_off.p, cx->keep_n.p, cx->keep_list.p,
-                           cx->keep_ks.p, cx->cand_order.p, first_yak, cx->reg_lable.p, cx->seed_cand.p);
+        launch_rech_apply_select(s, rp, n_jobs ? cx->sscore.p : nullptr, cx->keep_ks.p, cx->keep_n.p, cx->cand_order.p, first_yak,
+                                 cx->reg_lable.p, cx->seed_cand.p);
     }
     CnsDev out = splice_gpu(cx, in, n_reg, LB_RECH, pc.grow, to_b, version);
     launch_rech_relabel(s, cx->reg_lable.p, n_reg);
@@ -800,11 +796,8 @@
     cx->rflag.ensure(M_cap + 2);
     cx->rstart.ensure(M_cap + 2);
     cx->rend.ensure(M_cap + 2);
-    cx->ridx.ensure(M_cap + 2);
     cx->raw_start.ensure(M_cap + 2);
     cx->raw_end.ensure(M_cap + 2);
-    cx->headflag.ensure(M_cap + 2);
-    cx->hidx.ensure(M_cap + 2);
     cx->lq_start.ensure(M_cap + 2);
     cx->lq_end.ensure(M_cap + 2);
     cx->tmp.ensure(prim_temp_bytes((size_t)M_cap + 2));
@@ -819,14 +812,10 @@
     EventTimer t(cx, "lq_regions");
     launch_lq_scan(s, cx->cns_pos.p, cx->cns_base.p, cx->cns_cls.p, M_p, cx->lq_list.p, n_lq, b.lq_cap, cx->lq_kind.p,
                    cx->lq_next.p, cx->lq_nothead.p, cx->hbits.p, b.n_words + 1, cx->rstart.p, cx->rend.p);
-    launch_scan_lb_popc(s, next_lookback(cx, scan_lb_blocks((size_t)b.n_words + 1)), cx->hbits.p, cx->ridx.p, b.n_words,
-                        cx->scal.p + S_ERR);
-    launch_scatter_regions(s, cx->hbits.p, b.n_words, cx->ridx.p, cx->rstart.p, cx->rend.p, cx->raw_start.p,
-                           cx->raw_end.p, cx->scal.p + S_NRAW);
-    launch_lq_merge_scan_lb(s, next_lookback(cx, lq_merge_lb_blocks()), cx->raw_start.p, cx->raw_end.p, cx->scal.p + S_NRAW, b.M_cap,
-                            cx->headflag.p, cx->hidx.p, cx->scal.p + S_ERR);
-    launch_lq_merge_write(s, cx->raw_start.p, cx->raw_end.p, cx->scal.p + S_NRAW, cx->headflag.p, cx->hidx.p,
-                          cx->lq_start.p, cx->lq_end.p, cx->scal.p + S_NREG);
+    launch_lq_scatter_lb(s, next_lookback(cx, scan_lb_blocks((size_t)b.n_words + 1)), cx->hbits.p, b.n_words, cx->rstart.p,
+                         cx->rend.p, cx->raw_start.p, cx->raw_end.p, cx->scal.p + S_NRAW, cx->scal.p + S_ERR);
+    launch_lq_merge_lb(s, next_lookback(cx, lq_merge_lb_blocks()), cx->raw_start.p, cx->raw_end.p, cx->scal.p + S_NRAW, b.M_cap,
+                       cx->lq_start.p, cx->lq_end.p, cx->scal.p + S_NREG, cx->scal.p + S_ERR);
 }
 
 void consensus_and_regions_issue(np2_ctx *cx, np2_contig *c, uint32_t n_nodes, uint32_t n_runs, uint32_t T) {
diff --git a/nextpolish2_amd/csrc/np2_kernels.hip b/nextpolish2_amd/csrc/np2_kernels.hip
--- a/nextpolish2_amd/csrc/np2_kernels.hip
+++ b/nextpolish2_amd/csrc/np2_kernels.hip
@@ -30,7 +30,8 @@
                        uint32_t *__restrict__ dst0, const uint32_t *__restrict__ src0, uint32_t *__restrict__ dst1,
                        const uint32_t *__restrict__ src1, uint32_t *__restrict__ dst2, const uint32_t *__restrict__ src2,
                        uint32_t *__restrict__ dst3, const uint32_t *__restrict__ src3,
-                       const uint32_t *__restrict__ ends_of, uint32_t *__restrict__ ends_dst) {
+                       const uint32_t *__restrict__ ends_of, uint32_t *__restrict__ ends_dst,
+                       uint32_t *__restrict__ done_word, uint32_t done_seq, uint32_t *__restrict__ done_cnt, uint32_t done_n) {
     if (threadIdx.x == 0) {
         if (dst0) *dst0 = *src0;
         if (dst1) *dst1 = *src1;
@@ -47,9 +48,33 @@
         mbox[1 + threadIdx.x] = __hip_atomic_load(&scal[threadIdx.x], __ATOMIC_RELAXED, __HIP_MEMORY_SCOPE_AGENT);
     __threadfence_system();
     if (threadIdx.x == 0) __hip_atomic_store(&mbox[0], seq, __ATOMIC_RELEASE, __HIP_MEMORY_SCOPE_SYSTEM);
+    if (done_word && threadIdx.x == 0) {
+        __threadfence_system();
+        if (__hip_atomic_fetch_add(done_cnt, 1u, __ATOMIC_RELAXED, __HIP_MEMORY_SCOPE_AGENT) == done_n - 1) {
+            __hip_atomic_store(done_cnt, 0u, __ATOMIC_RELAXED, __HIP_MEMORY_SCOPE_AGENT);
+            __threadfence_system();
+            __hip_atomic_store(done_word, done_seq, __ATOMIC_RELEASE, __HIP_MEMORY_SCOPE_SYSTEM);
+        }
+    }
 }
 __device__ __forceinline__ void k_fill(const uint32_t np2_bid, const uint32_t np2_nb, uint8_t *__restrict__ p, uint64_t n, uint32_t v4) {
     const uint64_t o = ((uint64_t)np2_bid * 256 + threadIdx.x) * 16;
+    if (o >= n) return;
+    if ((((uintptr_t)p) & 15) == 0 && o + 16 <= n) {
+        *reinterpret_cast<uint4 *>(p + o) = make_uint4(v4, v4, v4, v4);
+    } else {
+        for (uint64_t i = o; i < min(o + 16, n); ++i) p[i] = (uint8_t)v4;
+    }
+}
+__device__ __forceinline__ void k_fill3(const uint32_t np2_bid, const uint32_t np2_nb, uint8_t *__restrict__ p0, uint64_t n0, uint32_t v0, uint8_t *__restrict__ p1,
+                                        uint64_t n1, uint32_t v1, uint8_t *__restrict__ p2, uint64_t n2, uint32_t v2) {
+    const uint32_t b0 = (uint32_t)((n0 + 4095) / 4096), b1 = (uint32_t)((n1 + 4095) / 4096);
+    uint8_t *p = p0;
+    uint64_t n = n0;
+    uint32_t v4 = v0, b = np2_bid;
+    if (b >= b0 + b1) p = p2, n = n2, v4 = v2, b -= b0 + b1;
+    else if (b >= b0) p = p1, n = n1, v4 = v1, b -= b0;
+    const uint64_t o = ((uint64_t)b * 256 + threadIdx.x) * 16;
     if (o >= n) return;
     if ((((uintptr_t)p) & 15) == 0 && o + 16 <= n) {
         *reinterpret_cast<uint4 *>(p + o) = make_uint4(v4, v4, v4, v4);
@@ -1057,59 +1082,6 @@
         atomicOr(&hbits[p >> 5], 1u << (p & 31));
     }
 }
-__device__ __forceinline__ void k_lq_bits_count(const uint32_t np2_bid, const uint32_t np2_nb, const uint32_t *__restrict__ hbits, uint32_t n_words,
-                                uint32_t *__restrict__ wcnt) {
-    const uint32_t w = np2_bid * blockDim.x + threadIdx.x;
-    if (w <= n_words) wcnt[w] = w < n_words ? (uint32_t)__builtin_popcount(hbits[w]) : 0u;
-}
-__device__ __forceinline__ void k_scatter_regions(const uint32_t np2_bid, const uint32_t np2_nb, const uint32_t *__restrict__ hbits, uint32_t n_words,
-                                  const uint32_t *__restrict__ woff, const uint32_t *__restrict__ rstart,
-                                  const uint32_t *__restrict__ rend, uint32_t *__restrict__ raw_start,
-                                  uint32_t *__restrict__ raw_end, uint32_t *__restrict__ n_raw) {
-    const uint32_t w = np2_bid * blockDim.x + threadIdx.x;
-    if (w == 0) *n_raw = woff[n_words];
-    if (w >= n_words) return;
-    uint32_t bits = hbits[w], k = woff[w];
-    for (; bits; bits &= bits - 1, ++k) {
-        const uint32_t p = (w << 5) + (uint32_t)__builtin_ctz(bits);
-        raw_start[k] = rstart[p];
-        raw_end[k] = rend[p];
-    }
-}
-
-__device__ __forceinline__ void k_lq_merge_flag(const uint32_t np2_bid, const uint32_t np2_nb, const uint32_t *__restrict__ raw_start, const uint32_t *__restrict__ raw_end,
-                                const uint32_t *__restrict__ n_raw, uint32_t *__restrict__ headflag) {
-    const uint32_t n = *n_raw;
-    for (uint32_t j = np2_bid * blockDim.x + threadIdx.x; j < n; j += np2_nb * blockDim.x)
-        headflag[j] = !(j >= 1 && raw_end[j] >= raw_start[j - 1]);
-}
-__device__ __forceinline__ void k_lq_merge_scan(const uint32_t np2_bid, const uint32_t np2_nb, const uint32_t *__restrict__ raw_start, const uint32_t *__restrict__ raw_end,
-                                                const uint32_t *__restrict__ n_raw, uint32_t n_host, uint32_t *__restrict__ headflag,
-                                                uint32_t *__restrict__ hidx) {
-    __shared__ uint32_t sh[16];
-    const uint32_t n = min(*n_raw, n_host);
-    block_scan_array<OpAdd>(
-        n, sh, [&](uint32_t j) { return (j >= 1 && raw_end[j] >= raw_start[j - 1]) ? 0u : 1u; },
-        [&](uint32_t j, uint32_t pre, uint32_t v) {
-            hidx[j] = pre;
-            headflag[j] = v;
-        });
-}
-__device__ __forceinline__ void k_lq_merge_write(const uint32_t np2_bid, const uint32_t np2_nb, const uint32_t *__restrict__ raw_start, const uint32_t *__restrict__ raw_end,
-                                 const uint32_t *__restrict__ n_raw, const uint32_t *__restrict__ headflag,
-                                 const uint32_t *__restrict__ hidx, uint32_t *__restrict__ lq_start,
-                                 uint32_t *__restrict__ lq_end, uint32_t *__restrict__ n_reg) {
-    const uint32_t n = *n_raw;
-    for (uint32_t j = np2_bid * blockDim.x + threadIdx.x; j < n; j += np2_nb * blockDim.x) {
-        if (headflag[j]) {
-            uint32_t l = j;
-            while (l + 1 < n && !headflag[l + 1]) ++l;
-            lq_end[hidx[j]] = raw_end[j];
-            lq_start[hidx[j]] = raw_start[l];
-        }
-        if (j == n - 1) *n_reg = hidx[j] + headflag[j];
-    }
-}
 
 __device__ __forceinline__ uint32_t count_ge_desc(const uint32_t *a, uint32_t n, uint32_t v) {
     uint32_t lo = 0, hi = n;
@@ -1332,10 +1304,31 @@
 void launch_post(hipStream_t s, uint32_t *scal, uint32_t n_scal, uint32_t *mbox, uint32_t seq, uint32_t *d0,
                  const uint32_t *s0, uint32_t *d1, const uint32_t *s1, uint32_t *d2, const uint32_t *s2, uint32_t *d3,
                  const uint32_t *s3, const uint32_t *ends_of, uint32_t *ends_dst) {
-    NP2_LAUNCH(k_post, dim3(1), 64, s, scal, n_scal, mbox, seq, d0, s0, d1, s1, d2, s2, d3, s3, ends_of, ends_dst);
+    NP2_LAUNCH(k_post, dim3(1), 64, s, scal, n_scal, mbox, seq, d0, s0, d1, s1, d2, s2, d3, s3, ends_of, ends_dst,
+               (uint32_t *)nullptr, 0u, (uint32_t *)nullptr, 0u);
+}
+bool post_carry_done(const char *kernel_name, void *pack, uint32_t *done_word, uint32_t done_seq, uint32_t *done_cnt, uint32_t done_n) {
+    if (strcmp(kernel_name, "k_post") != 0) return false;
+    using P = Sig<decltype(&k_post)>::pack_t;
+    constexpr size_t I = 14;
+    P &pk = *static_cast<P *>(pack);
+    auto set = [](const auto &field, auto v) {
+        static_assert(sizeof(field) == sizeof(v), "k_post's trailing parameters");
+        memcpy(const_cast<void *>(static_cast<const void *>(&field)), &v, sizeof v);
+    };
+    set(PackGet<I, P>::get(pk), done_word);
+    set(PackGet<I + 1, P>::get(pk), done_seq);
+    set(PackGet<I + 2, P>::get(pk), done_cnt);
+    set(PackGet<I + 3, P>::get(pk), done_n);
+    return true;
 }
 void launch_fill(hipStream_t s, uint8_t *p, uint64_t bytes, uint8_t byte) {
     if (bytes) NP2_LAUNCH(k_fill, grid1((bytes + 15) / 16), 256, s, p, bytes, 0x01010101u * byte);
+}
+void launch_fill3(hipStream_t s, uint8_t *p0, uint64_t n0, uint8_t v0, uint8_t *p1, uint64_t n1, uint8_t v1, uint8_t *p2, uint64_t n2,
+                  uint8_t v2) {
+    const uint64_t nb = (n0 + 4095) / 4096 + (n1 + 4095) / 4096 + (n2 + 4095) / 4096;
+    if (nb) NP2_LAUNCH(k_fill3, dim3((unsigned)nb), 256, s, p0, n0, 0x01010101u * v0, p1, n1, 0x01010101u * v1, p2, n2, 0x01010101u * v2);
 }
 void launch_copy(hipStream_t s, uint8_t *dst, const uint8_t *src, uint64_t bytes) {
     if (bytes) NP2_LAUNCH(k_copy, grid1((bytes + 15) / 16), 256, s, dst, src, bytes);
@@ -1403,27 +1396,6 @@
     NP2_LAUNCH(k_lq_scan, lq_grid(std::max(lq_cap, n_hwords / 4)), 256, s, cns_pos, cns_base, cns_cls, M_p, lq_list, n_lq, lq_cap, lq_kind, lq_next, lq_nothead, hbits, n_hwords);
     NP2_LAUNCH(k_lq_region, lq_grid(lq_cap), 256, s, cns_pos, cns_base, M_p, lq_list, n_lq, lq_cap, lq_kind, lq_next, lq_nothead, hbits, rstart, rend);
 }
-void launch_lq_bits_count(hipStream_t s, const uint32_t *hbits, uint32_t n_words, uint32_t *wcnt) {
-    NP2_LAUNCH(k_lq_bits_count, grid1((uint64_t)n_words + 1), 256, s, hbits, n_words, wcnt);
-}
-void launch_scatter_regions(hipStream_t s, const uint32_t *hbits, uint32_t n_words, const uint32_t *woff,
-                            const uint32_t *rstart, const uint32_t *rend, uint32_t *raw_start, uint32_t *raw_end,
-                            uint32_t *n_raw) {
-    NP2_LAUNCH(k_scatter_regions, grid1(std::max<uint32_t>(n_words, 1)), 256, s, hbits, n_words, woff, rstart, rend, raw_start, raw_end, n_raw);
-}
-void launch_lq_merge_flag(hipStream_t s, const uint32_t *raw_start, const uint32_t *raw_end, const uint32_t *n_raw,
-                          uint32_t *headflag) {
-    NP2_LAUNCH(k_lq_merge_flag, dim3(256), 256, s, raw_start, raw_end, n_raw, headflag);
-}
-void launch_lq_merge_scan(hipStream_t s, const uint32_t *raw_start, const uint32_t *raw_end, const uint32_t *n_raw, uint32_t n_host,
-                          uint32_t *headflag, uint32_t *hidx) {
-    NP2_LAUNCH(k_lq_merge_scan, dim3(1), 1024, s, raw_start, raw_end, n_raw, n_host, headflag, hidx);
-}
-void launch_lq_merge_write(hipStream_t s, const uint32_t *raw_start, const uint32_t *raw_end, const uint32_t *n_raw,
-                           const uint32_t *headflag, const uint32_t *hidx, uint32_t *lq_start, uint32_t *lq_end,
-                           uint32_t *n_reg) {
-    NP2_LAUNCH(k_lq_merge_write, dim3(256), 256, s, raw_start, raw_end, n_raw, headflag, hidx, lq_start, lq_end, n_reg);
-}
 void launch_read_m(hipStream_t s, const np2_read_t *reads, uint32_t R, const uint8_t *alive, const uint32_t *lq_start,
                    uint32_t n_reg, int32_t *mval) {
     NP2_LAUNCH(k_read_m, grid1(R), 256, s, reads, R, alive, lq_start, n_reg, mval);
diff --git a/nextpolish2_amd/csrc/np2_kernels.hpp b/nextpolish2_amd/csrc/np2_kernels.hpp
--- a/nextpolish2_amd/csrc/np2_kernels.hpp
+++ b/nextpolish2_amd/csrc/np2_kernels.hpp
@@ -119,6 +119,9 @@
                  const uint32_t *s2 = nullptr, uint32_t *d3 = nullptr, const uint32_t *s3 = nullptr,
                  const uint32_t *ends_of = nullptr, uint32_t *ends_dst = nullptr);
 void launch_fill(hipStream_t s, uint8_t *p, uint64_t bytes, uint8_t byte);
+void launch_fill3(hipStream_t s, uint8_t *p0, uint64_t n0, uint8_t v0, uint8_t *p1, uint64_t n1, uint8_t v1, uint8_t *p2, uint64_t n2,
+                  uint8_t v2);
+bool post_carry_done(const char *kernel_name, void *pack, uint32_t *done_word, uint32_t done_seq, uint32_t *done_cnt, uint32_t done_n);
 void launch_copy(hipStream_t s, uint8_t *dst, const uint8_t *src, uint64_t bytes);
 void launch_copy_len(hipStream_t s, uint8_t *dst, const uint8_t *src, const uint32_t *n_dev, uint32_t elem, uint64_t cap_bytes);
 void launch_copy_counted(hipStream_t s, uint32_t *dst, const uint32_t *src, const uint32_t *n_dev, uint32_t cap, uint32_t words_per = 1);
@@ -148,21 +151,12 @@
 void launch_lq_scan(hipStream_t s, const uint32_t *cns_pos, const uint8_t *cns_base, const uint8_t *cns_cls,
                     const uint32_t *M_p, const uint32_t *lq_list, const uint32_t *n_lq, uint32_t lq_cap, uint8_t *lq_kind,
                     uint32_t *lq_next, uint8_t *lq_nothead, uint32_t *hbits, uint32_t n_hwords, uint32_t *rstart, uint32_t *rend);
-void launch_lq_merge_scan_lb(hipStream_t s, const Lookback &lb, const uint32_t *raw_start, const uint32_t *raw_end, const uint32_t *n_raw,
-                             uint32_t n_host, uint32_t *headflag, uint32_t *hidx, uint32_t *err);
+void launch_lq_scatter_lb(hipStream_t s, const Lookback &lb, const uint32_t *hbits, uint32_t n_words, const uint32_t *rstart,
+                          const uint32_t *rend, uint32_t *raw_start, uint32_t *raw_end, uint32_t *n_raw, uint32_t *err);
+void launch_lq_merge_lb(hipStream_t s, const Lookback &lb, const uint32_t *raw_start, const uint32_t *raw_end, const uint32_t *n_raw,
+                        uint32_t n_host, uint32_t *lq_start, uint32_t *lq_end, uint32_t *n_reg, uint32_t *err);
 uint32_t lq_merge_lb_blocks();
-void launch_lq_merge_scan(hipStream_t s, const uint32_t *raw_start, const uint32_t *raw_end, const uint32_t *n_raw, uint32_t n_host,
-                          uint32_t *headflag, uint32_t *hidx);
 void launch_scan_lb_popc(hipStream_t s, const Lookback &lb, const uint32_t *bits, uint32_t *out, uint32_t n_words, uint32_t *err);
-void launch_lq_bits_count(hipStream_t s, const uint32_t *hbits, uint32_t n_words, uint32_t *wcnt);
-void launch_scatter_regions(hipStream_t s, const uint32_t *hbits, uint32_t n_words, const uint32_t *woff,
-                            const uint32_t *rstart, const uint32_t *rend, uint32_t *raw_start, uint32_t *raw_end,
-                            uint32_t *n_raw);
-void launch_lq_merge_flag(hipStream_t s, const uint32_t *raw_start, const uint32_t *raw_end, const uint32_t *n_raw,
-                          uint32_t *headflag);
-void launch_lq_merge_write(hipStream_t s, const uint32_t *raw_start, const uint32_t *raw_end, const uint32_t *n_raw,
-                           const uint32_t *headflag, const uint32_t *hidx, uint32_t *lq_start, uint32_t *lq_end,
-                           uint32_t *n_reg);
 void launch_read_m(hipStream_t s, const np2_read_t *reads, uint32_t R, const uint8_t *alive, const uint32_t *lq_start,
                    uint32_t n_reg, int32_t *mval);
 void launch_yak_insert(hipStream_t s, const uint64_t *words, const uint64_t *bucket_off, uint32_t n_buckets,
@@ -321,13 +315,11 @@
                         uint32_t *head_jobs, void *groups, uint32_t *job_off, uint32_t *n_groups, uint32_t *n_jobs,
                         unsigned long long *blob_bound, uint32_t *err);
 size_t rech_group_bytes();
-void launch_rech_job_len(hipStream_t s, const RechPtrs &p, uint32_t n_jobs, uint32_t *len);
-void launch_rech_job_build(hipStream_t s, const RechPtrs &p, uint32_t n_jobs, const uint32_t *soff32, uint64_t *soff64,
-                           uint8_t *blob);
-void launch_rech_apply(hipStream_t s, const RechPtrs &p, const uint16_t *score, uint16_t *keep_ks);
-void launch_rech_select(hipStream_t s, const uint32_t *rech, const uint32_t *n_rech_p, uint32_t max_rech,
-                        const uint32_t *cand_off, const uint32_t *keep_n, const uint32_t *keep_list, const uint16_t *keep_ks,
-                        const uint32_t *order, bool first_yak, uint8_t *reg_lable, uint32_t *seed_cand);
+uint32_t rech_string_blocks(uint32_t n_jobs);
+void launch_rech_strings(hipStream_t s, const Lookback &lb, const RechPtrs &p, uint32_t n_jobs, uint64_t *soff, uint8_t *blob,
+                         bool build, uint32_t *err);
+void launch_rech_apply_select(hipStream_t s, const RechPtrs &p, const uint16_t *score, uint16_t *keep_ks, const uint32_t *keep_n,
+                              const uint32_t *order, bool first_yak, uint8_t *reg_lable, uint32_t *seed_cand);
 void launch_rech_relabel(hipStream_t s, uint8_t *reg_lable, uint32_t n_reg);
 
 struct FrontOp {
diff --git a/nextpolish2_amd/csrc/np2_regions.hip b/nextpolish2_amd/csrc/np2_regions.hip
--- a/nextpolish2_amd/csrc/np2_regions.hip
+++ b/nextpolish2_amd/csrc/np2_regions.hip
@@ -975,71 +975,69 @@
         if (WRITE) out[o] = cx.cns_base[i];
     return o;
 }
-__device__ __forceinline__ void k_rech_job_len(const uint32_t np2_bid, const uint32_t np2_nb, RechCtx cx, uint32_t n_jobs, uint32_t *__restrict__ len) {
-    uint32_t j = np2_bid * blockDim.x + threadIdx.x;
-    if (j < n_jobs) len[j] = rech_string<false>(cx, j, nullptr);
-}
-__device__ __forceinline__ void k_rech_job_build(const uint32_t np2_bid, const uint32_t np2_nb, RechCtx cx, uint32_t n_jobs, const uint64_t *__restrict__ soff,
-                                 uint8_t *__restrict__ blob) {
-    uint32_t j = np2_bid * blockDim.x + threadIdx.x;
-    if (j < n_jobs) rech_string<true>(cx, j, blob + soff[j]);
-}
-__device__ __forceinline__ void k_u32_to_u64_off(const uint32_t np2_bid, const uint32_t np2_nb, const uint32_t *__restrict__ in, uint32_t n, uint64_t *__restrict__ out) {
-    uint32_t i = np2_bid * blockDim.x + threadIdx.x;
-    if (i < n) out[i] = in[i];
-}
-
-__device__ __forceinline__ void k_rech_apply(const uint32_t np2_bid, const uint32_t np2_nb, RechCtx cx, const uint16_t *__restrict__ score, uint16_t *__restrict__ keep_ks) {
+static constexpr uint32_t RECH_STR_THREADS = 256;
+__device__ __forceinline__ void k_rech_strings(const uint32_t np2_bid, const uint32_t np2_nb, Lookback lb, uint32_t n_blocks, RechCtx cx, uint32_t n_jobs,
+                                               uint64_t *__restrict__ soff, uint8_t *__restrict__ blob, uint32_t build, uint32_t *__restrict__ err) {
+    __shared__ uint32_t sh[8];
+    const uint32_t bid = lb_block_id(lb, sh);
+    const uint32_t j = bid * RECH_STR_THREADS + threadIdx.x;
+    const uint32_t len = j < n_jobs ? rech_string<false>(cx, j, nullptr) : 0u;
+    uint32_t total, pre, dummy;
+    const uint32_t ex = block_excl_scan<OpAdd, RECH_STR_THREADS / 64>(len, sh, total);
+    lb_exclusive2(lb, bid, total, 0u, sh, err, pre, dummy);
+    if (j < n_jobs) {
+        soff[j] = pre + ex;
+        if (build) rech_string<true>(cx, j, blob + (pre + ex));
+    }
+    if (bid == n_blocks - 1 && threadIdx.x == 0) soff[n_jobs] = pre + total;
+}
+
+__device__ __forceinline__ void k_rech_apply_select(const uint32_t np2_bid, const uint32_t np2_nb, RechCtx cx, const uint16_t *__restrict__ score, uint32_t apply,
+                                                    uint16_t *keep_ks, const uint32_t *__restrict__ keep_n, const uint32_t *__restrict__ order,
+                                                    uint32_t first_yak, uint8_t *__restrict__ reg_lable, uint32_t *__restrict__ seed_cand) {
     uint32_t gi = np2_bid * blockDim.x + threadIdx.x;
     if (gi >= cx.n_groups) return;
     const RechGroup &G = cx.groups[gi];
     const uint32_t j0 = cx.job_off[gi];
-    if (G.n == 1) {
+    if (apply && G.n == 1) {
         const uint32_t g = cx.rech[G.first];
         for (uint32_t t = 0; t < G.lens[0]; ++t) keep_ks[cx.cand_off[g] + t] = score[j0 + t];
-        return;
+    } else if (apply) {
+        for (uint32_t x = 0; x < G.n; ++x) {
+            const uint32_t g = cx.rech[G.first + x];
+            for (uint32_t t = 0; t < G.lens[x]; ++t) keep_ks[cx.cand_off[g] + t] = 0;
+        }
+        for (uint32_t j = 0; j < G.njobs; ++j) {
+            const uint16_t ks = score[j0 + j];
+            if (!ks) continue;
+            uint32_t rem = j;
+            for (uint32_t x = G.n; x-- > 0;) {
+                const uint32_t p = rem % G.lens[x];
+                rem /= G.lens[x];
+                keep_ks[cx.cand_off[cx.rech[G.first + x]] + p] = ks;
+            }
+        }
     }
     for (uint32_t x = 0; x < G.n; ++x) {
-        const uint32_t g = cx.rech[G.first + x];
-        for (uint32_t t = 0; t < G.lens[x]; ++t) keep_ks[cx.cand_off[g] + t] = 0;
-    }
-    for (uint32_t j = 0; j < G.njobs; ++j) {
-        const uint16_t ks = score[j0 + j];
-        if (!ks) continue;
-        uint32_t rem = j;
-        for (uint32_t x = G.n; x-- > 0;) {
-            const uint32_t p = rem % G.lens[x];
-            rem /= G.lens[x];
-            keep_ks[cx.cand_off[cx.rech[G.first + x]] + p] = ks;
-        }
-    }
-}
-
-__device__ __forceinline__ void k_rech_select(const uint32_t np2_bid, const uint32_t np2_nb, const uint32_t *__restrict__ rech, const uint32_t *__restrict__ n_rech_p,
-                              const uint32_t *__restrict__ cand_off, const uint32_t *__restrict__ keep_n,
-                              const uint32_t *__restrict__ keep_list, const uint16_t *__restrict__ keep_ks,
-                              const uint32_t *__restrict__ order, uint32_t first_yak, uint8_t *__restrict__ reg_lable,
-                              uint32_t *__restrict__ seed_cand) {
-    uint32_t e = np2_bid * blockDim.x + threadIdx.x;
-    if (e >= *n_rech_p) return;
-    const uint32_t g = rech[e], c0 = cand_off[g], n = keep_n[g];
-    uint32_t c = 0, valid = 0;
-    for (uint32_t p = 0; p < n; ++p)
-        if (keep_ks[c0 + p] != 0) {
-            if (c == 0 || order[keep_list[c0 + p]] == 0) c = p + 1;
-            ++valid;
-        }
-    if (valid > 1) reg_lable[g] |= LB_TEMP;
-    if (c != 0) {
-        seed_cand[g] = keep_list[c0 + c - 1];
-    } else if (first_yak) {
-        uint32_t i = 0;
+        const uint32_t g = cx.rech[G.first + x], c0 = cx.cand_off[g], n = keep_n[g];
+        uint32_t c = 0, valid = 0;
         for (uint32_t p = 0; p < n; ++p)
-            if (order[keep_list[c0 + p]] == 0) {
-                i = p;
-                break;
-            }
-        seed_cand[g] = keep_list[c0 + i];
+            if (keep_ks[c0 + p] != 0) {
+                if (c == 0 || order[cx.keep_list[c0 + p]] == 0) c = p + 1;
+                ++valid;
+            }
+        if (valid > 1) reg_lable[g] |= LB_TEMP;
+        if (c != 0) {
+            seed_cand[g] = cx.keep_list[c0 + c - 1];
+        } else if (first_yak) {
+            uint32_t i = 0;
+            for (uint32_t p = 0; p < n; ++p)
+                if (order[cx.keep_list[c0 + p]] == 0) {
+                    i = p;
+                    break;
+                }
+            seed_cand[g] = cx.keep_list[c0 + i];
+        }
     }
 }
 __device__ __forceinline__ void k_rech_relabel(const uint32_t np2_bid, const uint32_t np2_nb, uint8_t *__restrict__ reg_lable, uint32_t n_reg) {
@@ -1167,24 +1165,16 @@
     return RechCtx{(const RechGroup *)p.groups, p.job_off, p.rech, p.cand_off, p.keep_list, p.seq_off, p.seq,
                    p.cns_base, p.n_groups};
 }
-void launch_rech_job_len(hipStream_t s, const RechPtrs &p, uint32_t n_jobs, uint32_t *len) {
-    if (n_jobs) NP2_LAUNCH(k_rech_job_len, g1(n_jobs, 64), 64, s, mk_rech(p), n_jobs, len);
-}
-void launch_rech_job_build(hipStream_t s, const RechPtrs &p, uint32_t n_jobs, const uint32_t *soff32, uint64_t *soff64,
-                           uint8_t *blob) {
-    if (!n_jobs) return;
-    NP2_LAUNCH(k_u32_to_u64_off, g1(n_jobs + 1), 256, s, soff32, n_jobs + 1, soff64);
-    NP2_LAUNCH(k_rech_job_build, g1(n_jobs, 64), 64, s, mk_rech(p), n_jobs, soff64, blob);
-}
-void launch_rech_apply(hipStream_t s, const RechPtrs &p, const uint16_t *score, uint16_t *keep_ks) {
-    if (p.n_groups) NP2_LAUNCH(k_rech_apply, g1(p.n_groups, 64), 64, s, mk_rech(p), score, keep_ks);
-}
-void launch_rech_select(hipStream_t s, const uint32_t *rech, const uint32_t *n_rech_p, uint32_t max_rech,
-                        const uint32_t *cand_off, const uint32_t *keep_n, const uint32_t *keep_list,
-                        const uint16_t *keep_ks, const uint32_t *order, bool first_yak, uint8_t *reg_lable,
-                        uint32_t *seed_cand) {
-    if (max_rech)
-        NP2_LAUNCH(k_rech_select, g1(max_rech, 64), 64, s, rech, n_rech_p, cand_off, keep_n, keep_list, keep_ks, order, first_yak ? 1u : 0u, reg_lable, seed_cand);
+uint32_t rech_string_blocks(uint32_t n_jobs) { return std::max<uint32_t>(1, (n_jobs + RECH_STR_THREADS - 1) / RECH_STR_THREADS); }
+void launch_rech_strings(hipStream_t s, const Lookback &lb, const RechPtrs &p, uint32_t n_jobs, uint64_t *soff, uint8_t *blob,
+                         bool build, uint32_t *err) {
+    const uint32_t nb = rech_string_blocks(n_jobs);
+    NP2_LAUNCH(k_rech_strings, dim3(nb), RECH_STR_THREADS, s, lb, nb, mk_rech(p), n_jobs, soff, blob, build ? 1u : 0u, err);
+}
+void launch_rech_apply_select(hipStream_t s, const RechPtrs &p, const uint16_t *score, uint16_t *keep_ks, const uint32_t *keep_n,
+                              const uint32_t *order, bool first_yak, uint8_t *reg_lable, uint32_t *seed_cand) {
+    if (p.n_groups)
+        NP2_LAUNCH(k_rech_apply_select, g1(p.n_groups, 64), 64, s, mk_rech(p), score, score ? 1u : 0u, keep_ks, keep_n, order, first_yak ? 1u : 0u, reg_lable, seed_cand);
 }
 void launch_rech_relabel(hipStream_t s, uint8_t *reg_lable, uint32_t n_reg) {
     NP2_LAUNCH(k_rech_relabel, g1(n_reg), 256, s, reg_lable, n_reg);
```

Result: no change. 4257 (-0.7%).
